# genome/bam-readcount

Measured on AMD Instinct MI355X. Metric: pileup base-events/sec, higher is better.
Workload: dtype u32+f32

## Files before the change

bam_readcount_amd/capi.py:

```python
import ctypes as C
import os

import numpy as np

HERE = os.path.dirname(os.path.abspath(__file__))
PRODUCT_LIB = os.path.join(HERE, "csrc", "libbrc_hip.so")

NBUCKET, NI, NF, NWARN, NKERNEL = 6, 9, 4, 4, 8
I_NAMES = ["n", "smq", "sse", "plus", "minus", "nq2", "smmq", "sclip", "sbq"]
F_NAMES = ["sev", "sq2", "snm", "s3p"]

EXPORTS = [
    "brc_strerror", "brc_last_error", "brc_kernel_name", "brc_engine_kind", "brc_create", "brc_destroy",
    "brc_begin_region", "brc_push_reads", "brc_upload", "brc_compute", "brc_fetch_result", "brc_end_region",
    "brc_clear_indel_queue", "brc_region_counts", "brc_format_region", "brc_format_window", "brc_region_windows", "brc_region_warnings", "brc_window_warnings", "brc_warnings_text", "brc_set_option", "brc_format_region_parts", "brc_set_chrom", "brc_fetch_window", "brc_compute_n", "brc_host_alloc", "brc_host_free", "brc_push_reads_pinned", "brc_region_piece_steps", "brc_device_view_get", "brc_device_indels_get",
]


class Stat(C.Structure):
    _fields_ = [("i", C.c_uint32 * NI), ("f", C.c_float * NF)]


class Config(C.Structure):
    _fields_ = [("abi_version", C.c_int32), ("min_mapq", C.c_int32), ("min_bq", C.c_int32), ("max_cnt", C.c_int32),
# ... 687 lines not shown
    "brc_panel_create", "brc_panel_destroy", "brc_panel_kind", "brc_panel_last_error", "brc_panel_gather", "brc_panel_last_timing",
]
PANEL_OUT_OF_RANGE, PANEL_NOT_ASCENDING = 1, 2
PANEL_DESTS = ("ncol", "depth", "unavail", "istat", "fstat", "metrics")


class Panel(_Handle):

    PREFIX, EXPORTS, LIB, NAME = "brc_panel", PANEL_EXPORTS, PANEL_LIB, "panel"
    PROTOS = {"brc_panel_gather": (C.c_int, [C.c_void_p, C.POINTER(DeviceView), C.c_void_p, C.c_int64, C.c_int64] + [C.c_void_p] * 8)}

    def gather_raw(self, view, idx, n, dst_stride, ncol=None, depth=None, unavail=None, istat=None, fstat=None, metrics=None, status=None,
                   stream=None):
        return self.lib.brc_panel_gather(self.h, _ref(view), idx, n, dst_stride,
                                         ncol, depth, unavail, istat, fstat, metrics, status, stream)

    def gather(self, view, idx, n, dst_stride, **kw):
        self._check("brc_panel_gather", self.gather_raw(view, idx, n, dst_stride, **kw))

    def last_timing(self):
        return super().last_timing()


SELECT_LIB = os.path.join(HERE, "csrc", "libbrc_select_hip.so")
SELECT_EXPORTS = [
    "brc_select_create", "brc_select_destroy", "brc_select_kind", "brc_select_last_error", "brc_select_workspace", "brc_select_sites",
    "brc_select_last_timing",
]
SELECT_SNV, SELECT_INDEL = 1, 2
ROLE_IGNORE, ROLE_CASE, ROLE_CONTROL = 0, 1, 2
SELECT_MAX_LIB = 254
WHY_A, WHY_C, WHY_G, WHY_T, WHY_INS, WHY_DEL = 1, 2, 4, 8, 16, 32


class SelectParams(C.Structure):
    _fields_ = [("role", C.c_void_p), ("flags", C.c_uint32), ("min_depth", C.c_uint32), ("min_alt", C.c_uint32), ("frac_num", C.c_uint32),
                ("frac_den", C.c_uint32), ("ctl_min_depth", C.c_uint32), ("ctl_max_alt", C.c_uint32), ("ctl_frac_num", C.c_uint32),
                ("ctl_frac_den", C.c_uint32)]


def select_params(role=None, flags=SELECT_SNV | SELECT_INDEL, min_depth=0, min_alt=1, frac=(0, 1), ctl_min_depth=0, ctl_max_alt=2 ** 32 - 1,
                  ctl_frac=(1, 1)):
    p = SelectParams(None, flags, min_depth, min_alt, frac[0], frac[1], ctl_min_depth, ctl_max_alt, ctl_frac[0], ctl_frac[1])
    keep = None
    if role is not None:
        keep = np.ascontiguousarray(role, np.uint8)
        p.role = keep.ctypes.data
    return p, keep


class Select(_Handle):

    PREFIX, EXPORTS, LIB, NAME = "brc_select", SELECT_EXPORTS, SELECT_LIB, "select"
    PROTOS = {"brc_select_workspace": (C.c_int64, [C.POINTER(DeviceView), C.POINTER(DeviceIndels), C.c_int64]),
              "brc_select_sites": (C.c_int, [C.c_void_p, C.POINTER(DeviceView), C.POINTER(DeviceIndels), C.POINTER(SelectParams), C.c_int64, C.c_int64, C.c_int64] +
                                   [C.c_void_p] * 5)}

    def workspace(self, view, indels, n):
        return int(self.lib.brc_select_workspace(_ref(view), _ref(indels), n))

    def sites_raw(self, view, indels, params, k0, n, cap=0, idx=None, why=None, counts=None, workspace=None, stream=None):
        return self.lib.brc_select_sites(self.h, _ref(view), _ref(indels), _ref(params), k0, n, cap, idx, why, counts, workspace, stream)

    def sites(self, view, indels, params, k0, n, **kw):
        self._check("brc_select_sites", self.sites_raw(view, indels, params, k0, n, **kw))

    def last_timing(self):
        return super().last_timing()


BINS_LIB = os.path.join(HERE, "csrc", "libbrc_bins_hip.so")
BINS_EXPORTS = [
    "brc_bins_create", "brc_bins_destroy", "brc_bins_kind", "brc_bins_last_error", "brc_bins_reduce", "brc_bins_last_timing",
]
BINS_NSUM, BINS_MAX_THR, BINS_MAX_HIST, BINS_MAX_LIB = 12, 8, 4096, 65535
BINS_S_DEPTH, BINS_S_NCOL, BINS_S_BUCKET, BINS_S_NONREF, BINS_S_INS, BINS_S_DEL, BINS_S_MAXDEPTH = 0, 1, 2, 8, 9, 10, 11
BINS_DESCENDS, BINS_OUTSIDE = 1, 2


class BinsParams(C.Structure):
    _fields_ = [("edges", C.c_void_p), ("width", C.c_int64), ("n_bins", C.c_int64), ("n_thr", C.c_int32), ("n_hist", C.c_int32),
                ("thr", C.c_uint32 * BINS_MAX_THR)]


def bins_params(width=0, edges=None, n_bins=0, thresholds=(), n_hist=0):
    p = BinsParams(edges, width, n_bins, len(thresholds), n_hist)
    for t, x in enumerate(thresholds[:BINS_MAX_THR]):
        p.thr[t] = x
    return p


class Bins(_Handle):

    PREFIX, EXPORTS, LIB, NAME = "brc_bins", BINS_EXPORTS, BINS_LIB, "bins"
    PROTOS = {"brc_bins_reduce": (C.c_int, [C.c_void_p, C.POINTER(DeviceView), C.POINTER(DeviceIndels), C.POINTER(BinsParams), C.c_int64, C.c_int64] +
                                  [C.c_void_p] * 3 + [C.c_int64, C.c_void_p, C.c_void_p])}

    def reduce_raw(self, view, indels, params, k0, n, dst_stride, sums=None, covered=None, hist=None, status=None, stream=None):
        return self.lib.brc_bins_reduce(self.h, _ref(view), _ref(indels), _ref(params), k0, n, sums, covered, hist, dst_stride, status, stream)

    def reduce(self, view, indels, params, k0, n, dst_stride, **kw):
        self._check("brc_bins_reduce", self.reduce_raw(view, indels, params, k0, n, dst_stride, **kw))

    def last_timing(self):
        return super().last_timing()


RUNS_LIB = os.path.join(HERE, "csrc", "libbrc_runs_hip.so")
RUNS_EXPORTS = [
    "brc_runs_create", "brc_runs_destroy", "brc_runs_kind", "brc_runs_last_error", "brc_runs_workspace", "brc_runs_find", "brc_runs_last_timing",
]
RUNS_MAX_LIB, RUNS_MAX_CUT = 254, 15
RUNS_MIN, RUNS_MAX, RUNS_SUM = 0, 1, 2
RUNS_REF_N = 1


class RunsParams(C.Structure):
    _fields_ = [("role", C.c_void_p), ("combine", C.c_uint32), ("n_cut", C.c_uint32), ("cut", C.c_uint32 * RUNS_MAX_CUT), ("keep", C.c_uint32),
                ("flags", C.c_uint32)]


def runs_params(cuts, combine=RUNS_MIN, role=None, keep=None, flags=0):
    cuts = list(cuts)
    p = RunsParams(None, combine, len(cuts))
    for i, x in enumerate(cuts[:RUNS_MAX_CUT]):
        p.cut[i] = x
    p.keep = (1 << (len(cuts) + (2 if flags & RUNS_REF_N else 1))) - 1 if keep is None else keep
    p.flags = flags
    keepalive = None
    if role is not None:
        keepalive = np.ascontiguousarray(role, np.uint8)
        p.role = keepalive.ctypes.data
    return p, keepalive


class Runs(_Handle):

    PREFIX, EXPORTS, LIB, NAME = "brc_runs", RUNS_EXPORTS, RUNS_LIB, "runs"
    PROTOS = {"brc_runs_workspace": (C.c_int64, [C.c_int64]),
              "brc_runs_find": (C.c_int, [C.c_void_p, C.POINTER(DeviceView), C.POINTER(DeviceIndels), C.POINTER(RunsParams), C.c_int64, C.c_int64, C.c_int64] +
                                [C.c_void_p] * 7)}

    def workspace(self, n):
        return int(self.lib.brc_runs_workspace(n))

    def find_raw(self, view, indels, params, k0, n, cap=0, start=None, end=None, cls=None, counts=None, per_class=None, workspace=None, stream=None):
        return self.lib.brc_runs_find(self.h, _ref(view), _ref(indels), _ref(params), k0, n, cap, start, end, cls, counts, per_class, workspace, stream)

    def find(self, view, indels, params, k0, n, **kw):
        self._check("brc_runs_find", self.find_raw(view, indels, params, k0, n, **kw))

    def last_timing(self):
        return super().last_timing()
```

bam_readcount_amd/csrc/brc_engine.hip:

```cpp
#include <hip/hip_runtime.h>
#include <atomic>
#include <chrono>

#include <stdio.h>
#include <stdlib.h>
#include <string.h>

#include <algorithm>
#include <string>
#include <mutex>
#include <vector>

#include "brc_host.h"

namespace brc {

struct Counters {
    unsigned long long n_events, n_positions, w_sm, w_nm, w_lib;
    unsigned int n_indel_slots, n_xev;
    unsigned int xev_max, n_wave_reads;
    unsigned int n_wave_big, n_wave_huge;
    unsigned int n_literal, n_wave_eqx;
    unsigned int n_wave_eqx_big, pad_;
};

#ifdef BRC_EXP_KNOBS
#define BRC_PVAR(n) (c.variant == (n))
#define BRC_AVAR(n) (c.ann_variant == (n))
#else
#define BRC_PVAR(n) false
#define BRC_AVAR(n) false
#endif


#ifdef BRC_CHECKED
__device__ __forceinline__ const char* uniform_ptr(const char* p) {
    const uint64_t v = (uint64_t)p;
    return (const char*)(((uint64_t)(uint32_t)__builtin_amdgcn_readfirstlane((int)(uint32_t)(v >> 32)) << 32) | (uint64_t)(uint32_t)__builtin_amdgcn_readfirstlane((int)(uint32_t)v));
}
#define BRC_CKS(c, K, SITE, BUF, p, bytes, unit, piece) uniform_ptr(BRC_CK(c, K, SITE, BUF, p, bytes, unit, piece))
#else
#define BRC_CKS(c, K, SITE, BUF, p, bytes, unit, piece) (p)
#endif

__device__ __forceinline__ unsigned long long wave_sum_u64(unsigned long long v) {
#pragma unroll
    for (int o = 32; o > 0; o >>= 1) v += __shfl_xor(v, o, 64);
    return v;
}

__device__ __forceinline__ uint32_t wave_sum_u32(uint32_t v) {
    v += (uint32_t)__builtin_amdgcn_update_dpp(0, (int)v, 0xB1, 0xf, 0xf, true);
    v += (uint32_t)__builtin_amdgcn_update_dpp(0, (int)v, 0x4E, 0xf, 0xf, true);
    v += (uint32_t)__builtin_amdgcn_update_dpp(0, (int)v, 0x141, 0xf, 0xf, true);
    v += (uint32_t)__builtin_amdgcn_update_dpp(0, (int)v, 0x140, 0xf, 0xf, true);
    v += (uint32_t)__builtin_amdgcn_update_dpp(0, (int)v, 0x142, 0xa, 0xf, false);
    v += (uint32_t)__builtin_amdgcn_update_dpp(0, (int)v, 0x143, 0xc, 0xf, false);
    return (uint32_t)__builtin_amdgcn_readlane((int)v, 63);
}

__device__ __forceinline__ uint64_t wave_min_u64(uint64_t v) {
#pragma unroll
    for (int o = 32; o > 0; o >>= 1) {
        const uint64_t u = ((uint64_t)(uint32_t)__shfl_xor((int)(uint32_t)(v >> 32), o, 64) << 32) | (uint64_t)(uint32_t)__shfl_xor((int)(uint32_t)v, o, 64);
        v = u < v ? u : v;
    }
    return ((uint64_t)(uint32_t)__builtin_amdgcn_readfirstlane((int)(uint32_t)(v >> 32)) << 32) | (uint64_t)(uint32_t)__builtin_amdgcn_readfirstlane((int)(uint32_t)v);
}

__device__ __forceinline__ int lane_shr1(int v) { return __builtin_amdgcn_update_dpp(0, v, 0x138, 0xf, 0xf, false); }
__device__ __forceinline__ int lane_shl1(int v) { return __builtin_amdgcn_update_dpp(0, v, 0x130, 0xf, 0xf, false); }


enum { REFCODE_PAD = 16 };
__global__ void k_divcheck(uint32_t* __restrict__ bad) {
    const uint32_t i = blockIdx.x * blockDim.x + threadIdx.x;
    const uint32_t n = i / DIV_SMALL_M, m = i % DIV_SMALL_M;
    if (n >= DIV_SMALL_N || m == 0u) return;
    const float q = div_small((float)n, (float)m), want = (float)n / (float)m;
    if (__float_as_uint(q) != __float_as_uint(want)) atomicAdd(bad, 1u);
}
__global__ __launch_bounds__(256) void k_refcode(const char* __restrict__ ref, uint8_t* __restrict__ code, int64_t n) {
    const int64_t i = (int64_t)blockIdx.x * blockDim.x + threadIdx.x;
    const int64_t j0 = i * 16 - REFCODE_PAD;
    if (j0 >= n + REFCODE_PAD) return;
    uint32_t w[4];
    uint8_t src[16];
    if (j0 >= 0 && j0 + 16 <= n) __builtin_memcpy(src, ref + j0, 16);
    else for (int k = 0; k < 16; ++k) { const int64_t j = j0 + k; src[k] = (j >= 0 && j < n) ? (uint8_t)ref[j] : (uint8_t)'N'; }
#pragma unroll
    for (int q = 0; q < 4; ++q) {
        uint32_t v = 0;
#pragma unroll
        for (int k = 0; k < 4; ++k) {
            const int64_t j = j0 + 4 * q + k;
            const uint32_t ch = src[4 * q + k];
            const uint32_t cd = (j >= 0 && j < n) ? (ch ? nt16_of_char(ch) : 0x8fu) : 0x0fu;
            v |= cd << (8 * k);
        }
        w[q] = v;
    }
    *reinterpret_cast<uint4*>(code + i * 16) = make_uint4(w[0], w[1], w[2], w[3]);
}

enum { AW_MCAP = 1024,
       AW_MCAP_BIG = 5120,
       AW_MCAP_HUGE = 13500,
       AW_MCAP_EQX = 768, AW_MCAP_EQX_BIG = 3840 };
struct AnnPar { uint4 a, b, c; };

__device__ __forceinline__ uint32_t nzb7(uint32_t x) { return x + 0x7f7f7f7fu; }

#ifndef BRC_ANN_WAVES_PER_EU
#define BRC_ANN_WAVES_PER_EU 6
#endif
#if BRC_ANN_WAVES_PER_EU > 0
#define BRC_ANN_OCC __attribute__((amdgpu_waves_per_eu(one_stream ? BRC_ANN_WAVES_PER_EU : 5, one_stream ? BRC_ANN_WAVES_PER_EU : 5)))
#else
#define BRC_ANN_OCC
#endif
template <bool one_stream, int SH>
__global__ __launch_bounds__(256) BRC_ANN_OCC void k_annotate_groups(DevCfg c, DevIn in, DRead* __restrict__ reads, const uint32_t* __restrict__ piece_off,
                                                         Piece* __restrict__ pieces, PieceRare* __restrict__ rare, int2* __restrict__ keyreach,
                                                         uint8_t* __restrict__ eb, IndelEv* __restrict__ ev_raw, uint32_t* __restrict__ bucket_cnt,
                                                         const uint32_t* __restrict__ cigar_ro, const uint8_t* __restrict__ qual_ro,
                                                         const uint8_t* __restrict__ seq_ro, const uint8_t* __restrict__ refcode,
                                                         const uint16_t* __restrict__ wanted ) {
    c.pack_shift = SH;
    struct WaveLds { AnnPar par[64]; uint32_t sum[64]; uint32_t redo[64]; uint32_t wide[64]; uint32_t G[64]; unsigned long long mark; };
    __shared__ WaveLds lds_all[4];
    const int lane = threadIdx.x & 63;
    const uint32_t wv = __builtin_amdgcn_readfirstlane((uint32_t)threadIdx.x >> 6);
    WaveLds& W = lds_all[wv];
    const int64_t rb = ((int64_t)blockIdx.x * 4 + wv) * 64;
    if (rb >= c.n_reads) return;
    const int nrd = (int)((c.n_reads - rb) < 64 ? (c.n_reads - rb) : 64);
    const int64_t my = rb + (lane < nrd ? lane : nrd - 1);
    const bool have = lane < nrd;
    const int32_t pos = in.pos[my];
    const uint32_t flag = in.flag[my];
    const int32_t L = in.l_qseq[my];
    const uint32_t nc = in.n_cigar[my];
    const uint64_t qoff = in.qual_off[my], soff = in.seq_off[my], brow = in.bq_row[my];
    const uint32_t coff = (uint32_t)in.cig_off[my];
    int32_t rlen = 0; int clipped = L, left_clip = 0, right_clip = L; int64_t tot_d = 0, tot_is = 0;
    uint32_t cig0 = 0, n_idp = 0;
    CigShape shape;
    int n_m = 0; int32_t m1lo = 0, m1hi = 0, m2lo = 0, m2hi = 0; int64_t d1 = 0, d2 = 0;
    {
        int rs = 0; int64_t x = pos;
#ifdef BRC_CHECKED
        const uint32_t* const cig_row = BRC_CK(c, CK_ANNOTATE, 1, CB_CIGAR, cigar_ro + coff, 4ull * nc, my, -1);
#define BRC_CIG_AT(k) cig_row[k]
#else
#define BRC_CIG_AT(k) cigar_ro[coff + (k)]
#endif
        for (uint32_t k = 0; k < nc; ++k) {
            const uint32_t cg = BRC_CIG_AT(k);
            if (k == 0) cig0 = cg;
            const uint32_t op = cg & 0xfu; const int len = (int)(cg >> 4);
            shape_add(shape, op, len);
            if (is_refop(op)) rlen += len;
            if (op == CINS || op == CDEL || op == CPAD) ++n_idp;
            if (op == CDEL || op == CREF_SKIP) tot_d += len;
            if (op == CINS || op == CSOFT_CLIP) tot_is += len;
// ... 1567 lines not shown
__global__ __launch_bounds__(256) void k_xev_fold(const XEv* __restrict__ list, uint32_t* __restrict__ cnt, uint32_t* __restrict__ end, int64_t n_buckets, uint32_t* __restrict__ idx, XAgg* __restrict__ out) {
    for (int64_t b = (int64_t)blockIdx.x * 256 + threadIdx.x; b < n_buckets; b += (int64_t)gridDim.x * 256) {
        const uint32_t n = cnt[b];
        if (!n) continue;
        const uint32_t start = end[b] - n;
        const int nd = fold_xev_bucket(list, idx + start, (int)n, out + start);
        for (uint32_t j = (uint32_t)nd; j < n; ++j) out[start + j].k = NONE32;
        cnt[b] = (uint32_t)nd; end[b] = start + (uint32_t)nd;
    }
}
__global__ __launch_bounds__(256) void k_last_processed(DevCfg c, const uint32_t* __restrict__ ncol, const uint32_t* __restrict__ unavail, uint32_t* __restrict__ last) {
    __shared__ uint32_t best;
    const int l = blockIdx.x;
    if (threadIdx.x == 0) best = 0u;
    __syncthreads();
    for (int64_t hi = c.P; hi > 0; hi -= 256) {
        const int64_t k = hi - 1 - (int64_t)threadIdx.x;
        if (k >= 0 && ncol[(int64_t)l * c.PS + k] != 0u && !(c.per_lib && unavail[k] != NONE32)) atomicMax(&best, (uint32_t)k + 1u);
        __syncthreads();
        const uint32_t seen = best;
        __syncthreads();
        if (seen) break;
    }
    if (threadIdx.x == 0) last[l] = best ? best - 1u : NONE32;
}

__global__ __launch_bounds__(256) void k_text_len(DevCfg c, DevIn in, Planes pl, TextCtx t, TextAux ax, uint32_t* __restrict__ len) {
    const int64_t k = (int64_t)blockIdx.x * blockDim.x + threadIdx.x;
    if (k > c.P) return;
    len[k] = k < c.P ? text_line(c, in, pl, t, ax, k, nullptr) : 0u;
}
__global__ __launch_bounds__(256) void k_text_total(const uint32_t* __restrict__ len, int64_t n, unsigned long long* __restrict__ total) {
    unsigned long long v = 0ull;
    for (int64_t k = (int64_t)blockIdx.x * blockDim.x + threadIdx.x; k < n; k += (int64_t)gridDim.x * blockDim.x) v += len[k];
#pragma unroll
    for (int o = 32; o > 0; o >>= 1) v += (unsigned long long)__shfl_xor((long long)v, o, 64);
    if ((threadIdx.x & 63) == 0 && v) atomicAdd(total, v);
}
__global__ __launch_bounds__(256) void k_text_write(DevCfg c, DevIn in, Planes pl, TextCtx t, TextAux ax, const uint32_t* __restrict__ off, char* __restrict__ text) {
    const int64_t k = (int64_t)blockIdx.x * blockDim.x + threadIdx.x;
    if (k >= c.P || off[k + 1] == off[k]) return;
    (void)text_line(c, in, pl, t, ax, k, text + off[k]);
}

__global__ __launch_bounds__(256) void k_indel_scatter(DevCfg c, const IndelEv* __restrict__ raw, int64_t n_raw, uint32_t* __restrict__ cursor,
                                                       IndelEv* __restrict__ ev) {
    const int64_t i = (int64_t)blockIdx.x * blockDim.x + threadIdx.x;
    if (i >= n_raw) return;
    const IndelEv e = raw[i];
    if (e.key_lo == NONE32) return;
    ev[atomicAdd(&cursor[indel_bucket(c, e.key_lo)], 1u)] = e;
}

__global__ __launch_bounds__(256) void k_unavail(DevCfg c, DevIn in, uint32_t* __restrict__ unavail) {
    const int64_t i = (int64_t)blockIdx.x * blockDim.x + threadIdx.x;
    if (i >= c.n_reads || in.lib[i] >= 0) return;
    const uint32_t nc = in.n_cigar[i]; const uint32_t* cg = in.cigar + in.cig_off[i];
    if (!read_enters(in.flag[i], cg, nc) || in.pos[i] < 0) return;
    int64_t rlen = 0;
    for (uint32_t k = 0; k < nc; ++k) if (is_refop(cg[k] & 0xfu)) rlen += (int64_t)(cg[k] >> 4);
    int64_t k0 = (int64_t)in.pos[i] - c.pos0, k1 = k0 + rlen;
    if (k0 < 0) k0 = 0;
    if (k1 > c.P) k1 = c.P;
    for (int64_t k = k0; k < k1; ++k) atomicMin(&unavail[k], (uint32_t)i);
}

__global__ __launch_bounds__(256) void k_indel_reduce(DevCfg c, DevIn in, const DRead* __restrict__ reads, const uint32_t* __restrict__ cnt,
                                                      const uint32_t* __restrict__ cursor, int64_t n_buckets, IndelEv* __restrict__ ev,
                                                      const uint32_t* __restrict__ unavail, IndelOut* __restrict__ out,
                                                      Counters* __restrict__ ctr) {
    __shared__ unsigned long long sh[4 * 2];
    unsigned long long w[2] = {0, 0};
    if (blockIdx.x == 0 && threadIdx.x == 0) ctr->n_indel_slots = n_buckets > 0 ? cursor[n_buckets - 1] : 0u;
    const int64_t stride = (int64_t)gridDim.x * blockDim.x;
    for (int64_t b = (int64_t)blockIdx.x * blockDim.x + threadIdx.x; b < n_buckets; b += stride) {
        const uint32_t n = cnt[b];
        if (!n) continue;
        const uint32_t start = cursor[b] - n;
        uint32_t wsm = 0, wnm = 0;
        reduce_indel_bucket(c, in, reads, ev + start, (int)n, unavail, out + start, wsm, wnm);
        w[0] += wsm; w[1] += wnm;
    }
    block_sum_u64<2>(w, sh);
    if (threadIdx.x == 0) {
        if (w[0]) atomicAdd(&ctr->w_sm, w[0]);
        if (w[1]) atomicAdd(&ctr->w_nm, w[1]);
    }
}


static void* pinned_alloc(size_t n) {
    void* p = nullptr;
    if (hipHostMalloc(&p, n ? n : 1, hipHostMallocDefault) != hipSuccess) return nullptr;
    return p;
}
static void pinned_release(void* p) { (void)hipHostFree(p); }
static const HostAlloc kPinned = {pinned_alloc, pinned_release};

template <class T>
struct PBuf : HBuf<T> {
    PBuf() { this->A = &kPinned; } ~PBuf() { this->destroy(); }
    PBuf(const PBuf&) = delete; PBuf& operator=(const PBuf&) = delete;
};

static std::atomic<uint64_t> g_dev_allocs{0}, g_dev_alloc_ns{0};
template <class T>
struct DBuf {
    T* p = nullptr; size_t cap = 0;
    size_t req = 0;
    DBuf() = default; DBuf(const DBuf&) = delete; DBuf& operator=(const DBuf&) = delete;
    ~DBuf() { if (p) (void)hipFree(p); }
    template <class U> U* as() const { return reinterpret_cast<U*>(p); }
    hipError_t ensure(size_t bytes) {
        req = bytes;
        if (bytes <= cap) return hipSuccess;
        struct Tm { std::chrono::steady_clock::time_point t0 = std::chrono::steady_clock::now();
                    ~Tm() { g_dev_alloc_ns += (uint64_t)std::chrono::duration_cast<std::chrono::nanoseconds>(std::chrono::steady_clock::now() - t0).count(); ++g_dev_allocs; } } tm_;
        const bool regrow = p != nullptr;
        if (p) { (void)hipFree(p); p = nullptr; cap = 0; }
        size_t want = bytes + (regrow ? bytes / 2 : bytes / 8) + 256;
        hipError_t e = hipMalloc((void**)&p, want);
        if (e != hipSuccess) { e = hipMalloc((void**)&p, bytes); want = bytes; }
        if (e == hipSuccess) cap = want;
        return e;
    }
};

template <class H, hipError_t (*DESTROY)(H)>
struct Owned {
    H h = nullptr;
    Owned() = default; Owned(const Owned&) = delete; Owned& operator=(const Owned&) = delete;
    ~Owned() { if (h) (void)DESTROY(h); }
    operator H() const { return h; }
};
typedef Owned<hipStream_t, hipStreamDestroy> Stream;
typedef Owned<hipEvent_t, hipEventDestroy> Event;

enum { T_ANNOTATE = 0, T_SCAN_ENDS, T_TILES, T_PILEUP, T_COUNT, T_INDEL_SCAN, T_INDEL_FILL, T_INDEL_REDUCE, T_N };
static const char* kKernelNames[BRC_NKERNEL] = {"k_annotate", "k_scan_ends", "k_tiles", "k_pileup", "k_xev_fold+finalize",
                                                "k_scan_indel", "k_indel_fill", "k_indel_reduce"};

#define HIPCHK(x) do { hipError_t _e = (x); if (_e != hipSuccess) { return hip_fail(_e, #x); } } while (0)

[[maybe_unused]] static void pin_instantiation_order() {
    const void* const k[] = {(const void*)k_annotate_groups<true, 16>, (const void*)k_annotate_groups<true, 12>, (const void*)k_annotate_groups<false, 16>, (const void*)k_annotate_groups<false, 12>,
        (const void*)k_annotate_wave<16, AW_MCAP, 4>, (const void*)k_annotate_wave<12, AW_MCAP, 4>, (const void*)k_annotate_wave<16, AW_MCAP_BIG, 1>, (const void*)k_annotate_wave<12, AW_MCAP_BIG, 1>,
        (const void*)k_annotate_wave<16, AW_MCAP_EQX, 4, true>, (const void*)k_annotate_wave<12, AW_MCAP_EQX, 4, true>, (const void*)k_annotate_wave<16, AW_MCAP_EQX_BIG, 1, true>, (const void*)k_annotate_wave<12, AW_MCAP_EQX_BIG, 1, true>,
        (const void*)k_annotate_wave<16, AW_MCAP_HUGE, 1>, (const void*)k_annotate_wave<12, AW_MCAP_HUGE, 1>, (const void*)k_annotate_cursor<16>, (const void*)k_annotate_cursor<12>,
        (const void*)k_scan_reduce<OpSumU32>, (const void*)k_scan_aggregates<OpSumU32>, (const void*)k_scan_apply<OpSumU32, false>, (const void*)k_scan_aggregates<OpMaxU64>, (const void*)k_compact_tiles<true>, (const void*)k_compact_tiles<false>,
        (const void*)k_pileup2<true, 16>, (const void*)k_pileup2<true, 12>, (const void*)k_pileup2<false, 16>, (const void*)k_pileup2<false, 12>};
    (void)k;
}

class HipBackend : public Backend {
    std::string err; int device = 0;
    DevCfg c; DevIn in;
    int64_t ntiles = 0; uint64_t n_indel_cap = 0;
    std::vector<int64_t> lib_base;
    std::vector<uint16_t> h_wanted; bool has_wanted = false; std::vector<uint32_t> h_tilelist;
    unsigned wide_slices = 1;
    bool text_started[2] = {false, false}; uint64_t text_total[2] = {0, 0}; int64_t text_n[2] = {0, 0}; int text_slot = 0;
    std::mutex text_mu;
    Planes pl_last;
    enum { COMPACT_PIECES_PER_READ = 12 };
    bool compact_on = false; uint64_t compact_total = 0; bool compact_sized = false;
    struct { const uint4* pieces; const PieceRare* rare; const uint2* rng; } kp = {nullptr, nullptr, nullptr};
    bool wave_on = false;
    bool wave_big = false;
    enum { WAVE_FORM_BLOCKS = 768,
           WAVE_FORM_BLOCKS_BIG = 512,
           WAVE_FORM_BLOCKS_HUGE = 256 };
    bool wave_huge = false;
    bool wave_eqx = false; uint32_t s_max_ncigar = 0;
    bool cursor_on = false;
    unsigned long long h_steps[3] = {0, 0, 0};
    std::vector<XAgg> xagg_compact; std::vector<IndelOut> iout_compact;
    enum { XEV_SHARDS = 1024 }; size_t xev_cap = 0;
    Counters h_ctr; bool computed = false;
    bool lists_enqueued = false, lists_host = false;
    Stream stream, stream2;
    enum { EV_RING = 32 };
    struct EvSet { Event evt[T_N + 1], ev_indel[4]; };
    EvSet evsets[EV_RING]; size_t n_evsets = 0;
    Event* evt = nullptr; Event* ev_indel = nullptr;
    Event ev_text[2], ev_lines;
    PBuf<Staged::WidePair> h_wpairs; PBuf<char> h_text[2]; PBuf<uint32_t> h_toff[2], h_total, h_lastproc[2];
    struct HostSet { PBuf<uint32_t> ncol, depth, slotid, si, unavail; PBuf<float> sf; } h_pl, w_pl;
    PBuf<IndelOut> h_iout; PBuf<XAgg> h_xagg;
    DBuf<int32_t> d_pos, d_lq, d_nm, d_sm; DBuf<uint16_t> d_flag; DBuf<uint8_t> d_mapq, d_tags, d_seq, d_qual; DBuf<int16_t> d_lib;
    DBuf<uint32_t> d_nc, d_cigar, d_pieceoff, d_ievoff; DBuf<uint64_t> d_co, d_so, d_qo, d_bqrow; DBuf<char> d_ref; DBuf<uint8_t> d_refcode;
    DBuf<uint16_t> d_wanted; DBuf<uint32_t> d_tilelist; DBuf<uint2> d_wpairs; DBuf<int64_t> d_libbase;
    DBuf<uint8_t> d_bq; DBuf<uint16_t> d_bqw; DBuf<Piece> d_pieces; DBuf<PieceRare> d_rare; DBuf<int2> d_keyreach; DBuf<DRead> d_reads;
    DBuf<uint32_t> d_wavelist, d_nc_k1; DBuf<unsigned long long> d_agg; DBuf<uint2> d_rng;
    DBuf<uint32_t> d_ccnt, d_coff; DBuf<Piece> d_cpieces; DBuf<PieceRare> d_crare; DBuf<uint2> d_crng; DBuf<unsigned long long> d_ctot;
    DBuf<uint32_t> d_ncol, d_depth, d_slotid, d_si, d_unavail; DBuf<float> d_sf; DBuf<uint4> d_tilectr; DBuf<unsigned long long> d_part; DBuf<Counters> d_ctr;
    DBuf<XEv> d_xev, d_xevc; DBuf<uint32_t> d_xevn, d_xcnt, d_xend, d_xidx; DBuf<XAgg> d_xagg;
    DBuf<uint32_t> d_cnt, d_cursor; DBuf<IndelEv> d_ev, d_evraw; DBuf<IndelOut> d_iout;
    DBuf<uint32_t> d_tlen, d_toff, d_lastproc; DBuf<char> d_text, d_tctx; DBuf<unsigned long long> d_total64;
#ifdef BRC_CHECKED
    DBuf<ChkState> d_chk; ChkState h_chk;
    void chk_fill() {
        memset(&h_chk, 0, sizeof h_chk);
        auto set = [&](int b, const auto& d) { h_chk.ext[b].lo = (uint64_t)d.p; h_chk.ext[b].hi = (uint64_t)d.p + d.req; };
        set(CB_CIGAR, d_cigar); set(CB_SEQ, d_seq); set(CB_QUAL, d_qual); set(CB_REFCODE, d_refcode); set(CB_EB, d_bq); set(CB_BQW, d_bqw);
        set(CB_PIECES, d_pieces); set(CB_RARE, d_rare); set(CB_KEYREACH, d_keyreach); set(CB_READS, d_reads); set(CB_EVRAW, d_evraw); set(CB_CNT, d_cnt);
        set(CB_WANTED, d_wanted); set(CB_RNG, d_rng); set(CB_UNAVAIL, d_unavail); set(CB_TILELIST, d_tilelist); set(CB_NCOL, d_ncol); set(CB_DEPTH, d_depth);
        set(CB_SLOTID, d_slotid); set(CB_SI, d_si); set(CB_SF, d_sf); set(CB_XEV, d_xev); set(CB_XEVN, d_xevn); set(CB_TILECTR, d_tilectr);
        const bool cz = compact_on && compact_sized;
        set(CB_KP_PIECES, cz ? d_cpieces : d_pieces); set(CB_KP_RARE, cz ? d_crare : d_rare); set(CB_KP_RNG, cz ? d_crng : d_rng);
        if (const char* sh = getenv("BRC_CHECKED_SHRINK")) { const int b = atoi(sh); const char* cpos = strchr(sh, ':'); if (b >= 0 && b < CB_N && cpos) { const uint64_t by = strtoull(cpos + 1, nullptr, 10); ChkExt& x = h_chk.ext[b]; x.hi = x.hi - x.lo > by ? x.hi - by : x.lo; } }
    }
    int chk_report() {
        if (hipMemcpy(&h_chk, d_chk.p, sizeof h_chk, hipMemcpyDeviceToHost) != hipSuccess) { err = "checked build: cannot read the fault record"; return BRC_E_HIP; }
        if (!h_chk.count) return BRC_OK;
        static const char* const kBuf[CB_N] = {"cigar", "seq4", "qual", "refcode", "event bytes", "wide words", "pieces", "rare records", "keyreach", "reads", "raw indel events", "indel bucket counts",
                                               "wanted lanes", "tile ranges", "unavail", "tile list", "ncol", "depth", "slotid", "integer slot planes", "float slot planes", "third-allele lists",
                                               "third-allele cursors", "tile counters", "LDS rows", "LDS queue", "pieces (pileup)", "rare records (pileup)", "tile ranges (pileup)"};
        char b[512];
        snprintf(b, sizeof b, "BRC_CHECKED: %u out-of-bounds device access(es); first: kernel %s, site %u, buffer '%s' [0x%llx, 0x%llx), address 0x%llx + %llu bytes (offset %lld), %s %lld, piece %lld",
                 h_chk.count, h_chk.kernel == CK_ANNOTATE ? "k_annotate_groups" : "k_pileup2", h_chk.site, h_chk.buf < CB_N ? kBuf[h_chk.buf] : "?",
                 (unsigned long long)h_chk.ext[h_chk.buf < CB_N ? h_chk.buf : 0].lo, (unsigned long long)h_chk.ext[h_chk.buf < CB_N ? h_chk.buf : 0].hi, (unsigned long long)h_chk.addr,
                 (unsigned long long)h_chk.bytes, (long long)(h_chk.addr - h_chk.ext[h_chk.buf < CB_N ? h_chk.buf : 0].lo), h_chk.kernel == CK_ANNOTATE ? "read" : "tile", (long long)h_chk.unit, (long long)h_chk.piece);
        err = b; fprintf(stderr, "%s\n", b);
        return BRC_E_HIP;
    }
#endif

    int hip_fail(hipError_t e, const char* what) {
        char b[512];
        snprintf(b, sizeof b, "%s: %s", what, hipGetErrorString(e));
        err = b;
        return e == hipErrorOutOfMemory ? BRC_E_NOMEM : BRC_E_HIP;
    }
    bool indels_active() const { return n_indel_cap > 0 && c.P > 0 && c.n_reads > 0; }
    int ensure_xev_lists() {
        const size_t n = (size_t)XEV_SHARDS * xev_cap + 1;
        HIPCHK(d_xev.ensure(n * sizeof(XEv))); HIPCHK(d_xevc.ensure(n * sizeof(XEv))); HIPCHK(d_xidx.ensure(n * 4)); HIPCHK(d_xagg.ensure(n * sizeof(XAgg)));
        return BRC_OK;
    }

  public:
    int init(int dev) {
        int n = 0;
        if (hipGetDeviceCount(&n) != hipSuccess || n <= 0) { err = "no HIP device visible"; return BRC_E_NODEVICE; }
        if (dev < 0 || dev >= n) { err = "device ordinal out of range"; return BRC_E_NODEVICE; }
        device = dev;
        HIPCHK(hipSetDevice(device));
        HIPCHK(hipStreamCreateWithFlags(&stream.h, hipStreamNonBlocking));
        { const int rc0 = ensure_evsets(1); if (rc0) return rc0; }
        HIPCHK(hipStreamCreateWithFlags(&stream2.h, hipStreamNonBlocking));
        {
            uint32_t* d_bad = nullptr; uint32_t bad = 0;
            HIPCHK(hipMalloc(&d_bad, sizeof(uint32_t)));
            HIPCHK(hipMemsetAsync(d_bad, 0, sizeof(uint32_t), stream));
            hipLaunchKernelGGL(k_divcheck, dim3((DIV_SMALL_N * DIV_SMALL_M + 255) / 256), dim3(256), 0, stream, d_bad);
            HIPCHK(hipMemcpyAsync(&bad, d_bad, sizeof(uint32_t), hipMemcpyDeviceToHost, stream));
            HIPCHK(hipStreamSynchronize(stream));
            (void)hipFree(d_bad);
            if (bad) { err = "this device's reciprocal does not give correctly rounded small-integer quotients (div_small self-check failed)"; return BRC_E_HIP; }
        }
        for (Event& e : ev_text) HIPCHK(hipEventCreateWithFlags(&e.h, hipEventDisableTiming));
        HIPCHK(hipEventCreateWithFlags(&ev_lines.h, hipEventDisableTiming));
        return BRC_OK;
    }
    ~HipBackend() override {
        (void)hipSetDevice(device);
        if (getenv("BRC_ENGINE_TIMING")) fprintf(stderr, "device buffers: %llu (re)allocations, %.3f s\n", (unsigned long long)g_dev_allocs.load(), (double)g_dev_alloc_ns.load() * 1e-9);
    }
    int ensure_evsets(size_t n) {
        for (; n_evsets < n; ++n_evsets) {
            for (Event& e : evsets[n_evsets].evt) if (!e.h) HIPCHK(hipEventCreate(&e.h));
            for (Event& e : evsets[n_evsets].ev_indel) if (!e.h) HIPCHK(hipEventCreate(&e.h));
        }
        evt = evsets[0].evt; ev_indel = evsets[0].ev_indel;
        return BRC_OK;
    }
    const HostAlloc* host_alloc() override { return &kPinned; }
    const char* last_error() const override { return err.c_str(); }

    template <class T>
    int up(DBuf<T>& d, const HBuf<T>& h, size_t n) {
        HIPCHK(d.ensure((n + 16) * sizeof(T)));
        if (n) HIPCHK(hipMemcpyAsync(d.p, h.p, n * sizeof(T), hipMemcpyHostToDevice, stream));
        return BRC_OK;
    }

    int up_arena(DBuf<uint8_t>& d, const HBuf<uint8_t>& h, const std::vector<Staged::Seg>& segs, uint64_t total) {
        if (segs.empty()) return up(d, h, h.n);
        HIPCHK(d.ensure((size_t)total + 16));
        for (const Staged::Seg& g : segs) if (g.n) HIPCHK(hipMemcpyAsync(d.p + g.off, g.p, (size_t)g.n, hipMemcpyHostToDevice, stream));
        return BRC_OK;
    }
    bool adopts_arenas() const override { return true; }

    int upload(const brc_config& cfg, const Staged& s, Geometry& g) override {
        HIPCHK(hipSetDevice(device));
        computed = false;
        memset(&c, 0, sizeof c);
        c.min_mapq = cfg.min_mapq; c.min_bq = cfg.min_bq; c.per_lib = cfg.per_lib; c.insertion_centric = cfg.insertion_centric;
        c.Lp = g.Lp; c.ref_len_check = cfg.ref_len_check; c.has_ref = g.ref != nullptr;
        g.PS = (g.P + 63) & ~(int64_t)63;
        c.beg0 = g.beg0; c.end = g.end; c.pos0 = g.pos0; c.P = g.P; c.PS = g.PS; c.ref_lo = g.ref_lo; c.ref_hi = g.ref_hi; c.ref_len = g.ref_len;
        c.n_reads = s.n; c.table_len = test_knob(TK_NO_TABLE) ? 0 : s.modal_len();
        c.n_pieces = s.n_pieces; lib_base = s.lib_base; c.max_lqseq = s.max_lqseq;
        c.ibucket_shift = indel_bucket_shift(s.n_indel_ops, c.P, c.Lp);
        if (const char* ib = test_knob(TK_IBUCKET_SHIFT)) { const int v = atoi(ib); if (v == 2 || v == 4 || v == 6) c.ibucket_shift = v; }
        choose_pack(s.max_lqseq, test_knob(TK_FLUSH_K) ? atoi(test_knob(TK_FLUSH_K)) : 0, test_knob(TK_PACK_LIM) ? atoi(test_knob(TK_PACK_LIM)) : 0, c.flush_k, c.pack_lim, c.pack_lim_lo, c.pack_shift);
        c.force_dom = test_knob(TK_FORCE_DOM) ? atoi(test_knob(TK_FORCE_DOM)) : -1;
#ifdef BRC_CHECKED
        HIPCHK(d_chk.ensure(sizeof(ChkState))); c.chk = d_chk.p;
#endif
#ifdef BRC_EXP_KNOBS
        c.variant = getenv("BRC_PILEUP_VARIANT") ? atoi(getenv("BRC_PILEUP_VARIANT")) : 0;
        c.ann_variant = getenv("BRC_ANN_VARIANT") ? atoi(getenv("BRC_ANN_VARIANT")) : 0;
#endif
        compact_on = s.n > 0 && s.n_pieces > (int64_t)COMPACT_PIECES_PER_READ * s.n;
        if (const char* ck = test_knob(TK_COMPACT)) compact_on = atoi(ck) != 0 && s.n_pieces > 0;
        compact_sized = false; compact_total = 0; h_steps[0] = h_steps[1] = h_steps[2] = 0;
        const size_t n = (size_t)s.n;
        int rc;
        if ((rc = up(d_pos, s.pos, n)) || (rc = up(d_flag, s.flag, n)) || (rc = up(d_mapq, s.mapq, n)) || (rc = up(d_lib, s.lib, n)) ||
            (rc = up(d_lq, s.l_qseq, n)) || (rc = up(d_nc, s.n_cigar, n)) || (rc = up(d_co, s.cig_off, n)) || (rc = up(d_so, s.seq_off, n)) ||
            (rc = up(d_qo, s.qual_off, n)) || (rc = up(d_nm, s.nm, n)) || (rc = up(d_sm, s.sm, n)) || (rc = up(d_tags, s.tags, n)) ||
            (rc = up(d_cigar, s.cigar, s.cigar.n)) || (rc = up_arena(d_seq, s.seq4, s.seq_seg, s.seq_total)) || (rc = up_arena(d_qual, s.qual, s.qual_seg, s.qual_total)))
            return rc;
        const size_t rl = (size_t)(g.ref_hi - g.ref_lo);
        HIPCHK(d_ref.ensure(rl + 16));
        HIPCHK(d_refcode.ensure(rl + 2 * REFCODE_PAD + 16));
        if (rl) HIPCHK(hipMemcpyAsync(d_ref.p, g.ref + g.ref_lo, rl, hipMemcpyHostToDevice, stream));
        in.pos = d_pos.p; in.flag = d_flag.p; in.mapq = d_mapq.p; in.lib = d_lib.p; in.l_qseq = d_lq.p; in.n_cigar = d_nc.p; in.cig_off = d_co.p;
        in.seq_off = d_so.p; in.qual_off = d_qo.p; in.nm = d_nm.p; in.sm = d_sm.p; in.tags = d_tags.p; in.cigar = d_cigar.p; in.seq4 = d_seq.p; in.qual = d_qual.p;
        in.ref = d_ref.p;
        HIPCHK(d_bq.ensure(s.bq_elems + EB_PAD_FRONT + EB_PAD_BACK + (size_t)std::max<int32_t>(s.max_lqseq, 0)));
        {
            if (s.bq_elems >> 34) { err = "region too large: 2^34 bases and more"; return BRC_E_LIMIT; }
            const size_t tab_bytes = ((((size_t)(s.bq_elems >> 4) + 2) * 4) + 255) & ~(size_t)255;
            h_wpairs.clear();
            { const size_t nw = s.n_wide(); if (!h_wpairs.reserve(nw + 1)) { err = "host allocation failed (wide-stream list)"; return BRC_E_NOMEM; } h_wpairs.n = nw; }
            const uint64_t wq_elems = s.wide_layout(h_wpairs.p, (uint32_t)(tab_bytes / 32));
            {
                const uint64_t groups = (h_wpairs.n + 63) / 64, per_group = groups ? (wq_elems >> 4) / groups : 0;
                wide_slices = (unsigned)std::min<uint64_t>(std::max<uint64_t>(per_group / 512, 1), 64);
            }
            if ((tab_bytes / 32 + (wq_elems >> 4)) >> 32) { err = "region too large: 2^36 bases of reads with escape bases"; return BRC_E_LIMIT; }
            HIPCHK(d_bqw.ensure(tab_bytes + ((size_t)wq_elems + 16) * sizeof(uint16_t)));
            in.bqw = d_bqw.p;
#ifdef BRC_CHECKED
            HIPCHK(hipMemsetAsync(d_bqw.p, 0xff, tab_bytes, stream));
#endif
            if (h_wpairs.n) {
                HIPCHK(d_wpairs.ensure(h_wpairs.n * sizeof(Staged::WidePair)));
                HIPCHK(hipMemcpyAsync(d_wpairs.p, h_wpairs.p, h_wpairs.n * sizeof(Staged::WidePair), hipMemcpyHostToDevice, stream));
            }
        }
        in.eb = d_bq.p + EB_PAD_FRONT;
        if ((rc = up(d_bqrow, s.bq_row, n)) || (rc = up(d_pieceoff, s.piece_off, n))) return rc;
        in.bq_row = d_bqrow.p;
        in.rcp = nullptr;
        const size_t np = (size_t)c.n_pieces;
        HIPCHK(d_pieces.ensure((np + 4) * sizeof(Piece))); HIPCHK(d_rare.ensure((np + 2) * sizeof(PieceRare)));
        HIPCHK(d_keyreach.ensure((np + 16) * sizeof(int2)));
        wave_eqx = n > 0 && c.has_ref && s.has_eqx && s.max_ncigar >= 3;
        wave_on = n > 0 && c.has_ref && (s.max_ncigar >= 5 || wave_eqx);
        s_max_ncigar = s.max_ncigar;
        if (const char* wk = test_knob(TK_WAVE_FORM)) { wave_on = wave_on && atoi(wk) != 0; wave_eqx = wave_eqx && wave_on; }
        wave_big = wave_on && s.max_ncigar > (uint32_t)AW_MCAP;
        wave_huge = wave_on && s.max_ncigar > (uint32_t)AW_MCAP_BIG;
        cursor_on = n > 0 && s.has_empty_m;
        if (wave_on || cursor_on) { HIPCHK(d_wavelist.ensure((4 * (size_t)n + 96) * sizeof(uint32_t))); HIPCHK(d_nc_k1.ensure(((size_t)n + 16) * sizeof(uint32_t))); }
        HIPCHK(d_libbase.ensure((lib_base.size() + 1) * sizeof(int64_t)));
        if (!lib_base.empty()) HIPCHK(hipMemcpyAsync(d_libbase.p, lib_base.data(), lib_base.size() * sizeof(int64_t), hipMemcpyHostToDevice, stream));
        const size_t P = (size_t)c.PS, Lp = (size_t)c.Lp;
        ntiles = (c.P + TILE - 1) / TILE;
        n_indel_cap = c.has_ref ? s.n_indel_ops : 0;
        h_wanted = s.wanted_tiles(c.pos0, c.P); has_wanted = !h_wanted.empty();
        h_tilelist.clear();
        if (has_wanted) {
            HIPCHK(d_wanted.ensure(h_wanted.size() * 2 + 16)); HIPCHK(hipMemcpyAsync(d_wanted.p, h_wanted.data(), h_wanted.size() * 2, hipMemcpyHostToDevice, stream));
            for (size_t t = 0; t < h_wanted.size(); ++t) if (h_wanted[t] != (uint16_t)TILE_UNWANTED) h_tilelist.push_back((uint32_t)t);
            HIPCHK(d_tilelist.ensure(h_tilelist.size() * 4 + 16));
            if (!h_tilelist.empty()) HIPCHK(hipMemcpyAsync(d_tilelist.p, h_tilelist.data(), h_tilelist.size() * 4, hipMemcpyHostToDevice, stream));
        }
        if (n_indel_cap && ((uint64_t)c.P * (uint64_t)c.Lp >= 0xffffffffull || n_indel_cap >= 0xfffffff0ull)) { err = "region too large: (positions x libraries) and the indel operators must stay below 2^32"; return BRC_E_ARG; }
        const size_t nagg = std::max<size_t>(std::max<size_t>((std::max<size_t>(np, P * Lp) + SCAN_CHUNK - 1) / SCAN_CHUNK, (np + TR_CHUNK - 1) / TR_CHUNK), 1);
        HIPCHK(d_reads.ensure((n + 1) * sizeof(DRead)));
        HIPCHK(d_agg.ensure(nagg * 8 + 16)); HIPCHK(d_rng.ensure(((size_t)ntiles * Lp + 1) * sizeof(uint2)));
        HIPCHK(d_ncol.ensure(Lp * P * 4 + 16)); HIPCHK(d_depth.ensure(Lp * P * 4 + 16)); HIPCHK(d_unavail.ensure(P * 4 + 16));
        HIPCHK(d_slotid.ensure(Lp * P * 4 + 16)); HIPCHK(d_si.ensure(Lp * 2 * NI * P * 4 + 16)); HIPCHK(d_sf.ensure(Lp * 2 * NF * P * 4 + 16));
        {
            const char* xc = test_knob(TK_XEV_CAP);
            const size_t want = xc ? (size_t)std::max(atoi(xc), 1) : std::max<size_t>(256, np / 8 / XEV_SHARDS);
            if (want > xev_cap) xev_cap = want;
        }
        if ((rc = ensure_xev_lists())) return rc;
        HIPCHK(d_xevn.ensure((size_t)XEV_SHARDS * XEV_CTR_STRIDE * 4));
        HIPCHK(d_xcnt.ensure(((size_t)ntiles * Lp + 2) * 4)); HIPCHK(d_xend.ensure(((size_t)ntiles * Lp + 2) * 4));
        HIPCHK(d_part.ensure(4096 * 5 * sizeof(unsigned long long)));
        HIPCHK(d_ctr.ensure(sizeof(Counters))); HIPCHK(d_tilectr.ensure(((size_t)ntiles * Lp + 1) * sizeof(uint4)));
        in.iev_off = nullptr;
        if (n_indel_cap) {
            const size_t nbk = (size_t)indel_buckets(c);
            if ((rc = up(d_ievoff, s.iev_off, n))) return rc;
            in.iev_off = d_ievoff.p;
            HIPCHK(d_cnt.ensure(nbk * 4 + 16)); HIPCHK(d_cursor.ensure(nbk * 4 + 16)); HIPCHK(d_evraw.ensure((n_indel_cap + 1) * sizeof(IndelEv)));
            HIPCHK(d_ev.ensure((n_indel_cap + 1) * sizeof(IndelEv))); HIPCHK(d_iout.ensure((n_indel_cap + 1) * sizeof(IndelOut)));
        }
        if (has_wanted && P) {
            HIPCHK(hipMemsetAsync(d_ncol.p, 0, Lp * P * 4, stream)); HIPCHK(hipMemsetAsync(d_depth.p, 0, Lp * P * 4, stream));
            HIPCHK(hipMemsetD32Async((hipDeviceptr_t)d_slotid.p, (int)((uint32_t)NB_NONE | ((uint32_t)NB_NONE << 8)), Lp * P, stream));
            HIPCHK(hipMemsetAsync(d_tilectr.p, 0, (size_t)ntiles * Lp * sizeof(uint4), stream));
        }
        HIPCHK(hipStreamSynchronize(stream));
        return BRC_OK;
    }

    template <class K> K by_pack(K k16, K k12) const { return c.pack_shift == 16 ? k16 : k12; }
    uint8_t* eb_out() const { return d_bq.p + EB_PAD_FRONT; }
    IndelEv* evraw() const { return indels_active() ? d_evraw.p : nullptr; }
    const uint16_t* wanted() const { return has_wanted ? d_wanted.p : nullptr; }
    const uint8_t* refcode() const { return d_refcode.p + REFCODE_PAD; }

    void launch_annotate_groups(const DevIn& in_k1) {
        const auto k = c.Lp == 1 ? by_pack(k_annotate_groups<true, 16>, k_annotate_groups<true, 12>) : by_pack(k_annotate_groups<false, 16>, k_annotate_groups<false, 12>);
        hipLaunchKernelGGL(k, dim3((unsigned)((c.n_reads + 255) / 256)), dim3(256), 0, stream, c, in_k1, d_reads.p, d_pieceoff.p, d_pieces.p, d_rare.p, d_keyreach.p,
                           eb_out(), evraw(), d_cnt.p, in.cigar, in.qual, in.seq4, refcode(), wanted());
    }
    template <int MCAP, int WAVES, bool EQX = false>
    void launch_annotate_wave(unsigned grid, const uint32_t* list, int step, const unsigned int* count) {
        hipLaunchKernelGGL(by_pack(k_annotate_wave<16, MCAP, WAVES, EQX>, k_annotate_wave<12, MCAP, WAVES, EQX>), dim3(grid), dim3(WAVES * 64), 0, stream, c, in, list, step, count,
                           d_reads.p, d_pieceoff.p, d_pieces.p, d_rare.p, d_keyreach.p, eb_out(), evraw(), d_cnt.p, refcode(), wanted());
    }
    void launch_annotate_cursor() {
        hipLaunchKernelGGL(by_pack(k_annotate_cursor<16>, k_annotate_cursor<12>), dim3((unsigned)std::min<int64_t>((c.n_reads + 63) / 64, 1024)), dim3(64), 0, stream, c, in,
                           d_wavelist.p + (2 * (size_t)c.n_reads + 32), &d_ctr.p->n_literal, d_reads.p, d_pieceoff.p, d_pieces.p, d_rare.p, d_keyreach.p, eb_out(), evraw(), d_cnt.p, wanted());
    }
    template <class Op, bool INCL>
    int scan(const typename Op::T* src, typename Op::T* dst, int64_t n) {
        if (n <= 0) return BRC_OK;
        const int64_t nb = (n + SCAN_CHUNK - 1) / SCAN_CHUNK;
        typename Op::T* agg = d_agg.as<typename Op::T>();
        hipLaunchKernelGGL((k_scan_reduce<Op>), dim3((unsigned)nb), dim3(SCAN_T), 0, stream, src, n, agg);
        hipLaunchKernelGGL((k_scan_aggregates<Op>), dim3(1), dim3(1024), 0, stream, agg, nb);
        hipLaunchKernelGGL((k_scan_apply<Op, INCL>), dim3((unsigned)nb), dim3(SCAN_T), 0, stream, src, dst, n, agg);
        HIPCHK(hipGetLastError());
        return BRC_OK;
    }
    template <bool COUNT>
    void launch_compact_tiles() {
        hipLaunchKernelGGL((k_compact_tiles<COUNT>), dim3((unsigned)((ntiles + 3) / 4), (unsigned)c.Lp), dim3(256), 0, stream, c, d_pieces.as<const uint4>(), d_rare.p, d_rng.p, ntiles, d_ccnt.p,
                           COUNT ? nullptr : d_coff.p, COUNT ? nullptr : d_cpieces.as<uint4>(), COUNT ? nullptr : d_crare.p, COUNT ? nullptr : d_crng.p, d_ctot.p);
    }
    void stage_pileup() {
        const int64_t n_listed = (int64_t)h_tilelist.size();
        if (ntiles <= 0 || (has_wanted && n_listed == 0)) return;
        unsigned nwg = (unsigned)(((has_wanted ? n_listed : ntiles) + PILEUP_WAVES - 1) / PILEUP_WAVES);
        nwg = (nwg + 7u) & ~7u;
#ifdef BRC_EXP_KNOBS
        static const unsigned dyn_lds = getenv("BRC_PILEUP_LDS_PAD") ? (unsigned)atoi(getenv("BRC_PILEUP_LDS_PAD")) : 0u;
#else
        const unsigned dyn_lds = 0u;
#endif
        const auto k = has_wanted ? by_pack(k_pileup2<true, 16>, k_pileup2<true, 12>) : by_pack(k_pileup2<false, 16>, k_pileup2<false, 12>);
        hipLaunchKernelGGL(k, dim3(nwg, (unsigned)c.Lp), dim3(PILEUP_WAVES * 64), dyn_lds, stream, c, in, kp.pieces, kp.rare, kp.rng, ntiles, pl_last, d_tilectr.p, in.eb, in.bqw, d_unavail.p,
                           refcode(), d_wanted.p, d_tilelist.p, n_listed);
    }

    int stage_annotate() {
        const int64_t n = c.n_reads;
        if (n <= 0) { if (c.per_lib && c.P > 0) HIPCHK(hipMemsetAsync(d_unavail.p, 0xff, (size_t)c.PS * 4, stream)); return BRC_OK; }
        Counters* const ctr = d_ctr.p;
        const int64_t rl = c.ref_hi - c.ref_lo;
        if (c.has_ref)
            hipLaunchKernelGGL(k_refcode, dim3((unsigned)(((rl + 2 * REFCODE_PAD + 15) / 16 + 255) / 256)), dim3(256), 0, stream, in.ref, d_refcode.p, rl);
        if (h_wpairs.n)
            hipLaunchKernelGGL(k_wide_rows, dim3((unsigned)((h_wpairs.n + 255) / 256), wide_slices), dim3(256), 0, stream, c, in, d_wpairs.p, (uint32_t)h_wpairs.n, d_bqw.p);
        DevIn in_k1 = in;
        if (wave_on || cursor_on) {
            hipLaunchKernelGGL(k_pick_wave, dim3((unsigned)((n + 255) / 256)), dim3(256), 0, stream, c, in, d_nc_k1.p, d_wavelist.p, (uint32_t)n, &ctr->n_wave_reads, &ctr->n_wave_big, &ctr->n_wave_huge,
                               wave_on ? 1 : 0, cursor_on ? 1 : 0, &ctr->n_literal, &ctr->n_wave_eqx, &ctr->n_wave_eqx_big);
            in_k1.n_cigar = d_nc_k1.p;
        }
        launch_annotate_groups(in_k1);
        if (wave_on) {
            const uint32_t* const wl = d_wavelist.p;
            const unsigned nb = (unsigned)std::min<int64_t>((n + 3) / 4, (int64_t)WAVE_FORM_BLOCKS), nb_big = (unsigned)std::min<int64_t>(n, (int64_t)WAVE_FORM_BLOCKS_BIG);
            launch_annotate_wave<AW_MCAP, 4>(nb, wl, 1, &ctr->n_wave_reads);
            if (wave_big)
                launch_annotate_wave<AW_MCAP_BIG, 1>(nb_big, wl + (n - 1), -1, &ctr->n_wave_big);
            if (wave_eqx) {
                launch_annotate_wave<AW_MCAP_EQX, 4, true>(nb, wl + (3 * n + 48), 1, &ctr->n_wave_eqx);
                if (s_max_ncigar > (uint32_t)AW_MCAP_EQX) launch_annotate_wave<AW_MCAP_EQX_BIG, 1, true>(nb_big, wl + (4 * n + 47), -1, &ctr->n_wave_eqx_big);
            }
            if (wave_huge)
                launch_annotate_wave<AW_MCAP_HUGE, 1>((unsigned)std::min<int64_t>(n, (int64_t)WAVE_FORM_BLOCKS_HUGE), wl + (n + 16), 1, &ctr->n_wave_huge);
        }
        if (cursor_on) launch_annotate_cursor();
        if (c.per_lib) {
            HIPCHK(hipMemsetAsync(d_unavail.p, 0xff, (size_t)c.PS * 4, stream));
            hipLaunchKernelGGL(k_unavail, dim3((unsigned)((n + 255) / 256)), dim3(256), 0, stream, c, in, d_unavail.p);
        }
        return BRC_OK;
    }
    bool have_tiles() const { return c.n_pieces > 0 && ntiles > 0; }
    unsigned reach_blocks() const { return (unsigned)((c.n_pieces + TR_CHUNK - 1) / TR_CHUNK); }
    void stage_tile_reach() {
        if (!have_tiles()) return;
        hipLaunchKernelGGL(k_reach_blockmax, dim3(reach_blocks()), dim3(TR_T), 0, stream, d_keyreach.p, c.n_pieces, d_libbase.p, c.Lp, d_agg.p);
        hipLaunchKernelGGL((k_scan_aggregates<OpMaxU64>), dim3(1), dim3(1024), 0, stream, d_agg.p, (int64_t)reach_blocks());
    }
    int stage_tile_ranges() {
        const int Lp = c.Lp;
        for (int l = 0; l < Lp && ntiles > 0; ++l)
            if (lib_base[(size_t)l + 1] == lib_base[(size_t)l]) HIPCHK(hipMemsetAsync(d_rng.p + (int64_t)l * ntiles, 0, (size_t)ntiles * sizeof(uint2), stream));
        if (have_tiles())
            hipLaunchKernelGGL(k_tiles_all, dim3(reach_blocks()), dim3(TR_T), 0, stream, c, d_keyreach.p, c.n_pieces, d_libbase.p, Lp, d_agg.p, ntiles, d_rng.p);
        const int64_t n_listed = (int64_t)h_tilelist.size();
        if (has_wanted && n_listed > 0)
            hipLaunchKernelGGL(k_narrow_tiles, dim3((unsigned)((n_listed * Lp + 255) / 256)), dim3(256), 0, stream, d_wanted.p, d_tilelist.p, n_listed, ntiles, Lp, c.pos0, d_rng.p, d_keyreach.p);
        kp = {d_pieces.as<const uint4>(), d_rare.p, d_rng.p};
        return BRC_OK;
    }
    int stage_compact() {
        if (!compact_on || !have_tiles()) return BRC_OK;
        int rc; const int64_t np_all = c.n_pieces;
        const size_t nslot = (size_t)ntiles * (size_t)c.Lp;
        HIPCHK(d_ccnt.ensure((nslot + 2) * 4)); HIPCHK(d_coff.ensure((nslot + 2) * 4)); HIPCHK(d_crng.ensure((nslot + 1) * sizeof(uint2))); HIPCHK(d_ctot.ensure(24));
        HIPCHK(hipMemsetAsync(d_ctot.p, 0, 24, stream));
        HIPCHK(hipMemsetAsync(d_ccnt.p + nslot, 0, 4, stream));
        const bool by_read = c.Lp == 1 && !(test_knob(TK_COMPACT) && atoi(test_knob(TK_COMPACT)) == 2);
        if (by_read) {
            HIPCHK(hipMemsetAsync(d_ccnt.p, 0, nslot * 4, stream));
            hipLaunchKernelGGL(k_count_piece_tiles, dim3((unsigned)((np_all + 255) / 256)), dim3(256), 0, stream, c, d_pieces.as<const uint4>(), np_all, d_ccnt.p);
        } else launch_compact_tiles<true>();
        if ((rc = scan<OpSumU32, false>(d_ccnt.p, d_coff.p, (int64_t)nslot + 1))) return rc;
        const bool first_pass = !compact_sized;
        if (first_pass) {
            uint32_t tot = 0;
            HIPCHK(hipMemcpyAsync(&tot, d_coff.p + nslot, 4, hipMemcpyDeviceToHost, stream));
            HIPCHK(hipMemcpyAsync(h_steps, d_ctot.p, 16, hipMemcpyDeviceToHost, stream));
            HIPCHK(hipStreamSynchronize(stream));
            compact_total = tot; compact_sized = true;
            HIPCHK(d_cpieces.ensure(((size_t)compact_total + 4) * sizeof(Piece))); HIPCHK(d_crare.ensure(((size_t)compact_total + 2) * sizeof(PieceRare)));
        }
        if (by_read)
            hipLaunchKernelGGL(k_compact_reads, dim3((unsigned)((ntiles + 4 * CR_GROUP - 1) / (4 * CR_GROUP))), dim3(256), 0, stream, c, d_pieces.as<const uint4>(), d_rare.p, d_rng.p, d_pieceoff.p, d_keyreach.p, ntiles,
                               d_coff.p, d_cpieces.as<uint4>(), d_crare.p, d_crng.p, d_ctot.p);
        else launch_compact_tiles<false>();
        if (by_read && first_pass) {
            HIPCHK(hipMemcpyAsync(h_steps, d_ctot.p, 24, hipMemcpyDeviceToHost, stream));
            HIPCHK(hipStreamSynchronize(stream));
            if (h_steps[2]) { err = "tile compaction: a tile holds more live read segments than the pass over the segments counted for it"; return BRC_E_HIP; }
        }
        kp = {d_cpieces.as<const uint4>(), d_crare.p, d_crng.p};
#ifdef BRC_CHECKED
        {
            HIPCHK(hipStreamSynchronize(stream));
            ChkState seen; HIPCHK(hipMemcpy(&seen, d_chk.p, sizeof seen, hipMemcpyDeviceToHost));
            chk_fill(); ChkState upd = h_chk; upd.count = seen.count; upd.kernel = seen.kernel; upd.site = seen.site; upd.buf = seen.buf; upd.addr = seen.addr; upd.bytes = seen.bytes; upd.unit = seen.unit; upd.piece = seen.piece;
            HIPCHK(hipMemcpy(d_chk.p, &upd, sizeof upd, hipMemcpyHostToDevice));
        }
#endif
        return BRC_OK;
    }
    int stage_xev_fold() {
        if (ntiles <= 0) return BRC_OK;
        int rc; const int64_t nxb = ntiles * c.Lp;
        HIPCHK(hipMemsetAsync(d_xcnt.p, 0, (size_t)nxb * 4, stream));
        hipLaunchKernelGGL(k_xev_compact, dim3((unsigned)XEV_SHARDS), dim3(256), 0, stream, d_xev.p, d_xevn.p, (uint32_t)xev_cap, (uint32_t)XEV_SHARDS, d_xevc.p, d_ctr.p, d_xcnt.p, c.Lp);
        if ((rc = scan<OpSumU32, false>(d_xcnt.p, d_xend.p, nxb))) return rc;
        hipLaunchKernelGGL(k_xev_scatter, dim3(256), dim3(256), 0, stream, d_xevc.p, d_ctr.p, d_xend.p, d_xidx.p, c.Lp);
        hipLaunchKernelGGL(k_xev_fold, dim3((unsigned)std::min<int64_t>((nxb + 255) / 256, 2048)), dim3(256), 0, stream, d_xevc.p, d_xcnt.p, d_xend.p, nxb, d_xidx.p, d_xagg.p);
        return BRC_OK;
    }
    void stage_counters() {
        if (c.P <= 0) return;
        const unsigned nb = (unsigned)std::min<int64_t>(((c.Lp > 1 ? c.P / 4 : ntiles) + 255) / 256 + 1, c.Lp > 1 ? 4096 : 256);
        hipLaunchKernelGGL(k_finalize, dim3(nb), dim3(256), 0, stream, c, d_ncol.p, d_tilectr.p, (int64_t)ntiles * c.Lp, d_part.p);
        hipLaunchKernelGGL(k_finalize_sum, dim3(1), dim3(256), 0, stream, d_part.p, (int)nb, d_ctr.p);
    }
    int stage_indels() {
        int rc; const int64_t n_buckets = indel_buckets(c);
        HIPCHK(hipEventRecord(ev_indel[0], stream));
        if ((rc = scan<OpSumU32, false>(d_cnt.p, d_cursor.p, n_buckets))) return rc;
        HIPCHK(hipEventRecord(ev_indel[1], stream));
        hipLaunchKernelGGL(k_indel_scatter, dim3((unsigned)((n_indel_cap + 255) / 256)), dim3(256), 0, stream, c, d_evraw.p, (int64_t)n_indel_cap, d_cursor.p, d_ev.p);
        HIPCHK(hipEventRecord(ev_indel[2], stream));
        hipLaunchKernelGGL(k_indel_reduce, dim3((unsigned)std::min<int64_t>((n_buckets + 255) / 256, 4096)), dim3(256), 0, stream, c, in, d_reads.p, d_cnt.p, d_cursor.p, n_buckets, d_ev.p, d_unavail.p,
                           d_iout.p, d_ctr.p);
        HIPCHK(hipEventRecord(ev_indel[3], stream));
        return BRC_OK;
    }

    int enqueue_pass(size_t set) {
        evt = evsets[set].evt; ev_indel = evsets[set].ev_indel;
        int rc;
        lists_host = lists_enqueued = false;
        HIPCHK(hipMemsetAsync(d_ctr.p, 0, sizeof(Counters), stream));
        HIPCHK(hipMemsetAsync(d_xevn.p, 0, (size_t)XEV_SHARDS * XEV_CTR_STRIDE * 4, stream));
        if (indels_active()) HIPCHK(hipMemsetAsync(d_cnt.p, 0, (size_t)indel_buckets(c) * 4, stream));
#ifdef BRC_CHECKED
        if (set == 0) { chk_fill(); HIPCHK(hipMemcpyAsync(d_chk.p, &h_chk, sizeof h_chk, hipMemcpyHostToDevice, stream)); HIPCHK(hipStreamSynchronize(stream)); }
#endif
        pl_last = Planes{d_ncol.p, d_depth.p, d_slotid.p, d_si.p, d_sf.p, d_unavail.p, d_xev.p, d_xevn.p, (uint32_t)xev_cap, (uint32_t)XEV_SHARDS};
        HIPCHK(hipEventRecord(evt[T_ANNOTATE], stream));
        if ((rc = stage_annotate())) return rc;
        HIPCHK(hipEventRecord(evt[T_SCAN_ENDS], stream));
        stage_tile_reach();
        HIPCHK(hipEventRecord(evt[T_TILES], stream));
        if ((rc = stage_tile_ranges()) || (rc = stage_compact())) return rc;
        HIPCHK(hipEventRecord(evt[T_PILEUP], stream));
        stage_pileup();
        HIPCHK(hipEventRecord(evt[T_COUNT], stream));
        if ((rc = stage_xev_fold())) return rc;
        stage_counters();
        HIPCHK(hipEventRecord(evt[T_INDEL_SCAN], stream));
        if (indels_active() && (rc = stage_indels())) return rc;
        HIPCHK(hipEventRecord(evt[T_N], stream));
        HIPCHK(hipGetLastError());
        return BRC_OK;
    }
    int finish_passes(bool* again) {
        HIPCHK(hipMemcpyAsync(&h_ctr, d_ctr.p, sizeof(Counters), hipMemcpyDeviceToHost, stream));
        HIPCHK(hipStreamSynchronize(stream));
        *again = false;
#ifdef BRC_CHECKED
        { const int rcc = chk_report(); if (rcc) return rcc; }
#endif
        if ((size_t)h_ctr.xev_max > xev_cap) {
            xev_cap = (size_t)h_ctr.xev_max * 2;
            const int rc = ensure_xev_lists(); if (rc) return rc;
            *again = true;
        }
        return BRC_OK;
    }
    int add_timing(size_t set, brc_timing* t) {
// ... 218 lines not shown
```

bam_readcount_amd/csrc/brc_host.cpp:

```cpp
#if defined(__x86_64__)
#include <immintrin.h>
#endif
#include "brc_host.h"

#include <math.h>
#include <stdio.h>
#include <stdlib.h>

#include <algorithm>
#include <atomic>
#include <chrono>
#include <deque>
#include <thread>
#include <functional>
#include <memory>
#include <queue>
#include <condition_variable>

namespace brc {

static unsigned probe_cpus() {
    unsigned n = std::thread::hardware_concurrency(); if (n == 0) n = 1;
    double quota = 0;
    if (FILE* f = fopen("/sys/fs/cgroup/cpu.max", "r")) {
        char q[64]; long long per = 0;
        if (fscanf(f, "%63s %lld", q, &per) == 2 && strcmp(q, "max") != 0 && per > 0) quota = atof(q) / (double)per;
        fclose(f);
    } else {
        long long q = -1, per = 0;
        if (FILE* g = fopen("/sys/fs/cgroup/cpu/cpu.cfs_quota_us", "r")) { if (fscanf(g, "%lld", &q) != 1) q = -1; fclose(g); }
        if (FILE* g = fopen("/sys/fs/cgroup/cpu/cpu.cfs_period_us", "r")) { if (fscanf(g, "%lld", &per) != 1) per = 0; fclose(g); }
        if (q > 0 && per > 0) quota = (double)q / (double)per;
    }
    if (quota > 0 && quota < (double)n) n = (unsigned)(quota + 0.999);
    if (n < 1) n = 1;
    return n;
}
unsigned effective_cpus() { static const unsigned cached = probe_cpus(); return cached; }

static inline double now_s() { return std::chrono::duration<double>(std::chrono::steady_clock::now().time_since_epoch()).count(); }

template <class F>
static void parallel_for(int64_t n, unsigned nthr, F fn) {
    if (n <= 0) return;
    if (nthr > (unsigned)n) nthr = (unsigned)n;
    if (nthr <= 1) { for (int64_t i = 0; i < n; ++i) fn(i); return; }
    std::atomic<int64_t> next(0);
    auto work = [&]() { for (;;) { const int64_t i = next.fetch_add(1); if (i >= n) break; fn(i); } };
    std::vector<std::thread> th;
    for (unsigned t = 1; t < nthr; ++t) th.emplace_back(work);
    work();
    for (std::thread& t : th) t.join();
}

class Pool {
    std::vector<std::thread> th;
    std::mutex mu; std::condition_variable cv_go, cv_done;
    std::function<void(int64_t)> job; int64_t job_n = 0; std::atomic<int64_t> next{0};
    uint64_t gen = 0; unsigned busy = 0; bool stop = false;
    void worker() {
        uint64_t seen = 0;
        for (;;) {
            { std::unique_lock<std::mutex> lk(mu); cv_go.wait(lk, [&] { return stop || gen != seen; }); if (stop) return; seen = gen; }
            for (;;) { const int64_t i = next.fetch_add(1); if (i >= job_n) break; job(i); }
            { std::lock_guard<std::mutex> lk(mu); if (--busy == 0) cv_done.notify_one(); }
        }
    }
  public:
    explicit Pool(unsigned n) { try { th.reserve(n); for (unsigned t = 0; t < n; ++t) th.emplace_back([this] { worker(); }); } catch (...) {} }
    ~Pool() { { std::lock_guard<std::mutex> lk(mu); stop = true; } cv_go.notify_all(); for (std::thread& t : th) t.join(); }
    unsigned size() const { return (unsigned)th.size() + 1; }
    template <class F> void run(int64_t n, F fn) {
        if (n <= 0) return;
        if (th.empty() || n == 1) { for (int64_t i = 0; i < n; ++i) fn(i); return; }
        { std::lock_guard<std::mutex> lk(mu); job = fn; job_n = n; next = 0; busy = (unsigned)th.size(); ++gen; }
        cv_go.notify_all();
        for (;;) { const int64_t i = next.fetch_add(1); if (i >= n) break; fn(i); }
        std::unique_lock<std::mutex> lk(mu); cv_done.wait(lk, [&] { return busy == 0; });
    }
};

void Staged::init(const HostAlloc* A) { each_buf([A](auto& h) { h.A = A; }); }
void Staged::clear() {
    each_buf([](auto& h) { h.clear(); });
    bq_elems = 0; memset(len_hist, 0, sizeof len_hist); n = 0; min_pos = 0; max_end = 0; n_indel_ops = 0;
    seq_seg.clear(); qual_seg.clear(); seq_total = 0; qual_total = 0;
    lib_base.clear(); n_pieces = 0; max_lqseq = 0; max_ncigar = 0; has_empty_m = false; has_eqx = false; max_span = 0;
    win_beg.clear(); win_end.clear();
}
void Staged::destroy() { each_buf([](auto& h) { h.destroy(); }); }
bool Staged::reserve_reads(size_t reads, size_t cigar_ops) {
    bool ok = cigar.reserve(cigar_ops);
    each_read_buf([&](auto& h) { ok = ok && h.reserve(reads); });
    return ok;
}
std::vector<uint16_t> Staged::wanted_tiles(int32_t pos0, int64_t P) const {
    std::vector<uint16_t> w;
    if (win_beg.empty() || P <= 0) return w;
    const int64_t nt = (P + TILE - 1) / TILE;
    w.assign((size_t)nt, (uint16_t)TILE_UNWANTED);
    for (size_t i = 0; i < win_beg.size(); ++i) {
        int64_t k0 = (int64_t)win_beg[i] - 1 - pos0, k1 = (int64_t)win_end[i] - pos0;
        if (k0 < 0) k0 = 0;
        if (k1 > P) k1 = P;
        for (int64_t t = k0 / TILE; k1 > k0 && t <= (k1 - 1) / TILE; ++t) {
            const uint32_t a = (uint32_t)std::max<int64_t>(k0 - t * TILE, 0), b = (uint32_t)std::min<int64_t>(k1 - 1 - t * TILE, TILE - 1);
            uint16_t& x = w[(size_t)t];
            if (x == (uint16_t)TILE_UNWANTED) x = (uint16_t)(a | (b << 8));
            else x = (uint16_t)(std::min<uint32_t>(x & 0xffu, a) | (std::max<uint32_t>(x >> 8, b) << 8));
        }
    }
    return w;
}
void Staged::layout_pieces(int Lp, bool per_lib) {
    lib_base.assign((size_t)Lp + 1, 0);
    for (int64_t i = 0; i < n; ++i) if (piece_cnt.p[i]) lib_base[(size_t)(per_lib ? lib.p[i] : 0) + 1] += piece_cnt.p[i];
    for (int l = 0; l < Lp; ++l) lib_base[(size_t)l + 1] += lib_base[(size_t)l];
    n_pieces = lib_base[(size_t)Lp];
    std::vector<int64_t> cur(lib_base.begin(), lib_base.end() - 1);
    piece_off.n = (size_t)n;
    for (int64_t i = 0; i < n; ++i) {
        const int l = per_lib ? (int)lib.p[i] : 0;
        if (!piece_cnt.p[i]) { piece_off.p[i] = (uint32_t)cur[(size_t)((l >= 0 && l < Lp) ? l : 0)]; continue; }
        piece_off.p[i] = (uint32_t)cur[(size_t)l]; cur[(size_t)l] += piece_cnt.p[i];
    }
    if (per_lib && Lp > 1) {
        std::vector<uint64_t> rows((size_t)Lp + 2, 0);
        auto slot = [&](int64_t i) { const int l = (int)lib.p[i]; return (size_t)((l >= 0 && l < Lp) ? l : Lp); };
        for (int64_t i = 0; i < n; ++i) rows[slot(i) + 1] += ((uint64_t)l_qseq.p[i] + 15u) & ~(uint64_t)15u;
        for (int l = 0; l <= Lp; ++l) rows[(size_t)l + 1] += rows[(size_t)l];
        for (int64_t i = 0; i < n; ++i) { const size_t k = slot(i); bq_row.p[i] = rows[k]; rows[k] += ((uint64_t)l_qseq.p[i] + 15u) & ~(uint64_t)15u; }
    }
}
uint64_t Staged::wide_layout(WidePair* pairs, uint32_t first16) const {
    uint64_t w = 0; size_t k = 0;
    for (int64_t i = 0; i < n; ++i) if (wide.p[i]) {
        if (pairs) { WidePair x; x.read = (uint32_t)i; x.w16 = first16 + (uint32_t)(w >> 4); pairs[k++] = x; }
        w += ((uint64_t)l_qseq.p[i] + 15u) & ~(uint64_t)15u;
    }
    return w;
}
static bool read_has_escape_words(const uint8_t* qual, const uint8_t* seq4, int32_t L) {
    if (L <= 0) return false;
    const uint64_t K01 = 0x0101010101010101ull, K80 = 0x8080808080808080ull, K7F = 0x7f7f7f7f7f7f7f7full;
    int32_t j = 0;
    for (; j + 8 <= L; j += 8) {
        uint64_t x; memcpy(&x, qual + j, 8);
        const uint64_t zero = (x - K01) & ~x & K80;
        const uint64_t big = (((x & K7F) + (uint64_t)(128 - EB_ESC) * K01) | x) & K80;
        if (zero | big) return true;
    }
    for (; j < L; ++j) if ((uint8_t)(qual[j] - 1u) >= (uint8_t)(EB_ESC - 1)) return true;
    const int32_t nb = L / 2;
    const uint64_t K11 = 0x1111111111111111ull, K88 = 0x8888888888888888ull;
    int32_t t = 0;
    for (; t + 8 <= nb; t += 8) {
        uint64_t x; memcpy(&x, seq4 + t, 8);
        if ((x - K11) & ~x & K88) return true;
        if (x & (x - K11)) return true;
    }
    auto bad = [](uint32_t n) { return n == 0u || (n & (n - 1u)) != 0u; };
    for (; t < nb; ++t) if (bad(seq4[t] >> 4) || bad(seq4[t] & 15u)) return true;
    if ((L & 1) && bad(seq4[nb] >> 4)) return true;
    return false;
}
#if defined(__x86_64__)
__attribute__((target("ssse3"))) static bool read_has_escape_ssse3(const uint8_t* qual, const uint8_t* seq4, int32_t L) {
    if (L < 32) return read_has_escape_words(qual, seq4, L);
    const __m128i one = _mm_set1_epi8(1), lim = _mm_set1_epi8((char)(EB_ESC - 1)), zero = _mm_setzero_si128(), m0f = _mm_set1_epi8(0x0f);
    const __m128i lut = _mm_setr_epi8(0, 1, 1, 0, 1, 0, 0, 0, 1, 0, 0, 0, 0, 0, 0, 0);
    __m128i bad = zero;
#define BRC_Q16(p) { const __m128i t_ = _mm_sub_epi8(_mm_loadu_si128(reinterpret_cast<const __m128i*>(p)), one); bad = _mm_or_si128(bad, _mm_cmpeq_epi8(_mm_max_epu8(t_, lim), t_)); }
#define BRC_S16(p) { const __m128i x_ = _mm_loadu_si128(reinterpret_cast<const __m128i*>(p)); \
                     const __m128i ok_ = _mm_and_si128(_mm_shuffle_epi8(lut, _mm_and_si128(x_, m0f)), _mm_shuffle_epi8(lut, _mm_and_si128(_mm_srli_epi16(x_, 4), m0f))); \
                     bad = _mm_or_si128(bad, _mm_cmpeq_epi8(ok_, zero)); }
    int32_t j = 0;
    for (; j + 16 <= L; j += 16) BRC_Q16(qual + j)
    if (j < L) BRC_Q16(qual + L - 16)
    if (_mm_movemask_epi8(bad)) return true;
    const int32_t nb = L / 2;
    int32_t t = 0;
    for (; t + 16 <= nb; t += 16) BRC_S16(seq4 + t)
    if (t < nb) BRC_S16(seq4 + nb - 16)
    if (_mm_movemask_epi8(bad)) return true;
#undef BRC_Q16
#undef BRC_S16
    if (L & 1) { const uint32_t n = seq4[nb] >> 4; if (n == 0u || (n & (n - 1u)) != 0u) return true; }
    return false;
}
static bool read_has_escape(const uint8_t* qual, const uint8_t* seq4, int32_t L) {
    static const bool ssse3 = __builtin_cpu_supports("ssse3") != 0;
    return ssse3 ? read_has_escape_ssse3(qual, seq4, L) : read_has_escape_words(qual, seq4, L);
}
#else
static bool read_has_escape(const uint8_t* qual, const uint8_t* seq4, int32_t L) { return read_has_escape_words(qual, seq4, L); }
#endif

static const char kD2[201] =
    "00010203040506070809101112131415161718192021222324252627282930313233343536373839404142434445464748495051525354555657585960616263646566676869"
    "707172737475767778798081828384858687888990919293949596979899";

static inline int fmt_u64(char* out, uint64_t v) {
    char t[24]; int n = 0;
    while (v >= 100) { const unsigned d = (unsigned)(v % 100); v /= 100; t[n++] = kD2[2 * d + 1]; t[n++] = kD2[2 * d]; }
    if (v >= 10) { t[n++] = kD2[2 * v + 1]; t[n++] = kD2[2 * v]; } else t[n++] = (char)('0' + v);
    for (int i = 0; i < n; ++i) out[i] = t[n - 1 - i];
    return n;
}
int fmt_u32(char* out, uint32_t v) {
    if (v < 10) { out[0] = (char)('0' + v); return 1; }
    if (v < 100) { out[0] = kD2[2 * v]; out[1] = kD2[2 * v + 1]; return 2; }
    return fmt_u64(out, v);
}

int fmt_f2(char* out, float v) {
    if (!(fabsf(v) < 4.0e13f)) return snprintf(out, 64, "%.2f", (double)v);
    const double s = fabs((double)v * 100.0);
    volatile double big = s + 4503599627370496.0;
    const uint64_t u = (uint64_t)(big - 4503599627370496.0);
    int n = 0;
    if (signbit(v)) out[n++] = '-';
    const uint64_t ip = u / 100; const unsigned fr = (unsigned)(u % 100);
    n += ip < 100 ? fmt_u32(out + n, (uint32_t)ip) : fmt_u64(out + n, ip);
    out[n++] = '.'; out[n++] = kD2[2 * fr]; out[n++] = kD2[2 * fr + 1];
    return n;
}

void expand_slots(const HostPlanes& hp, int Lp, int64_t P, int64_t PS, uint32_t* istat, float* fstat) {
    const int64_t CH = 1 << 16;
    const int64_t nch = (PS + CH - 1) / CH;
    std::atomic<int64_t> next(0);
    auto work = [&]() {
        for (;;) {
            const int64_t ci = next.fetch_add(1);
            if (ci >= nch) break;
            const int64_t k0 = ci * CH, k1 = std::min(PS, k0 + CH);
            for (int l = 0; l < Lp; ++l) {
                for (int b = 0; b < NBUCKET; ++b) {
                    for (int f = 0; f < NI; ++f) memset(istat + (((int64_t)l * NBUCKET + b) * NI + f) * PS + k0, 0, (size_t)(k1 - k0) * 4);
                    for (int f = 0; f < NF; ++f) memset(fstat + (((int64_t)l * NBUCKET + b) * NF + f) * PS + k0, 0, (size_t)(k1 - k0) * 4);
                }
                const uint32_t* sid = hp.slotid + (int64_t)l * PS;
                for (int sl = 0; sl < 2; ++sl) {
                    for (int f = 0; f < NI; ++f) {
                        const uint32_t* src = hp.si + (((int64_t)l * 2 + sl) * NI + f) * PS;
                        for (int64_t k = k0; k < std::min(P, k1); ++k) {
                            const uint32_t b = (sid[k] >> (8 * sl)) & 0xffu;
                            if (b < (uint32_t)NBUCKET && src[k]) istat[(((int64_t)l * NBUCKET + b) * NI + f) * PS + k] = src[k];
                        }
                    }
                    for (int f = 0; f < NF; ++f) {
                        const float* src = hp.sf + (((int64_t)l * 2 + sl) * NF + f) * PS;
                        for (int64_t k = k0; k < std::min(P, k1); ++k) {
                            const uint32_t b = (sid[k] >> (8 * sl)) & 0xffu;
                            if (b < (uint32_t)NBUCKET) fstat[(((int64_t)l * NBUCKET + b) * NF + f) * PS + k] = src[k];
                        }
                    }
                }
            }
        }
    };
    unsigned nt = effective_cpus(); if (nt > 32) nt = 32; if (nt < 1) nt = 1;
    if (nch < (int64_t)nt) nt = (unsigned)nch;
    std::vector<std::thread> th;
    for (unsigned t = 1; t < nt; ++t) th.emplace_back(work);
// ... 197 lines not shown
}

extern "C" {

const char* brc_strerror(int code) {
    switch (code) {
        case BRC_OK: return "ok";
        case BRC_E_ARG: return "bad argument or call order";
        case BRC_E_NODEVICE: return "no HIP device / kernels unavailable (the engine has no CPU fallback)";
        case BRC_E_HIP: return "HIP runtime error";
        case BRC_E_NOMEM: return "out of memory";
        case BRC_E_LIMIT: return "engine limit exceeded";
        default: return "unknown error";
    }
}
const char* brc_last_error(const brc_engine* e) { return e ? e->err.c_str() : ""; }
const char* brc_kernel_name(int k) { return (k >= 0 && k < BRC_NKERNEL) ? backend_kernel_name(k) : NULL; }
const char* brc_engine_kind(void) { return backend_kind(); }

int brc_create(const brc_config* cfg, brc_engine** out) {
    if (!cfg || !out || cfg->abi_version != BRC_ABI_VERSION) return BRC_E_ARG;
    if (cfg->per_lib && (cfg->n_libs < 0 || (cfg->n_libs > 0 && !cfg->lib_names) || cfg->n_libs > 254)) return BRC_E_ARG;
    if (cfg->per_lib) for (int i = 0; i < cfg->n_libs; ++i) {
        if (!cfg->lib_names[i]) return BRC_E_ARG;
        if (i && strcmp(cfg->lib_names[i - 1], cfg->lib_names[i]) >= 0) return BRC_E_ARG;
    }
    brc_engine* e = new (std::nothrow) brc_engine();
    if (!e) return BRC_E_NOMEM;
    e->cfg = *cfg;
    if (e->cfg.max_cnt <= 0) e->cfg.max_cnt = 10000000;
    if (cfg->per_lib) for (int i = 0; i < cfg->n_libs; ++i) e->libs.push_back(cfg->lib_names[i]);
    e->cfg.lib_names = NULL;
    e->g.Lp = cfg->per_lib ? (cfg->n_libs > 0 ? cfg->n_libs : 1) : 1;
    int err = BRC_OK;
    e->be.reset(make_backend(e->cfg, &err));
    if (!e->be) { delete e; return err ? err : BRC_E_NODEVICE; }
    e->st.init(e->be->host_alloc());
    e->queue.resize((size_t)e->g.Lp);
    *out = e;
    return BRC_OK;
}

void brc_destroy(brc_engine* e) {
    if (!e) return;
    if (getenv("BRC_ENGINE_TIMING"))
        fprintf(stderr, "engine timing (%lld regions): push %.3f s, upload %.3f s, compute %.3f s, download %.3f s, assemble %.3f s, format %.3f s (of which waiting for the device text %.3f s); third-allele events %llu, indel buckets %llu\n",
                (long long)e->n_regions, e->t_push, e->t_upload, e->t_compute, e->t_d2h, e->t_post, e->t_format, e->t_textwait, (unsigned long long)e->n_xev_total, (unsigned long long)e->n_indel_total);
    e->st.destroy();
    delete e;
}

int brc_set_chrom(brc_engine* e, const char* chrom) {
    if (!e || !chrom) return BRC_E_ARG;
    e->chrom = chrom;
    return BRC_OK;
}

int brc_set_option(brc_engine* e, int option, int64_t value) {
    if (!e) return BRC_E_ARG;
    switch (option) {
        case BRC_OPT_TEXT_ONLY: e->text_only = value != 0; return BRC_OK;
        case BRC_OPT_EXPECT_READS: e->hint_reads = value > 0 ? (size_t)std::min<int64_t>(value, (int64_t)1 << 31) : 0; return BRC_OK;
        case BRC_OPT_EXPECT_BASES: e->hint_bases = value > 0 ? (size_t)std::min<int64_t>(value, (int64_t)1 << 36) : 0; return BRC_OK;
        case BRC_OPT_DEVICE_TEXT: e->device_text = value != 0; return BRC_OK;
        case BRC_OPT_CONTINUES_PREVIOUS: e->continues = value == 1; e->warn_skip_lead = value == 1 || value == 2; return BRC_OK;
        case BRC_OPT_FORMAT_THREADS: e->format_threads = value > 0 ? (unsigned)std::min<int64_t>(value, 1024) : 0u; return BRC_OK;
        case BRC_OPT_MAX_COUNT: if (value < INT32_MIN || value > INT32_MAX) return fail(e, BRC_E_ARG, "max count out of range"); e->cfg.max_cnt = (int32_t)value; return BRC_OK;
        case BRC_OPT_EXPECT_TEXT: { if (value <= 0) return BRC_OK; const int rc = e->be->reserve_text((size_t)value); return rc ? fail(e, rc, e->be->last_error()) : BRC_OK; }
        default: return fail(e, BRC_E_ARG, "unknown engine option");
    }
}

int brc_begin_region(brc_engine* e, int32_t tid, int32_t beg0, int32_t end, const char* ref, int64_t ref_len) {
    if (!e) return BRC_E_ARG;
    if (beg0 < 0 || end < beg0 || (ref && ref_len < 0)) return fail(e, BRC_E_ARG, "bad region");
    e->st.clear();
    e->g.tid = tid; e->g.beg0 = beg0; e->g.end = end; e->g.ref = ref; e->g.ref_len = ref ? ref_len : 0;
    e->g.P = 0; e->g.pos0 = 0;
    e->accepted = 0; e->n_ext = 0; e->last_acc_pos = 0; e->last_pos = INT32_MIN; e->heap_built = false;
    while (!e->live_ends.empty()) e->live_ends.pop();
    e->state = 1;
    return BRC_OK;
}

}

static inline int32_t cigar_rlen(const uint32_t* cig, uint32_t nc, uint64_t* n_indel_ops) {
    int64_t l = 0;
    for (uint32_t k = 0; k < nc; ++k) {
        const uint32_t op = cig[k] & 0xfu;
        if (is_refop(op)) l += (int64_t)(cig[k] >> 4);
        if (op == CINS || op == CDEL || op == CPAD) ++*n_indel_ops;
    }
    return l > INT32_MAX ? -1 : (int32_t)l;
}

static const char* const kEmptyM = "a mapped read has an empty M/=/X CIGAR operator behind its last base (the reference would read past the read's qualities)";
struct Chunk {
    uint64_t bq = 0, idp = 0, np = 0;
    int32_t max_lq = 0; int64_t max_span = 0, min_pos = INT64_MAX, max_end = INT64_MIN, n_ext = 0, acc = 0;
    int32_t last_acc_pos = 0; bool empty_m = false, eqx = false;
    int err = 0; const char* msg = nullptr;
    uint32_t hist[TABLE_MAX + 1];
    Chunk() { memset(hist, 0, sizeof hist); }
};
struct PushCtx { brc_engine* e; const brc_read_batch* b; size_t n0; uint64_t cb, sb, qb; };

template <class Admit>
static inline bool stage_read(const PushCtx& x, size_t i, int32_t prev, Chunk& C, Admit admit) {
    brc_engine* const e = x.e; Staged& s = e->st; const brc_read_batch* const b = x.b;
    auto bad = [&](int code, const char* m) { C.err = code; C.msg = m; return false; };
    const size_t r = x.n0 + i;
    uint32_t nc = s.n_cigar.p[r];
    const int32_t lq = s.l_qseq.p[r];
    if (b->cigar_off[i] + nc > b->n_cigar_total || b->qual_off[i] + (uint64_t)(lq > 0 ? lq : 0) > b->qual_bytes ||
        b->seq_off[i] + (uint64_t)((lq + 1) / 2) > b->seq_bytes || lq < 0) return bad(BRC_E_ARG, "read offsets outside the batch arenas");
    if (e->cfg.per_lib && s.lib.p[r] >= e->g.Lp) return bad(BRC_E_ARG, "library index out of range");
    s.cig_off.p[r] += x.cb; s.seq_off.p[r] += x.sb; s.qual_off.p[r] += x.qb;
    const uint64_t rowlen = ((uint64_t)lq + 15u) & ~(uint64_t)15u;
    s.bq_row.p[r] = rowlen; C.bq += rowlen;
    if (lq <= TABLE_MAX) C.hist[lq]++;
    if (lq >= (1 << 22)) return bad(BRC_E_LIMIT, "reads of 4 Mbases and more are not supported");
    if (lq > C.max_lq) C.max_lq = lq;
    const int32_t pos = s.pos.p[r];
    if (pos < prev) return bad(BRC_E_ARG, "reads are not coordinate-sorted");
    uint16_t fl = (uint16_t)(s.flag.p[r] & 0x7fffu);
    const uint32_t* const cg = s.cigar.p + s.cig_off.p[r];
    if (lq > 0 && nc > 0) {
        int64_t ql = 0; bool empty_m = false, eqx = false;
        for (uint32_t k = 0; k < nc; ++k) { const uint32_t op = cg[k] & 0xfu; if (op == CMATCH || op == CINS || op == CSOFT_CLIP || op == CEQUAL || op == CDIFF) ql += cg[k] >> 4; if (is_mop(op) && (cg[k] >> 4) == 0u) empty_m = true; if (op == CEQUAL || op == CDIFF) eqx = true; }
        if (ql != lq) {
            if (!(fl & FUNMAP)) return bad(BRC_E_ARG, "a read's CIGAR and sequence length disagree");
            nc = 0; s.n_cigar.p[r] = 0;
        } else if (empty_m && !(fl & FUNMAP)) C.empty_m = true;
        if (eqx) C.eqx = true;
    }
    uint64_t idp = 0;
    const int32_t rlen = cigar_rlen(cg, nc, &idp);
    if (rlen < 0 || (int64_t)pos + rlen > (int64_t)INT32_MAX) {
        if (!(fl & FUNMAP)) return bad(BRC_E_ARG, "a read ends beyond the last 32-bit position");
        nc = 0; s.n_cigar.p[r] = 0; idp = 0;
    }
    s.iev_off.p[r] = (uint32_t)idp; C.idp += idp;
    if (lq == 0 && nc > 0 && !(fl & (FUNMAP | BRC_NOCOUNT_MASK))) return bad(BRC_E_ARG, "a read without sequence would be counted");
    const int32_t end = (!(fl & FUNMAP) && nc > 0) ? pos + rlen : pos + 1;
    if (rlen > C.max_span) C.max_span = rlen;
    if (!(fl & FUNMAP) && pos >= 0) {
        if (pos < C.min_pos) C.min_pos = pos;
        if (end > C.max_end) C.max_end = end;
        C.n_ext++;
        if (admit(r, pos, end, C)) { C.acc++; C.last_acc_pos = pos; } else fl |= FHOSTDROP;
    }
    s.flag.p[r] = fl;
    const bool entered = read_enters(fl, cg, nc) && pos >= 0 && !(e->cfg.per_lib && s.lib.p[r] < 0);
    const bool counts = (int)s.mapq.p[r] >= e->cfg.min_mapq && !(fl & BRC_NOCOUNT_MASK);
    uint32_t np = 0; bool past = false;
    walk_pieces(e->cfg.insertion_centric != 0, entered, counts, pos, cg, nc, [&](int32_t, int32_t len, int32_t, int qoff, bool) { ++np; if (len > 0 && qoff + len > lq) past = true; });
    if (past) return bad(BRC_E_ARG, kEmptyM);
    s.piece_cnt.p[r] = np; C.np += np;
    s.wide.p[r] = read_has_escape(b->qual + b->qual_off[i], b->seq4 + b->seq_off[i], lq) ? 1 : 0;
    return true;
}
template <class Admit>
static void stage_chunk(const PushCtx& x, size_t i0, size_t i1, Chunk& C, Admit admit) {
    const Staged& s = x.e->st;
    for (size_t i = i0; i < i1; ++i) if (!stage_read(x, i, i == 0 ? x.e->last_pos : s.pos.p[x.n0 + i - 1], C, admit)) return;
}
static int merge_chunks(brc_engine* e, const Chunk* ch, size_t nch, uint64_t* bq0, uint64_t* idp0) {
    Staged& s = e->st;
    for (size_t ci = 0; ci < nch; ++ci) if (ch[ci].err) return fail(e, ch[ci].err, ch[ci].msg);
    for (size_t ci = 0; ci < nch; ++ci) {
        const Chunk& C = ch[ci];
        bq0[ci] = s.bq_elems; idp0[ci] = s.n_indel_ops;
        s.bq_elems += C.bq; s.n_indel_ops += C.idp;
        if ((uint64_t)(s.n_pieces += (int64_t)C.np) >= 0xFFFFFFF0ull) return fail(e, BRC_E_LIMIT, "more than 2^32 read segments in one region: split the region");
        for (int l = 0; l <= TABLE_MAX; ++l) s.len_hist[l] += C.hist[l];
        if (C.max_lq > s.max_lqseq) s.max_lqseq = C.max_lq;
        if (C.max_span > s.max_span) s.max_span = C.max_span;
        if (C.n_ext) {
            if (e->n_ext == 0) { s.min_pos = C.min_pos; s.max_end = C.max_end; }
            else { if (C.min_pos < s.min_pos) s.min_pos = C.min_pos; if (C.max_end > s.max_end) s.max_end = C.max_end; }
            e->n_ext += C.n_ext;
        }
        if (C.acc) { e->accepted += C.acc; e->last_acc_pos = C.last_acc_pos; }
        if (C.empty_m) s.has_empty_m = true;
        if (C.eqx) s.has_eqx = true;
    }
    return BRC_OK;
}
static void stage_offsets(Staged& s, size_t r0, size_t r1, uint64_t bq, uint64_t idp) {
    for (size_t r = r0; r < r1; ++r) {
        const uint64_t len = s.bq_row.p[r]; s.bq_row.p[r] = bq; bq += len;
        const uint32_t k = s.iev_off.p[r]; s.iev_off.p[r] = (uint32_t)idp; idp += k;
    }
}

static int push_reads_staged(brc_engine* e, const brc_read_batch* b, bool* touched, bool pinned) {
    if (e->state != 1) return fail(e, BRC_E_ARG, "brc_push_reads outside an open region");
    if (b->n_reads < 0) return fail(e, BRC_E_ARG, "negative n_reads");
    if (e->cfg.per_lib && !b->lib && b->n_reads) return fail(e, BRC_E_ARG, "per-library mode needs brc_read_batch.lib");
    Staged& s = e->st;
    const double t_in = now_s();
    struct Tm { brc_engine* e; double t0; ~Tm() { e->t_push += now_s() - t0; } } tm_{e, t_in};
    const size_t n = (size_t)b->n_reads, n0 = (size_t)s.n;
    if ((uint64_t)s.n + n >= 0xFFFFFFF0ull || s.cigar.n + b->n_cigar_total >= 0xFFFFFFF0ull)
        return fail(e, BRC_E_LIMIT, "more than 2^32 reads or CIGAR operators in one region: split the region");
    const bool adopt = pinned && e->be->adopts_arenas();
    if (s.n > 0 && adopt != s.adopted() && (s.seq_total || s.qual_total)) return fail(e, BRC_E_ARG, "a region takes brc_push_reads or brc_push_reads_pinned, not both");
    const PushCtx x = {e, b, n0, s.cigar.n, s.seq_total, s.qual_total};
    if (e->hint_reads > n0 + n || e->hint_bases > x.qb + b->qual_bytes) {
        const size_t hr = std::max(e->hint_reads, n0 + n) + 16, hb = std::max<size_t>(e->hint_bases, x.qb + b->qual_bytes) + 16;
        if (!(s.reserve_reads(hr, hr + hr / 4) && (adopt || (s.qual.reserve(hb) && s.seq4.reserve(hb / 2 + hr))))) return fail(e, BRC_E_NOMEM, "host staging allocation failed");
    }
    unsigned pthr = effective_cpus(); if (pthr > 8) pthr = 8;
    if (e->format_threads && e->format_threads < pthr) pthr = e->format_threads;
    const bool par = n >= 8192 && pthr > 1;
    if (par && !e->pool) e->pool.reset(new (std::nothrow) Pool(pthr - 1));
    Pool* const pool = par ? e->pool.get() : nullptr;
    *touched = true;
    bool ok = s.reserve_reads(n0 + n + 16, s.cigar.n + b->n_cigar_total + 16) &&
              s.pos.append(b->pos, n) && s.flag.append(b->flag, n) && s.mapq.append(b->mapq, n) && s.l_qseq.append(b->l_qseq, n) &&
              s.n_cigar.append(b->n_cigar, n) && s.cig_off.append(b->cigar_off, n) && s.seq_off.append(b->seq_off, n) &&
              s.qual_off.append(b->qual_off, n) && s.cigar.append(b->cigar, b->n_cigar_total) &&
              (adopt || (append_big(pool, s.seq4, b->seq4, b->seq_bytes) && append_big(pool, s.qual, b->qual, b->qual_bytes)));
    if (!ok) return fail(e, BRC_E_NOMEM, "host staging allocation failed");
    { uint32_t mx = s.max_ncigar; for (size_t i = 0; i < n; ++i) mx = b->n_cigar[i] > mx ? b->n_cigar[i] : mx; s.max_ncigar = mx; }
    if (adopt) {
        if (b->seq_bytes) { Staged::Seg g; g.p = b->seq4; g.off = x.sb; g.n = b->seq_bytes; s.seq_seg.push_back(g); }
        if (b->qual_bytes) { Staged::Seg g; g.p = b->qual; g.off = x.qb; g.n = b->qual_bytes; s.qual_seg.push_back(g); }
    }
    s.seq_total = x.sb + b->seq_bytes; s.qual_total = x.qb + b->qual_bytes;
    for (size_t i = 0; i < n; ++i) {
        uint64_t off = ~0ull;
        if (b->qname && b->qname[i]) { off = s.qnames.n; if (!s.qnames.append(b->qname[i], strlen(b->qname[i]) + 1)) return fail(e, BRC_E_NOMEM, "host staging allocation failed"); }
        s.qname_off.p[n0 + i] = off;
    }
    for (size_t i = 0; i < n; ++i) {
        s.lib.p[n0 + i] = (e->cfg.per_lib && b->lib) ? b->lib[i] : 0;
        s.nm.p[n0 + i] = b->nm ? b->nm[i] : 0;
        s.sm.p[n0 + i] = b->sm ? b->sm[i] : 0;
        s.tags.p[n0 + i] = b->tags ? b->tags[i] : 0;
    }
    s.qname_off.n = s.lib.n = s.nm.n = s.sm.n = s.tags.n = s.bq_row.n = s.wide.n = s.piece_cnt.n = s.iev_off.n = n0 + n;
    const int32_t maxcnt = e->cfg.max_cnt;
    if (pool && e->accepted + (int64_t)n < (int64_t)maxcnt && !e->heap_built) {
        const size_t CH = (n + (size_t)pool->size() * 4 - 1) / ((size_t)pool->size() * 4);
        const size_t nch = (n + CH - 1) / CH;
        std::vector<Chunk> ch(nch); std::vector<uint64_t> bq0(nch), idp0(nch);
        pool->run((int64_t)nch, [&](int64_t ci) { stage_chunk(x, (size_t)ci * CH, std::min(n, (size_t)ci * CH + CH), ch[(size_t)ci], [](size_t, int32_t, int32_t, const Chunk&) { return true; }); });
        const int rc = merge_chunks(e, ch.data(), nch, bq0.data(), idp0.data());
        if (rc) return rc;
        pool->run((int64_t)nch, [&](int64_t ci) { stage_offsets(s, n0 + (size_t)ci * CH, n0 + std::min(n, (size_t)ci * CH + CH), bq0[(size_t)ci], idp0[(size_t)ci]); });
    } else {
        Chunk C; uint64_t bq0 = 0, idp0 = 0;
        stage_chunk(x, 0, n, C, [&](size_t r, int32_t pos, int32_t end, const Chunk& c) {
            bool take = true;
            if (e->accepted + c.acc >= maxcnt) {
                if (!e->heap_built) {
                    uint64_t dummy = 0;
                    for (size_t j = 0; j < r; ++j) {
                        if (s.flag.p[j] & BRC_PUSH_MASK) continue;
                        const int32_t rl = cigar_rlen(s.cigar.p + s.cig_off.p[j], s.n_cigar.p[j], &dummy);
                        e->live_ends.push(s.n_cigar.p[j] > 0 ? s.pos.p[j] + rl : s.pos.p[j] + 1);
                    }
                    e->heap_built = true;
                }
                while (!e->live_ends.empty() && e->live_ends.top() < pos) e->live_ends.pop();
                take = !(pos == (c.acc ? c.last_acc_pos : e->last_acc_pos) && (int64_t)e->live_ends.size() + 1 > (int64_t)maxcnt);
            }
            if (take && e->heap_built) e->live_ends.push(end);
            return take;
        });
        const int rc = merge_chunks(e, &C, 1, &bq0, &idp0);
        if (rc) return rc;
        stage_offsets(s, n0, n0 + n, bq0, idp0);
    }
    if (n) e->last_pos = s.pos.p[n0 + n - 1];
    s.n += (int64_t)n;
    return BRC_OK;
}

static int push_reads_any(brc_engine* e, const brc_read_batch* b, bool pinned) {
    if (!e || !b) return BRC_E_ARG;
    bool touched = false;
    int rc;
    try { rc = push_reads_staged(e, b, &touched, pinned); }
    catch (const std::bad_alloc&) { touched = true; rc = fail(e, BRC_E_NOMEM, "host allocation failed while staging reads"); }
    catch (const std::exception& ex) { touched = true; rc = fail(e, BRC_E_NOMEM, ex.what()); }
    catch (...) { touched = true; rc = fail(e, BRC_E_NOMEM, "unexpected failure while staging reads"); }
    if (rc != BRC_OK && touched) e->state = 0;
    return rc;
}

extern "C" {

void* brc_host_alloc(size_t bytes) { return backend_host_alloc(bytes); }
void brc_host_free(void* p) { if (p) backend_host_free(p); }
int brc_push_reads(brc_engine* e, const brc_read_batch* b) { return push_reads_any(e, b, false); }
int brc_push_reads_pinned(brc_engine* e, const brc_read_batch* b) { return push_reads_any(e, b, true); }

int brc_upload(brc_engine* e) {
    if (!e) return BRC_E_ARG;
    if (e->state != 1) return fail(e, BRC_E_ARG, "brc_upload needs an open region");
    const double t_in = now_s();
    Geometry& g = e->g; const Staged& s = e->st;
    int64_t lo = g.beg0 > 0 ? g.beg0 - 1 : 0, hi = g.end;
    if (e->n_ext == 0) { hi = lo; }
    else { if (s.min_pos > lo) lo = s.min_pos; if (s.max_end < hi) hi = s.max_end; if (hi < lo) hi = lo; }
    g.pos0 = (int32_t)lo; g.P = hi - lo;
    g.ref_lo = g.ref_hi = 0;
    if (g.ref && e->n_ext) {
        g.ref_lo = std::min<int64_t>(std::max<int64_t>(s.min_pos, 0), g.ref_len);
        g.ref_hi = std::min<int64_t>(std::max<int64_t>(s.max_end, g.ref_lo), g.ref_len);
    }
    e->st.layout_pieces(g.Lp, e->cfg.per_lib != 0);
    int rc = e->be->upload(e->cfg, s, g);
    if (rc) return fail(e, rc, e->be->last_error());
    e->state = 2; e->t_upload += now_s() - t_in; e->n_regions++;
    return BRC_OK;
}

static int compute_passes(brc_engine* e, int32_t n, brc_timing* t);
int brc_compute(brc_engine* e, brc_timing* t) { return compute_passes(e, 0, t); }
int brc_compute_n(brc_engine* e, int32_t n, brc_timing* t) {
    if (n < 1) return e ? fail(e, BRC_E_ARG, "brc_compute_n: at least one pass") : BRC_E_ARG;
    return compute_passes(e, n, t);
}
static int compute_passes(brc_engine* e, int32_t n, brc_timing* t) {
    if (!e) return BRC_E_ARG;
    if (e->state < 2) return fail(e, BRC_E_ARG, "brc_compute before brc_upload");
    const double t_in = now_s();
    int rc = n > 0 ? e->be->compute_n(n, t) : e->be->compute(t);
    if (rc) return fail(e, rc, e->be->last_error());
    uint64_t nx_ = 0, ni_ = 0; e->be->list_sizes(&nx_, &ni_);
    e->text_computed = e->text_only && e->device_text && !e->chrom.empty() &&
                       (double)e->g.P * (double)e->g.Lp * 700.0 + 64.0 * (double)e->g.P + 2.0 * (double)ni_ * (700.0 + (double)e->st.max_span) < 4.0e9;
    if (e->text_computed) {
        rc = e->be->text_begin(e->chrom, e->libs, &e->text_slot_computed);
        if (rc == BRC_TEXT_TOO_LONG) e->text_computed = false;
        else if (rc) return fail(e, rc, e->be->last_error());
    }
    e->state = 3; e->t_compute += now_s() - t_in;
    return BRC_OK;
}

static void fill_refbase(const Geometry& g, int64_t pos0, int64_t n, std::vector<char>& out) {
    out.resize((size_t)n + 1);
    const int64_t have = g.ref ? std::max<int64_t>(0, std::min<int64_t>(n, g.ref_len - pos0)) : 0;
    if (have) memcpy(out.data(), g.ref + pos0, (size_t)have);
    for (int64_t k = 0; k < have; ++k) if (!out[(size_t)k]) out[(size_t)k] = 'N';
    if (n > have) memset(out.data() + have, 'N', (size_t)(n - have));
}
static int expand_dense(brc_engine* e, DenseResult& d, const HostPlanes& hp, int64_t n, int64_t stride) {
    if (!d.ensure((size_t)e->g.Lp * NBUCKET * (size_t)stride + 16)) return fail(e, BRC_E_NOMEM, "host allocation of the dense planes failed");
    expand_slots(hp, e->g.Lp, n, stride, d.i, d.f);
    return BRC_OK;
}
static void fill_result(const brc_engine* e, brc_result* out, int32_t beg0, int32_t end, int32_t pos0, int64_t n, int64_t stride, const HostPlanes& hp, const DenseResult& d) {
    memset(out, 0, sizeof *out);
    out->tid = e->g.tid; out->beg0 = beg0; out->end = end; out->pos0 = pos0; out->n_pos = n; out->stride = stride; out->n_lib = e->g.Lp;
    out->ncol = hp.ncol; out->depth = hp.depth; out->istat = d.i; out->fstat = d.f;
    out->unavail = e->cfg.per_lib ? hp.unavail : NULL;
    out->refbase = d.refbase.data();
    out->n_indel = (int64_t)d.indels.size(); out->indel = d.indels.data();
    out->alleles = d.alleles.data(); out->alleles_len = d.alleles.size();
}

int brc_fetch_result(brc_engine* e, brc_result* out) {
    if (!e || !out) return BRC_E_ARG;
    if (e->state < 3) return fail(e, BRC_E_ARG, "brc_fetch_result before brc_compute");
    const double t_in = now_s();
    e->text_result = e->text_computed; e->text_slot = e->text_slot_computed;
    int rc = e->be->fetch(&e->hp, !e->text_result);
    if (rc) return fail(e, rc, e->be->last_error());
    const double t_dl = now_s(); e->t_d2h += t_dl - t_in;
    e->n_xev_total += e->hp.n_xagg; e->n_indel_total += (uint64_t)e->hp.n_indel;
    const Geometry& g = e->g; const HostPlanes& hp = e->hp; DenseResult& d = e->res;
    if (e->text_result) {
        d.indels.clear(); d.alleles.clear(); prepare_text_queues(e);
    } else {
        fill_refbase(g, g.pos0, g.P, d.refbase);
        assemble_indels(e, hp.indel, hp.n_indel, d);
        if (e->text_only) {
            e->xagg.clear(); e->xagg.reserve((size_t)hp.n_xagg);
            for (uint64_t i = 0; i < hp.n_xagg; ++i) {
                const XAgg& x = hp.xagg[i];
                if ((int64_t)(x.lib_b >> 8) >= g.Lp || (x.lib_b & 0xffu) >= (uint32_t)NBUCKET || (int64_t)x.k >= g.P) continue;
                XKey a; a.key = ((uint64_t)x.k << 16) | (uint64_t)(x.lib_b & 0xffffu); a.st = stat_of(x);
                e->xagg.push_back(a);
            }
            std::sort(e->xagg.begin(), e->xagg.end(), [](const XKey& a, const XKey& b) { return a.key < b.key; });
        } else if ((rc = expand_dense(e, d, hp, g.P, g.PS)) != BRC_OK) return rc;
    }
    fill_result(e, out, g.beg0, g.end, g.pos0, g.P, g.PS, hp, d);
    if (e->text_only) { out->istat = NULL; out->fstat = NULL; }
    if (e->text_result) { out->ncol = out->depth = out->unavail = NULL; out->refbase = NULL; }
    out->n_events = hp.n_events;
    for (int w = 0; w < BRC_N_WARN; ++w) out->warn[w] = hp.warn[w];
    e->state = 4; e->t_post += now_s() - t_dl;
    return BRC_OK;
}

int brc_fetch_window(brc_engine* e, int32_t beg0, int32_t end, brc_result* out) {
    if (!e || !out) return BRC_E_ARG;
    if (e->state < 3) return fail(e, BRC_E_ARG, "brc_fetch_window before brc_compute");
    const Geometry& g = e->g;
    if (beg0 < g.beg0 || end > g.end || end < beg0) return fail(e, BRC_E_ARG, "brc_fetch_window: the window must lie inside the computed region");
    int64_t k0 = (int64_t)(beg0 > 0 ? beg0 - 1 : 0) - g.pos0, k1 = (int64_t)end - g.pos0;
    if (k0 < 0) k0 = 0;
    if (k0 > g.P) k0 = g.P;
    if (k1 > g.P) k1 = g.P;
    if (k1 < k0) k1 = k0;
    const int64_t n = k1 - k0;
    HostPlanes hw; int64_t WS = 0;
    int rc = e->be->fetch_window(k0, n, &hw, &WS);
    if (rc) return fail(e, rc, e->be->last_error());
    const int32_t wpos0 = (int32_t)(g.pos0 + k0);
    e->win_xagg.clear(); e->win_iout.clear();
    for (uint64_t i = 0; i < hw.n_xagg; ++i) { const XAgg& x = hw.xagg[i]; if ((int64_t)x.k >= k0 && (int64_t)x.k < k1) { XAgg y = x; y.k = (uint32_t)((int64_t)x.k - k0); e->win_xagg.push_back(y); } }
    for (int64_t i = 0; i < hw.n_indel; ++i) { const IndelOut& o = hw.indel[i]; if (o.pos >= wpos0 && (int64_t)o.pos < (int64_t)wpos0 + n) e->win_iout.push_back(o); }
    hw.xagg = e->win_xagg.data(); hw.n_xagg = e->win_xagg.size();
    DenseResult& d = e->win;
    assemble_indels(e, e->win_iout.data(), (int64_t)e->win_iout.size(), d);
    if ((rc = expand_dense(e, d, hw, n, WS)) != BRC_OK) return rc;
    fill_refbase(g, wpos0, n, d.refbase);
    fill_result(e, out, beg0, end, wpos0, n, WS, hw, d);
    uint64_t ev = 0;
    for (int l = 0; l < g.Lp; ++l) for (int64_t k = 0; k < n; ++k) {
        if ((int64_t)wpos0 + k < (int64_t)beg0) continue;
        if (e->cfg.per_lib && hw.unavail && hw.unavail[k] != 0xFFFFFFFFu) continue;
        ev += hw.ncol[(int64_t)l * WS + k];
    }
    out->n_events = ev;
    return BRC_OK;
}

int brc_end_region(brc_engine* e, brc_result* out) {
    int rc = brc_upload(e);
    if (rc) return rc;
    rc = brc_compute(e, NULL);
    if (rc) return rc;
    return brc_fetch_result(e, out);
}

int brc_region_counts(brc_engine* e, uint64_t* n_events, uint64_t* n_positions) {
    if (!e) return BRC_E_ARG;
    if (e->state < 3) return fail(e, BRC_E_ARG, "brc_region_counts before brc_compute");
    int rc = e->be->counts(n_events, n_positions);
    if (rc) return fail(e, rc, e->be->last_error());
    return BRC_OK;
}

int brc_region_piece_steps(brc_engine* e, uint64_t* ranged, uint64_t* walked) {
    if (!e || !ranged || !walked) return BRC_E_ARG;
    if (e->state < 3) return fail(e, BRC_E_ARG, "brc_region_piece_steps before brc_compute");
    e->be->piece_steps(ranged, walked);
    return BRC_OK;
}

int brc_device_view_get(brc_engine* e, brc_device_view* out) {
    if (!e || !out) return BRC_E_ARG;
    if (e->state < 3) return fail(e, BRC_E_ARG, "brc_device_view_get before brc_compute");
    brc_device_view v; memset(&v, 0, sizeof v);
    const int rc = e->be->device_view(&v);
    if (rc) return fail(e, rc, e->be->last_error());
    const Geometry& g = e->g;
    v.n_lib = g.Lp; v.pos0 = g.pos0; v.n_pos = g.P; v.stride = g.PS;
    if (!e->cfg.per_lib) v.unavail = NULL;
// ... 564 lines not shown
```

bam_readcount_amd/csrc/brc_host.h:

```cpp
#ifndef BRC_HOST_H
#define BRC_HOST_H

#include <stddef.h>
#include <stdint.h>
#include <string.h>

#include <string>
#include <vector>

#include "../../include/brc.h"
#include "brc_core.h"

namespace brc {

struct HostAlloc {
    void* (*alloc)(size_t bytes);
    void (*release)(void* p);
};

template <class T>
struct HBuf {
    T* p = nullptr;
    size_t n = 0, cap = 0;
    const HostAlloc* A = nullptr;
    bool reserve(size_t want) {
        if (want <= cap) return true;
        size_t c = cap ? 2 * cap : (size_t)(1u << 16);
        if (c < want) c = want + want / 8;
        T* q = (T*)A->alloc(c * sizeof(T));
        if (!q) return false;
        if (n) memcpy(q, p, n * sizeof(T));
        if (p) A->release(p);
        p = q; cap = c;
        return true;
    }
    bool append(const T* src, size_t k) {
        if (!reserve(n + k + 16)) return false;
        if (k) memcpy(p + n, src, k * sizeof(T));
        n += k;
        return true;
    }
    void clear() { n = 0; }
    void destroy() { if (p) A->release(p); p = nullptr; n = cap = 0; }
};

struct Staged {
    HBuf<int32_t> pos; HBuf<uint16_t> flag; HBuf<uint8_t> mapq; HBuf<int16_t> lib; HBuf<int32_t> l_qseq;
    HBuf<uint32_t> n_cigar; HBuf<uint64_t> cig_off, seq_off, qual_off; HBuf<int32_t> nm, sm; HBuf<uint8_t> tags;
    HBuf<uint32_t> cigar; HBuf<uint8_t> seq4, qual;
    struct Seg { const uint8_t* p; uint64_t off, n; };
    std::vector<Seg> seq_seg, qual_seg;
    uint64_t seq_total = 0, qual_total = 0;
    bool adopted() const { return !seq_seg.empty() || !qual_seg.empty(); }
    static const uint8_t* seg_at(const std::vector<Seg>& v, uint64_t off) {
        size_t lo = 0, hi = v.size();
        while (hi - lo > 1) { const size_t mid = (lo + hi) / 2; if (v[mid].off <= off) lo = mid; else hi = mid; }
        return v[lo].p + (off - v[lo].off);
    }
    const uint8_t* seq_at(uint64_t off) const { return seq_seg.empty() ? seq4.p + off : seg_at(seq_seg, off); }
    const uint8_t* qual_at(uint64_t off) const { return qual_seg.empty() ? qual.p + off : seg_at(qual_seg, off); }
    HBuf<uint64_t> bq_row;
    uint64_t bq_elems = 0;
    HBuf<uint8_t> wide;
    struct WidePair { uint32_t read, w16; };
    uint64_t wide_layout(WidePair* pairs , uint32_t first16) const;
    size_t n_wide() const { size_t k = 0; for (int64_t i = 0; i < n; ++i) k += wide.p[i] != 0; return k; }
    HBuf<char> qnames; HBuf<uint64_t> qname_off;
    HBuf<uint32_t> piece_cnt, piece_off;
    HBuf<uint32_t> iev_off;
    std::vector<int64_t> lib_base;
    int64_t n_pieces = 0;
    int32_t max_lqseq = 0;
    uint32_t max_ncigar = 0;
    bool has_eqx = false;
    bool has_empty_m = false;
    int64_t max_span = 0;
    void layout_pieces(int Lp, bool per_lib);
    uint32_t len_hist[TABLE_MAX + 1] = {0};
    int32_t modal_len() const { uint32_t best = 0; int32_t arg = 0; for (int l = 1; l <= TABLE_MAX; ++l) if (len_hist[l] > best) { best = len_hist[l]; arg = l; } return arg; }
    int64_t n = 0;
    int64_t min_pos = 0, max_end = 0;
    uint64_t n_indel_ops = 0;
    std::vector<int32_t> win_beg, win_end;
    std::vector<uint16_t> wanted_tiles(int32_t pos0, int64_t P) const;
    template <class F> void each_read_buf(F f) {
        f(pos); f(flag); f(mapq); f(lib); f(l_qseq); f(n_cigar); f(cig_off); f(seq_off); f(qual_off); f(nm); f(sm); f(tags);
        f(bq_row); f(wide); f(piece_cnt); f(piece_off); f(iev_off); f(qname_off);
    }
    template <class F> void each_buf(F f) { each_read_buf(f); f(cigar); f(seq4); f(qual); f(qnames); }
    bool reserve_reads(size_t reads, size_t cigar_ops);
    void init(const HostAlloc* A);
    void clear();
    void destroy();
};

struct Geometry {
    int32_t tid = 0, beg0 = 0, end = 0;
    int32_t pos0 = 0; int64_t P = 0; int Lp = 1;
    int64_t PS = 0;
    const char* ref = nullptr; int64_t ref_len = 0;
    int64_t ref_lo = 0, ref_hi = 0;
};

struct HostPlanes {
    uint32_t *ncol = nullptr, *depth = nullptr, *slotid = nullptr, *si = nullptr, *unavail = nullptr;
    float* sf = nullptr;
    const XAgg* xagg = nullptr; uint64_t n_xagg = 0;
    const IndelOut* indel = nullptr; int64_t n_indel = 0;
    uint64_t n_events = 0, n_positions = 0;
    uint64_t warn[BRC_N_WARN] = {0, 0, 0, 0};
};

struct HostText { const char* text = nullptr; const uint32_t* off = nullptr; uint64_t total = 0; int64_t n = 0;
                  const uint32_t* last_processed = nullptr; };

enum { BRC_TEXT_TOO_LONG = 1000 };

class Backend {
  public:
    virtual ~Backend() {}
    virtual const HostAlloc* host_alloc() = 0;
    virtual bool adopts_arenas() const { return false; }
    virtual int upload(const brc_config& cfg, const Staged& s, Geometry& g) = 0;
    virtual int compute(brc_timing* t) = 0;
    virtual int compute_n(int n, brc_timing* t) {
        brc_timing acc; memset(&acc, 0, sizeof acc);
        for (int i = 0; i < n; ++i) { brc_timing one; memset(&one, 0, sizeof one); const int rc = compute(&one); if (rc) return rc; for (int k = 0; k < BRC_NKERNEL; ++k) acc.ms[k] += one.ms[k]; acc.total_ms += one.total_ms; }
        if (t && n > 0) { for (int k = 0; k < BRC_NKERNEL; ++k) t->ms[k] = acc.ms[k] / (float)n; t->total_ms = acc.total_ms / (float)n; }
        return BRC_OK;
    }
    virtual int fetch(HostPlanes* out, bool planes) = 0;
    virtual int fetch_window(int64_t k0, int64_t n, HostPlanes* out, int64_t* stride) = 0;
    virtual int text_begin(const std::string& chrom, const std::vector<std::string>& libs, int* slot) = 0;
    virtual int text_wait(int slot, HostText* out) = 0;
    virtual int reserve_text(size_t) { return BRC_OK; }
    virtual void list_sizes(uint64_t* n_xev, uint64_t* n_indel_slots) { *n_xev = 0; *n_indel_slots = 0; }
    virtual int device_view(brc_device_view* out) {
        HostPlanes hp;
        const int rc = fetch(&hp, true); if (rc) return rc;
        out->memory = BRC_MEM_HOST; out->device = 0;
        out->ncol = hp.ncol; out->depth = hp.depth; out->slotid = hp.slotid; out->si = hp.si; out->sf = hp.sf; out->unavail = hp.unavail;
        out->xagg = hp.xagg; out->n_xagg = hp.n_xagg;
        return BRC_OK;
    }
    virtual int device_indels(const Staged& s, const Geometry& g, brc_device_indels* out) {
        HostPlanes hp;
        const int rc = fetch(&hp, false); if (rc) return rc;
        out->memory = BRC_MEM_HOST; out->device = 0;
        out->slots = hp.n_indel ? hp.indel : nullptr; out->n_slots = (uint64_t)hp.n_indel;
        out->seq4 = s.seq4.p; out->seq_off = s.seq_off.p; out->l_qseq = s.l_qseq.p; out->n_reads = s.n;
        out->ref = g.ref ? g.ref + g.ref_lo : nullptr;
        return BRC_OK;
    }
    virtual int counts(uint64_t* n_events, uint64_t* n_positions) = 0;
    virtual void piece_steps(uint64_t* ranged, uint64_t* walked) { *ranged = 0; *walked = 0; }
    virtual const char* last_error() const = 0;
};

Backend* make_backend(const brc_config& cfg, int* err);
void* backend_host_alloc(size_t bytes);
void backend_host_free(void* p);
const char* backend_kind();
const char* backend_kernel_name(int k);

void expand_slots(const HostPlanes& hp, int Lp, int64_t P, int64_t PS, uint32_t* istat, float* fstat);

unsigned effective_cpus();

enum TestKnob { TK_NO_TABLE = 0, TK_FLUSH_K, TK_PACK_LIM, TK_FORCE_DOM, TK_IBUCKET_SHIFT, TK_XEV_CAP, TK_DEVICE_TEXT_LIMIT, TK_FORMAT_THREADS, TK_FORMAT_CHUNK, TK_COMPACT, TK_WAVE_FORM, TK_N };
const char* test_knob(int which);

int fmt_f2(char* out, float v);
int fmt_u32(char* out, uint32_t v);

}
#endif
```

Before: 346.1 billion.

## Split annotation into per-class kernels via separate annotator library

Reads are classified on the host into general, uniform-length simple and other simple lists, and a separate annotator library launches specialised wave-per-64-reads kernels for the simple single-match reads. These kernels cooperatively fetch quality, sequence and reference bytes in 8-base groups and compute mismatch runs across lanes. The aim is to replace the thread-per-read annotate kernel for the common case with coalesced wave-level work. It adds host classification passes, extra list uploads and a fallback path when the library declines a region.

```diff
diff --git a/bam_readcount_amd/capi.py b/bam_readcount_amd/capi.py
--- a/bam_readcount_amd/capi.py
+++ b/bam_readcount_amd/capi.py
@@ -863,3 +863,44 @@
 
     def last_timing(self):
         return super().last_timing()
+
+
+ANNOT_LIB = os.path.join(HERE, "csrc", "libbrc_annot_hip.so")
+ANNOT_LIB_CHECKED = os.path.join(HERE, "csrc", "libbrc_annot_hip_checked.so")
+ANNOT_EXPORTS = ["brc_annot_kind", "brc_annot_region", "brc_annot_simple", "brc_annot_general", "brc_annot_last_counts"]
+ANNOT_COUNTS = ("uniform", "other", "general", "declined")
+
+
+class AnnotBufs(C.Structure):
+    _fields_ = [("reads", C.c_void_p), ("piece_off", C.c_void_p), ("pieces", C.c_void_p), ("rare", C.c_void_p), ("keyreach", C.c_void_p),
+                ("eb", C.c_void_p), ("ev_raw", C.c_void_p), ("bucket_cnt", C.c_void_p), ("refcode", C.c_void_p), ("wanted", C.c_void_p)]
+
+
+class Annot:
+
+    PROTOS = {"brc_annot_kind": (C.c_char_p, []),
+              "brc_annot_region": (C.c_int, [C.c_void_p, C.c_size_t, C.c_size_t]),
+              "brc_annot_simple": (C.c_int, [C.c_void_p, C.c_size_t, C.c_void_p, C.c_size_t, C.POINTER(AnnotBufs), C.c_void_p, C.c_uint32, C.c_int32, C.c_void_p]),
+              "brc_annot_general": (C.c_int, [C.c_void_p, C.c_size_t, C.c_void_p, C.c_size_t, C.POINTER(AnnotBufs), C.c_void_p, C.c_uint32, C.c_void_p]),
+              "brc_annot_last_counts": (None, [C.POINTER(C.c_uint64 * 4)])}
+
+    def __init__(self, path=None):
+        path = path or ANNOT_LIB
+        if not os.path.exists(path):
+            raise BrcError("annotator library not found: %s (run `python __graft_entry__.py` / build() first)" % path)
+        self.path = path
+        self.lib = L = _load(path)
+        for s in ANNOT_EXPORTS:
+            if not hasattr(L, s):
+                raise BrcError("%s does not export %s" % (path, s))
+        for name, (restype, argtypes) in self.PROTOS.items():
+            f = getattr(L, name)
+            f.restype = restype; f.argtypes = argtypes
+
+    def kind(self):
+        return self.lib.brc_annot_kind().decode()
+
+    def last_counts(self):
+        out = (C.c_uint64 * 4)()
+        self.lib.brc_annot_last_counts(C.byref(out))
+        return dict(zip(ANNOT_COUNTS, (int(x) for x in out)))
diff --git a/bam_readcount_amd/csrc/brc_annot.hip b/bam_readcount_amd/csrc/brc_annot.hip
--- /dev/null
+++ b/bam_readcount_amd/csrc/brc_annot.hip
@@ -0,0 +1,555 @@
+#include <hip/hip_runtime.h>
+#include <atomic>
+
+#include <stdint.h>
+#include <string.h>
+
+#include "../../include/brc_annot.h"
+#include "brc_annot_core.h"
+
+namespace brc {
+
+enum { REFCODE_PAD = BRC_ANNOT_REFCODE_PAD };
+
+struct RunCarry { bool open; uint32_t t; int jr; };
+__device__ __forceinline__ void grp_mismatch_runs(int lane, int jr, bool act, uint2 mm, uint2 Q, uint32_t* sum, RunCarry& cy) {
+    const bool has_mm = (mm.x | mm.y) != 0u;
+    const int nbits = __builtin_popcount(mm.x) + __builtin_popcount(mm.y);
+    const bool bit0 = (mm.x & 0x80u) != 0u, bit7 = (mm.y & 0x80000000u) != 0u;
+    const int pjr = lane_shr1(jr); const int pb7 = lane_shr1(bit7 ? 1 : 0);
+    const bool link = bit0 && (lane ? (pjr == jr && pb7 != 0) : (cy.open && cy.jr == jr));
+    if (cy.open && lane == 0 && !link) atomicAdd(&sum[cy.jr], cy.t);
+    const unsigned long long any_mm = __ballot(has_mm);
+    uint32_t t_out = 0u;
+    if (any_mm) {
+        const int nlink = lane_shl1(link ? 1 : 0);
+        const unsigned long long hard = __ballot(has_mm && (nbits > 1 || link || (bit7 && (lane == 63 || nlink != 0))));
+        if (!hard) {
+            if (has_mm) {
+                const int k = mm.x ? (__builtin_ctz(mm.x) >> 3) : 4 + (__builtin_ctz(mm.y) >> 3);
+                const uint32_t qv = ((k < 4 ? Q.x : Q.y) >> ((k & 3) << 3)) & 0xffu;
+                atomicAdd(&sum[jr], qv);
+            }
+        } else {
+            const unsigned long long m64 = (unsigned long long)mm.x | ((unsigned long long)mm.y << 32);
+            const unsigned long long q64 = (unsigned long long)Q.x | ((unsigned long long)Q.y << 32);
+            const bool full = nbits == 8;
+            uint32_t t_own = 0u; { bool open = false; uint32_t cur = 0u;
+                _Pragma("unroll") for (int k = 0; k < 8; ++k) { const bool m = (m64 >> (8 * k + 7)) & 1ull; const uint32_t qv = (uint32_t)(q64 >> (8 * k)) & 0xffu;
+                    if (m) { cur = open ? (cur > qv ? cur : qv) : qv; open = true; } else open = false; }
+                t_own = open ? cur : 0u; }
+            uint32_t t = t_own;
+            for (;;) {
+                uint32_t pt = (uint32_t)lane_shr1((int)t);
+                if (lane == 0) pt = cy.t;
+                const uint32_t nt = (full && link) ? (t_own > pt ? t_own : pt) : t_own;
+                const bool ch = nt != t; t = nt;
+                if (!__ballot(ch)) break;
+            }
+            uint32_t pt = (uint32_t)lane_shr1((int)t);
+            if (lane == 0) pt = cy.t;
+            uint32_t add = 0u; { bool open = link; uint32_t cur = link ? pt : 0u;
+                _Pragma("unroll") for (int k = 0; k < 8; ++k) { const bool m = (m64 >> (8 * k + 7)) & 1ull; const uint32_t qv = (uint32_t)(q64 >> (8 * k)) & 0xffu;
+                    if (m) { cur = open ? (cur > qv ? cur : qv) : qv; open = true; } else { if (open) add += cur; open = false; } }
+                if (open) { if (lane < 63 && !nlink) add += cur; else t_out = cur; } }
+            if (has_mm || link) { if (add) atomicAdd(&sum[jr], add); }
+            if (lane < 63) t_out = 0u;
+        }
+    }
+    cy.open = __builtin_amdgcn_readlane((bit7 && act) ? 1 : 0, 63) != 0;
+    cy.t = (uint32_t)__builtin_amdgcn_readlane((int)t_out, 63);
+    cy.jr = __builtin_amdgcn_readlane(jr, 63);
+}
+
+__device__ __forceinline__ int q2_scan(const uint8_t* q, int32_t L, bool rev, bool have_w0, unsigned long long w0) {
+    int found = -1;
+    if (rev) {
+        for (int k = 0; k < L && found < 0; k += 8) {
+            unsigned long long w; const int nv = L - k < 8 ? L - k : 8;
+            if (k == 0 && have_w0) w = w0; else if (nv == 8) __builtin_memcpy(&w, q + k, 8); else { w = 0x0202020202020202ull; for (int j = 0; j < nv; ++j) w = (w & ~(0xffull << (8 * j))) | ((unsigned long long)q[k + j] << (8 * j)); }
+            const unsigned long long x = w ^ 0x0202020202020202ull;
+            if (x) found = k + (__builtin_ctzll(x) >> 3);
+        }
+    } else {
+        for (int k = L; k > 0 && found < 0; k -= 8) {
+            unsigned long long w; const int lo8 = k - 8;
+            if (k == L && have_w0) w = w0; else if (lo8 >= 0) __builtin_memcpy(&w, q + lo8, 8); else { w = 0x0202020202020202ull; for (int j = 0; j < k; ++j) w = (w & ~(0xffull << (8 * (j - lo8)))) | ((unsigned long long)q[j] << (8 * (j - lo8))); }
+            const unsigned long long x = w ^ 0x0202020202020202ull;
+            if (x) found = lo8 + ((63 - __builtin_clzll(x)) >> 3);
+        }
+    }
+    return found;
+}
+
+typedef uint32_t u32x2s __attribute__((ext_vector_type(2)));
+typedef uint32_t u32x4s __attribute__((ext_vector_type(4)));
+
+template <bool UNIFORM, int SH>
+__global__ __launch_bounds__(256) void k_annot_simple(DevCfg c, DevIn in, const uint32_t* __restrict__ piece_off, Piece* __restrict__ pieces, PieceRare* __restrict__ rare,
+                                                      int2* __restrict__ keyreach, uint8_t* __restrict__ eb, const uint8_t* __restrict__ qual_ro, const uint8_t* __restrict__ seq_ro,
+                                                      const uint8_t* __restrict__ refcode, const uint32_t* __restrict__ list, uint32_t n_list,
+                                                      int32_t Lu, uint32_t Gu, uint32_t magic ) {
+    c.pack_shift = SH;
+    struct WaveLds { uint4 a[64]; uint4 b[64]; uint32_t sum[64]; uint32_t redo[64]; uint32_t wide[64]; unsigned long long mark; };
+    __shared__ WaveLds lds_all[4];
+    const int lane = threadIdx.x & 63;
+    const uint32_t wv = __builtin_amdgcn_readfirstlane((uint32_t)threadIdx.x >> 6);
+    WaveLds& W = lds_all[wv];
+    const uint32_t rb = (blockIdx.x * 4u + wv) * 64u;
+    if (rb >= n_list) return;
+    const int nrd = (int)((n_list - rb) < 64u ? (n_list - rb) : 64u);
+    const bool have = lane < nrd;
+    const int64_t my = (int64_t)list[rb + (uint32_t)(have ? lane : nrd - 1)];
+    const int32_t pos = in.pos[my];
+    const uint32_t flag = in.flag[my];
+    const int32_t L = in.l_qseq[my];
+    const uint64_t qoff = in.qual_off[my], soff = in.seq_off[my], brow = in.bq_row[my];
+    const int64_t d1 = (int64_t)pos - c.ref_lo;
+    const uint64_t qbase = wave_min_u64(qoff), sbase = wave_min_u64(soff);
+    const bool odd = d1 < -(int64_t)L || d1 > 0x7fff0000ll || qoff - qbase > 0xff000000ull || soff - sbase > 0xff000000ull || L <= 0 || (UNIFORM && L != Lu);
+    const bool serial_wave = __ballot(odd) != 0ull;
+    if (!serial_wave) {
+        if (have) {
+            W.a[lane] = make_uint4((uint32_t)(qoff - qbase), (uint32_t)(soff - sbase), (uint32_t)brow, (uint32_t)(brow >> 32));
+            W.b[lane].x = (uint32_t)(int32_t)d1; W.b[lane].y = (uint32_t)L;
+        }
+        W.sum[lane] = 0u; W.redo[lane] = 0u; W.wide[lane] = 0u;
+        uint32_t T, g_me = 0u, S_me = 0u;
+        if (UNIFORM) T = (uint32_t)nrd * Gu;
+        else {
+            g_me = have ? ((uint32_t)L + 7u) >> 3 : 0u;
+            uint32_t incl = g_me;
+#pragma unroll
+            for (int d = 1; d < 64; d <<= 1) { const uint32_t o = (uint32_t)__shfl_up((int)incl, d, 64); if (lane >= d) incl += o; }
+            T = (uint32_t)__builtin_amdgcn_readlane((int)incl, 63);
+            S_me = incl - g_me;
+            if (have) W.b[lane].z = S_me;
+        }
+        __builtin_amdgcn_fence(__ATOMIC_SEQ_CST, "wavefront");
+
+        int jbefore = -1;
+        RunCarry cy = {false, 0u, -1};
+        const int64_t ref_n = c.ref_hi - c.ref_lo;
+        const uint8_t* const qwave = qual_ro + qbase; const uint8_t* const swave = seq_ro + sbase; const uint8_t* const refpad = refcode - REFCODE_PAD;
+        struct Fetch { int jr; int32_t b; uint2 Q; uint32_t S; uint2 R1; };
+        auto fetch = [&](uint32_t base) -> Fetch {
+            Fetch F;
+            const uint32_t G = base + (uint32_t)lane;
+            if (UNIFORM) {
+                const uint32_t q = annot_group_div(G, Gu, magic);
+                F.jr = G < T ? (int)q : nrd - 1;
+                F.b = G < T ? (int32_t)((G - q * Gu) << 3) : 0;
+            } else {
+                if (lane == 0) __hip_atomic_store(&W.mark, 0ull, __ATOMIC_RELAXED, __HIP_MEMORY_SCOPE_WAVEFRONT);
+                __builtin_amdgcn_fence(__ATOMIC_SEQ_CST, "wavefront");
+                { const uint32_t d = S_me - base; if (g_me && d < 64u) __hip_atomic_fetch_or(&W.mark, 1ull << d, __ATOMIC_RELAXED, __HIP_MEMORY_SCOPE_WAVEFRONT); }
+                __builtin_amdgcn_fence(__ATOMIC_SEQ_CST, "wavefront");
+                unsigned long long M = __hip_atomic_load(&W.mark, __ATOMIC_RELAXED, __HIP_MEMORY_SCOPE_WAVEFRONT);
+                M = (unsigned long long)(uint32_t)__builtin_amdgcn_readfirstlane((int)(uint32_t)M) | ((unsigned long long)(uint32_t)__builtin_amdgcn_readfirstlane((int)(uint32_t)(M >> 32)) << 32);
+                const int below = (int)__builtin_amdgcn_mbcnt_hi((uint32_t)(M >> 32), __builtin_amdgcn_mbcnt_lo((uint32_t)M, 0u));
+                F.jr = jbefore + below + (int)((M >> lane) & 1ull);
+                jbefore += __builtin_popcountll(M);
+                F.b = G < T ? (int32_t)((G - W.b[F.jr].z) << 3) : 0;
+            }
+            const uint4 Pa = W.a[F.jr];
+            __builtin_memcpy(&F.Q, BRC_CK(c, CK_ANNOTATE, 2, CB_QUAL, qwave + (uint32_t)(Pa.x + (uint32_t)F.b), 8, rb + F.jr, F.b), 8);
+            __builtin_memcpy(&F.S, BRC_CK(c, CK_ANNOTATE, 3, CB_SEQ, swave + (uint32_t)(Pa.y + ((uint32_t)F.b >> 1)), 4, rb + F.jr, F.b), 4);
+            int64_t r1off = (int64_t)F.b + (int32_t)W.b[F.jr].x;
+            if (r1off < -8 || r1off > ref_n) r1off = 0;
+            __builtin_memcpy(&F.R1, BRC_CK(c, CK_ANNOTATE, 4, CB_REFCODE, refpad + (uint32_t)((int32_t)r1off + REFCODE_PAD), 8, rb + F.jr, F.b), 8);
+            return F;
+        };
+        Fetch Fn = fetch(0u);
+        for (uint32_t base = 0; base < T; base += 64u) {
+            const Fetch F = Fn;
+            if (base + 64u < T) Fn = fetch(base + 64u);
+            const int jr = F.jr;
+            const bool act = base + (uint32_t)lane < T;
+            const uint4 Pa = W.a[jr];
+            const int32_t b = F.b;
+            const int32_t Lr = UNIFORM ? Lu : (int32_t)W.b[jr].y;
+            const int nv = act ? (Lr - b < 8 ? Lr - b : 8) : 0;
+            const uint2 Q = F.Q; const uint32_t S = F.S; const uint2 R1 = F.R1;
+            const unsigned long long vflags = (nv >= 8 ? ~0ull : ((1ull << (8 * nv)) - 1ull)) & 0x8080808080808080ull;
+            const uint32_t Ev = (S >> 4) & 0x0f0f0f0fu, Od = S & 0x0f0f0f0fu;
+            uint2 N;
+            N.x = __builtin_amdgcn_perm(Od, Ev, 0x05010400u);
+            N.y = __builtin_amdgcn_perm(Od, Ev, 0x07030602u);
+            uint2 mm;
+            const uint32_t rx = R1.x & 0x0f0f0f0fu, ry = R1.y & 0x0f0f0f0fu;
+            mm.x = nzb7(N.x ^ rx) & nzb7(rx ^ 0x0f0f0f0fu) & nzb7(N.x) & (uint32_t)vflags;
+            mm.y = nzb7(N.y ^ ry) & nzb7(ry ^ 0x0f0f0f0fu) & nzb7(N.y) & (uint32_t)(vflags >> 32);
+            const uint32_t nul = (R1.x & (uint32_t)vflags) | (R1.y & (uint32_t)(vflags >> 32));
+            if (act) {
+                uint32_t ex, ey;
+                uint2 E; E.x = grp_ev_bytes(Q.x, grp_index_of(N.x), (uint32_t)vflags, ex); E.y = grp_ev_bytes(Q.y, grp_index_of(N.y), (uint32_t)(vflags >> 32), ey);
+                if (ex | ey) { grp_escape(c, Q, ex, ey, E); atomicOr(&W.wide[jr], 1u); }
+                u32x2s* dst = reinterpret_cast<u32x2s*>(BRC_CK(c, CK_ANNOTATE, 7, CB_EB, eb + ((((uint64_t)Pa.w) << 32) | (uint64_t)Pa.z) + (uint32_t)b, 8, rb + jr, b));
+                const u32x2s val = {E.x, E.y};
+                __builtin_nontemporal_store(val, dst);
+            }
+            if (nul & 0x80808080u) atomicOr(&W.redo[jr], 1u);
+            grp_mismatch_runs(lane, jr, act, mm, Q, W.sum, cy);
+        }
+        if (cy.open && lane == 0) atomicAdd(&W.sum[cy.jr], cy.t);
+        __builtin_amdgcn_fence(__ATOMIC_SEQ_CST, "wavefront");
+    }
+    if (!have) return;
+    const uint32_t mapq_l = in.mapq[my], tags_l = in.tags[my];
+    const bool rev = (flag & FREVERSE) != 0;
+    const bool serial = serial_wave || W.redo[lane] != 0u;
+    const bool q2_pre = !serial_wave && L >= 8;
+    unsigned long long q2_w0 = 0ull;
+    if (q2_pre) __builtin_memcpy(&q2_w0, BRC_CK(c, CK_ANNOTATE, 8, CB_QUAL, qual_ro + qoff + (rev ? 0 : L - 8), 8, my, -1), 8);
+    bool wide = !serial_wave && W.wide[lane] != 0u;
+    DRead r;
+    if (serial) {
+        r = annotate_read(c, in, my, eb, nullptr, wide);
+    } else {
+        const int found = q2_scan(BRC_CK(c, CK_ANNOTATE, 9, CB_QUAL, qual_ro + qoff, (uint64_t)L, my, -1), L, rev, q2_pre, q2_w0);
+        int tp, q2 = found >= 0 ? found - 1 : -1;
+        if (rev) { tp = 0; if (tp < q2) tp = q2; }
+        else { tp = L - 1; if (tp > q2 && q2 != -1) tp = q2; }
+        r.pos = pos; r.end = pos + L;
+        r.cig_off = 0u; r.n_cigar = 1u; r.bq_off = brow;
+        uint32_t misc = (mapq_l << 8) | (1u << 16) | M_SIMPLE | M_STAGED;
+        if (rev) misc |= M_REV;
+        if (flag & BRC_NOCOUNT_MASK) misc |= M_NOCOUNT;
+        if (q2 > -1) misc |= M_Q2OK;
+        uint32_t sse;
+        if (flag & FPROPER_PAIR) { if (tags_l & 2u) sse = (uint32_t)in.sm[my]; else { sse = 0; misc |= M_SMW; } } else sse = mapq_l;
+        float snm = 0.0f;
+        if (tags_l & 1u) snm = (float)in.nm[my] / (float)L; else misc |= M_NMW;
+        r.misc = finish_misc(misc, c.table_len > 0 && L == c.table_len, false); r.l_qseq = L; r.q2 = q2; r.tp = tp; r.left = 0; r.clipped = L;
+        r.zm_sum = W.sum[lane]; r.sse_add = sse; r.snm_add = snm; r.clipped_dup = L;
+    }
+    {
+        struct Cig1 { uint32_t c0; __device__ __forceinline__ uint32_t operator()(uint32_t) const { return c0; } } cig1;
+        cig1.c0 = ((uint32_t)L << 4) | (uint32_t)CMATCH;
+        const ReadConst rc = read_const(c, r, (uint32_t)my, wide);
+        uint32_t slot = piece_off[my];
+        walk_pieces_at(c.insertion_centric != 0, r.end > r.pos && pos >= 0, rc.counts, pos, cig1, 1u, [&](int32_t rs, int32_t len, int32_t ext, int qoff_, bool nb) {
+            Piece h; PieceRare rr;
+            make_piece(c, rc, rs, len, ext, qoff_, nb, h, rr, SH);
+            Piece* const pdst = BRC_CK(c, CK_ANNOTATE, 12, CB_PIECES, pieces + slot, sizeof(Piece), my, slot);
+            const u32x4s* hs = reinterpret_cast<const u32x4s*>(&h); u32x4s* hd = reinterpret_cast<u32x4s*>(pdst);
+            __builtin_nontemporal_store(hs[0], hd); __builtin_nontemporal_store(hs[1], hd + 1); __builtin_nontemporal_store(hs[2], hd + 2);
+            if (piece_has_rare(piece_flags(h))) *BRC_CK(c, CK_ANNOTATE, 13, CB_RARE, rare + slot, sizeof(PieceRare), my, slot) = rr;
+            *BRC_CK(c, CK_ANNOTATE, 14, CB_KEYREACH, keyreach + slot, sizeof(int2), my, slot) = make_int2(pos, rs + ext);
+            ++slot;
+        });
+    }
+}
+
+struct AnnPar { uint4 a, b, c; };
+template <bool one_stream, int SH>
+__global__ __launch_bounds__(256) void k_annot_general(DevCfg c, DevIn in, DRead* __restrict__ reads, const uint32_t* __restrict__ piece_off,
+                                                       Piece* __restrict__ pieces, PieceRare* __restrict__ rare, int2* __restrict__ keyreach,
+                                                       uint8_t* __restrict__ eb, IndelEv* __restrict__ ev_raw, uint32_t* __restrict__ bucket_cnt,
+                                                       const uint32_t* __restrict__ cigar_ro, const uint8_t* __restrict__ qual_ro,
+                                                       const uint8_t* __restrict__ seq_ro, const uint8_t* __restrict__ refcode,
+                                                       const uint16_t* __restrict__ wanted ,
+                                                       const uint32_t* __restrict__ list, uint32_t n_list) {
+    c.pack_shift = SH;
+    struct WaveLds { AnnPar par[64]; uint32_t sum[64]; uint32_t redo[64]; uint32_t wide[64]; uint32_t G[64]; unsigned long long mark; };
+    __shared__ WaveLds lds_all[4];
+    const int lane = threadIdx.x & 63;
+    const uint32_t wv = __builtin_amdgcn_readfirstlane((uint32_t)threadIdx.x >> 6);
+    WaveLds& W = lds_all[wv];
+    const uint32_t rb = (blockIdx.x * 4u + wv) * 64u;
+    if (rb >= n_list) return;
+    const int nrd = (int)((n_list - rb) < 64u ? (n_list - rb) : 64u);
+    const bool have = lane < nrd;
+    const int64_t my = (int64_t)list[rb + (uint32_t)(have ? lane : nrd - 1)];
+    const int32_t pos = in.pos[my];
+    const uint32_t flag = in.flag[my];
+    const int32_t L = in.l_qseq[my];
+    const uint32_t nc = in.n_cigar[my];
+    const uint64_t qoff = in.qual_off[my], soff = in.seq_off[my], brow = in.bq_row[my];
+    const uint32_t coff = (uint32_t)in.cig_off[my];
+    int32_t rlen = 0; int clipped = L, left_clip = 0, right_clip = L; int64_t tot_d = 0, tot_is = 0;
+    uint32_t cig0 = 0, n_idp = 0;
+    CigShape shape;
+    int n_m = 0; int32_t m1lo = 0, m1hi = 0, m2lo = 0, m2hi = 0; int64_t d1 = 0, d2 = 0;
+    {
+        int rs = 0; int64_t x = pos;
+#ifdef BRC_CHECKED
+        const uint32_t* const cig_row = BRC_CK(c, CK_ANNOTATE, 1, CB_CIGAR, cigar_ro + coff, 4ull * nc, my, -1);
+#define BRC_CIG_AT(k) cig_row[k]
+#else
+#define BRC_CIG_AT(k) cigar_ro[coff + (k)]
+#endif
+        for (uint32_t k = 0; k < nc; ++k) {
+            const uint32_t cg = BRC_CIG_AT(k);
+            if (k == 0) cig0 = cg;
+            const uint32_t op = cg & 0xfu; const int len = (int)(cg >> 4);
+            shape_add(shape, op, len);
+            if (is_refop(op)) rlen += len;
+            if (op == CINS || op == CDEL || op == CPAD) ++n_idp;
+            if (op == CDEL || op == CREF_SKIP) tot_d += len;
+            if (op == CINS || op == CSOFT_CLIP) tot_is += len;
+            if (op == CSOFT_CLIP) { clipped -= len; if (k == 0) left_clip += len; else right_clip -= len; }
+            if (op == CMATCH) {
+                if (n_m == 0) { m1lo = rs; m1hi = rs + len; d1 = x - rs - c.ref_lo; }
+                else if (n_m == 1) { m2lo = rs; m2hi = rs + len; d2 = x - rs - c.ref_lo; }
+                ++n_m; rs += len; x += len;
+            } else if (op == CDEL || op == CREF_SKIP) x += len;
+            else if (op == CINS || op == CSOFT_CLIP) rs += len;
+        }
+#undef BRC_CIG_AT
+    }
+    const bool simple = nc == 1 && (cig0 & 0xfu) == CMATCH;
+    bool dropped = (flag & BRC_PUSH_MASK) != 0;
+    if (nc == 0) dropped = true;
+    if (nc == 1 && !is_mop(cig0 & 0xfu)) dropped = true;
+    if (m1hi > L) m1hi = L; if (m2hi > L) m2hi = L; if (m1lo > m1hi) m1lo = m1hi; if (m2lo > m2hi) m2lo = m2hi;
+    const uint64_t qbase = wave_min_u64(qoff), sbase = wave_min_u64(soff);
+    const bool fallback = !c.has_ref || pos < 0 || (int64_t)pos + rlen > c.ref_len || n_m > 2 ||
+                          d1 < -(int64_t)L || d2 < -(int64_t)L || d1 > 0x7fff0000ll || d2 > 0x7fff0000ll ||
+                          qoff - qbase > 0xff000000ull || soff - sbase > 0xff000000ull;
+    const bool work_me = have && !dropped && !fallback && L > 0;
+    const unsigned long long work = __ballot(work_me);
+    const int nd = __builtin_popcountll(work);
+    const int rank = (int)__builtin_amdgcn_mbcnt_hi((uint32_t)(work >> 32), __builtin_amdgcn_mbcnt_lo((uint32_t)work, 0u));
+    uint32_t T = 0;
+    if (nd) {
+        if (work_me) {
+            AnnPar p;
+            p.a = make_uint4((uint32_t)L, (uint32_t)(qoff - qbase), (uint32_t)(soff - sbase), (uint32_t)brow);
+            p.b = make_uint4(0u, (uint32_t)m1lo, (uint32_t)m1hi, (uint32_t)(int32_t)d1);
+            p.c = make_uint4((uint32_t)m2lo, (uint32_t)m2hi, (uint32_t)(int32_t)d2, (uint32_t)(brow >> 32));
+            W.par[rank] = p;
+            W.G[rank] = ((uint32_t)L + 7u) >> 3;
+        }
+        W.sum[lane] = 0u; W.redo[lane] = 0u; W.wide[lane] = 0u;
+        __builtin_amdgcn_fence(__ATOMIC_SEQ_CST, "wavefront");
+        const uint32_t g_me = lane < nd ? W.G[lane] : 0u;
+        uint32_t incl = g_me;
+#pragma unroll
+        for (int d = 1; d < 64; d <<= 1) { const uint32_t o = (uint32_t)__shfl_up((int)incl, d, 64); if (lane >= d) incl += o; }
+        T = (uint32_t)__builtin_amdgcn_readlane((int)incl, 63);
+        const uint32_t S_me = incl - g_me;
+        if (lane < nd) W.par[lane].b.x = S_me;
+        __builtin_amdgcn_fence(__ATOMIC_SEQ_CST, "wavefront");
+
+        int jbefore = -1;
+        RunCarry cy = {false, 0u, -1};
+        const int64_t ref_n = c.ref_hi - c.ref_lo;
+        const uint8_t* const qwave = qual_ro + qbase; const uint8_t* const swave = seq_ro + sbase; const uint8_t* const refpad = refcode - REFCODE_PAD;
+        struct Fetch { int jr; int32_t b; uint2 Q; uint32_t S; uint2 R1; };
+        auto fetch = [&](uint32_t base) -> Fetch {
+            Fetch F;
+            if (lane == 0) __hip_atomic_store(&W.mark, 0ull, __ATOMIC_RELAXED, __HIP_MEMORY_SCOPE_WAVEFRONT);
+            __builtin_amdgcn_fence(__ATOMIC_SEQ_CST, "wavefront");
+            { const uint32_t d = S_me - base; if (lane < nd && g_me && d < 64u) __hip_atomic_fetch_or(&W.mark, 1ull << d, __ATOMIC_RELAXED, __HIP_MEMORY_SCOPE_WAVEFRONT); }
+            __builtin_amdgcn_fence(__ATOMIC_SEQ_CST, "wavefront");
+            unsigned long long M = __hip_atomic_load(&W.mark, __ATOMIC_RELAXED, __HIP_MEMORY_SCOPE_WAVEFRONT);
+            M = (unsigned long long)(uint32_t)__builtin_amdgcn_readfirstlane((int)(uint32_t)M) | ((unsigned long long)(uint32_t)__builtin_amdgcn_readfirstlane((int)(uint32_t)(M >> 32)) << 32);
+            const int below = (int)__builtin_amdgcn_mbcnt_hi((uint32_t)(M >> 32), __builtin_amdgcn_mbcnt_lo((uint32_t)M, 0u));
+            F.jr = jbefore + below + (int)((M >> lane) & 1ull);
+            jbefore += __builtin_popcountll(M);
+            const uint32_t G = base + (uint32_t)lane;
+            const uint4 Pa = W.par[F.jr].a, Pb = W.par[F.jr].b;
+            F.b = G < T ? (int32_t)((G - Pb.x) << 3) : 0;
+            __builtin_memcpy(&F.Q, BRC_CK(c, CK_ANNOTATE, 2, CB_QUAL, qwave + (uint32_t)(Pa.y + (uint32_t)F.b), 8, rb + F.jr, F.b), 8);
+            __builtin_memcpy(&F.S, BRC_CK(c, CK_ANNOTATE, 3, CB_SEQ, swave + (uint32_t)(Pa.z + ((uint32_t)F.b >> 1)), 4, rb + F.jr, F.b), 4);
+            int64_t r1off = (int64_t)F.b + (int32_t)Pb.w;
+            if (r1off < -8 || r1off > ref_n) r1off = 0;
+            __builtin_memcpy(&F.R1, BRC_CK(c, CK_ANNOTATE, 4, CB_REFCODE, refpad + (uint32_t)((int32_t)r1off + REFCODE_PAD), 8, rb + F.jr, F.b), 8);
+            return F;
+        };
+        Fetch Fn = fetch(0u);
+        for (uint32_t base = 0; base < T; base += 64u) {
+            const Fetch F = Fn;
+            if (base + 64u < T) Fn = fetch(base + 64u);
+            const int jr = F.jr;
+            const uint32_t G = base + (uint32_t)lane;
+            const bool act = G < T;
+            const AnnPar P = W.par[jr];
+
+            const int32_t b = F.b;
+            const int32_t Lr = (int32_t)P.a.x;
+            const int nv = act ? (Lr - b < 8 ? Lr - b : 8) : 0;
+            const uint2 Q = F.Q; const uint32_t S = F.S; const uint2 R1 = F.R1;
+            const unsigned long long vflags = (nv >= 8 ? ~0ull : ((1ull << (8 * nv)) - 1ull)) & 0x8080808080808080ull;
+            unsigned long long f1 = vflags, f2 = 0ull;
+            const bool plain = (int32_t)P.b.y == 0 && (int32_t)P.b.z == Lr;
+            if (__ballot(act && !plain)) {
+                const int lo1 = (int32_t)P.b.y - b, hi1 = (int32_t)P.b.z - b;
+                const int a1 = lo1 < 0 ? 0 : (lo1 > 8 ? 8 : lo1), e1 = hi1 < 0 ? 0 : (hi1 > 8 ? 8 : hi1);
+                const unsigned long long below_e1 = e1 >= 8 ? ~0ull : ((1ull << (8 * e1)) - 1ull), below_a1 = a1 >= 8 ? ~0ull : ((1ull << (8 * a1)) - 1ull);
+                f1 = vflags & below_e1 & ~below_a1;
+                const int lo2 = (int32_t)P.c.x - b, hi2 = (int32_t)P.c.y - b;
+                const int a2 = lo2 < 0 ? 0 : (lo2 > 8 ? 8 : lo2), e2 = hi2 < 0 ? 0 : (hi2 > 8 ? 8 : hi2);
+                const unsigned long long below_e2 = e2 >= 8 ? ~0ull : ((1ull << (8 * e2)) - 1ull), below_a2 = a2 >= 8 ? ~0ull : ((1ull << (8 * a2)) - 1ull);
+                f2 = vflags & below_e2 & ~below_a2;
+            }
+            const uint32_t Ev = (S >> 4) & 0x0f0f0f0fu, Od = S & 0x0f0f0f0fu;
+            uint2 N;
+            N.x = __builtin_amdgcn_perm(Od, Ev, 0x05010400u);
+            N.y = __builtin_amdgcn_perm(Od, Ev, 0x07030602u);
+            uint2 mm; uint32_t nul;
+            {
+                const uint32_t rx = R1.x & 0x0f0f0f0fu, ry = R1.y & 0x0f0f0f0fu;
+                mm.x = nzb7(N.x ^ rx) & nzb7(rx ^ 0x0f0f0f0fu) & nzb7(N.x) & (uint32_t)f1;
+                mm.y = nzb7(N.y ^ ry) & nzb7(ry ^ 0x0f0f0f0fu) & nzb7(N.y) & (uint32_t)(f1 >> 32);
+                nul = (R1.x & (uint32_t)f1) | (R1.y & (uint32_t)(f1 >> 32));
+            }
+            if (__ballot(f2 != 0ull)) {
+                int64_t r2off = (int64_t)b + (int32_t)P.c.z;
+                if (!f2 || r2off < -8 || r2off > ref_n) r2off = 0;
+                uint2 R2; __builtin_memcpy(&R2, BRC_CK(c, CK_ANNOTATE, 5, CB_REFCODE, refpad + (uint32_t)((int32_t)r2off + REFCODE_PAD), 8, rb + jr, b), 8);
+                const uint32_t rx = R2.x & 0x0f0f0f0fu, ry = R2.y & 0x0f0f0f0fu;
+                mm.x |= nzb7(N.x ^ rx) & nzb7(rx ^ 0x0f0f0f0fu) & nzb7(N.x) & (uint32_t)f2;
+                mm.y |= nzb7(N.y ^ ry) & nzb7(ry ^ 0x0f0f0f0fu) & nzb7(N.y) & (uint32_t)(f2 >> 32);
+                nul |= (R2.x & (uint32_t)f2) | (R2.y & (uint32_t)(f2 >> 32));
+            }
+            if (act) {
+                uint32_t ex, ey;
+                uint2 E; E.x = grp_ev_bytes(Q.x, grp_index_of(N.x), (uint32_t)vflags, ex); E.y = grp_ev_bytes(Q.y, grp_index_of(N.y), (uint32_t)(vflags >> 32), ey);
+                if (ex | ey) { grp_escape(c, Q, ex, ey, E); atomicOr(&W.wide[jr], 1u); }
+                u32x2s* dst = reinterpret_cast<u32x2s*>(BRC_CK(c, CK_ANNOTATE, 7, CB_EB, eb + ((((uint64_t)P.c.w) << 32) | (uint64_t)P.a.w) + (uint32_t)b, 8, rb + jr, b));
+                const u32x2s val = {E.x, E.y};
+                if (one_stream) __builtin_nontemporal_store(val, dst); else *dst = val;
+            }
+            if (nul & 0x80808080u) atomicOr(&W.redo[jr], 1u);
+            grp_mismatch_runs(lane, jr, act, mm, Q, W.sum, cy);
+        }
+        if (cy.open && lane == 0) atomicAdd(&W.sum[cy.jr], cy.t);
+        __builtin_amdgcn_fence(__ATOMIC_SEQ_CST, "wavefront");
+    }
+    if (!have) return;
+    const uint32_t mapq_l = in.mapq[my], tags_l = in.tags[my];
+    const int lib_l = c.per_lib ? (int)in.lib[my] : 0;
+    const uint32_t cig1_l = nc > 1u ? cigar_ro[coff + 1u] : 0u, cig2_l = nc > 2u ? cigar_ro[coff + 2u] : 0u;
+    const bool q2_pre = work_me && L >= 8;
+    unsigned long long q2_w0 = 0ull;
+    if (q2_pre) __builtin_memcpy(&q2_w0, BRC_CK(c, CK_ANNOTATE, 8, CB_QUAL, qual_ro + qoff + ((flag & FREVERSE) ? 0 : L - 8), 8, my, -1), 8);
+    DRead r;
+    bool serial = fallback;
+    bool wide = work_me && W.wide[rank] != 0u;
+    uint32_t my_sum = 0; int my_hi = -1, my_lo = -1;
+    if (work_me && W.redo[rank]) serial = true;
+    if (work_me && !serial) {
+        my_sum = W.sum[rank];
+        const int found = q2_scan(BRC_CK(c, CK_ANNOTATE, 9, CB_QUAL, qual_ro + qoff, (uint64_t)L, my, -1), L, (flag & FREVERSE) != 0, q2_pre, q2_w0);
+        if (flag & FREVERSE) my_lo = found; else my_hi = found;
+    }
+    if (serial) {
+        r = annotate_read(c, in, my, eb, nullptr, wide);
+    } else {
+        const bool rev = (flag & FREVERSE) != 0;
+        int tp, q2;
+        if (rev) { tp = 0; if (tp < left_clip) tp = left_clip; q2 = my_lo >= 0 ? my_lo - 1 : -1; if (tp < q2) tp = q2; }
+        else { tp = L - 1; if (tp > right_clip) tp = right_clip; q2 = my_hi >= 0 ? my_hi - 1 : -1; if (tp > q2 && q2 != -1) tp = q2; }
+        const uint32_t mapq = mapq_l; const uint32_t tags = tags_l;
+        r.pos = pos; r.end = dropped ? pos : pos + rlen;
+        r.cig_off = coff; r.n_cigar = nc; r.bq_off = brow;
+        const int lib = lib_l;
+        uint32_t misc = (mapq << 8) | ((uint32_t)((lib + 1) & 0xff) << 16);
+        if (rev) misc |= M_REV;
+        if (flag & BRC_NOCOUNT_MASK) misc |= M_NOCOUNT;
+        if (q2 > -1) misc |= M_Q2OK;
+        if (simple) misc |= M_SIMPLE;
+        if (tot_d + tot_is <= STAGE_SLACK) misc |= M_STAGED | ((uint32_t)tot_d << 24);
+        uint32_t sse;
+        if (flag & FPROPER_PAIR) { if (tags & 2u) sse = (uint32_t)in.sm[my]; else { sse = 0; misc |= M_SMW; } } else sse = mapq;
+        float snm = 0.0f;
+        if (tags & 1u) snm = (float)in.nm[my] / (float)clipped; else misc |= M_NMW;
+        r.misc = finish_misc(misc, c.table_len > 0 && L == c.table_len && clipped == L, shape_clipm(shape, nc, left_clip)); r.l_qseq = L; r.q2 = q2; r.tp = tp; r.left = left_clip; r.clipped = clipped;
+        r.zm_sum = my_sum; r.sse_add = sse; r.snm_add = snm; r.clipped_dup = clipped;
+    }
+    if (nc >= 2u) *BRC_CK(c, CK_ANNOTATE, 10, CB_READS, reads + my, sizeof(DRead), my, -1) = r;
+    struct CigRegs {
+        uint32_t c0, c1, c2; const uint32_t* p;
+        __device__ __forceinline__ uint32_t operator()(uint32_t k) const { return k == 0u ? c0 : k == 1u ? c1 : k == 2u ? c2 : p[k]; }
+    } cigr;
+    cigr.p = BRC_CK(c, CK_ANNOTATE, 11, CB_CIGAR, cigar_ro + coff, 4ull * nc, my, -1); cigr.c0 = cig0;
+    cigr.c1 = cig1_l; cigr.c2 = cig2_l;
+    {
+        const bool nolib = c.per_lib && lib_l < 0;
+        const bool enters = r.end > r.pos && pos >= 0;
+        const ReadConst rc = read_const(c, r, (uint32_t)my, wide);
+        uint32_t slot = piece_off[my];
+        walk_pieces_at(c.insertion_centric != 0, enters && !nolib, rc.counts, pos, cigr, nc, [&](int32_t rs, int32_t len, int32_t ext, int qoff_, bool nb) {
+            Piece h; PieceRare rr;
+            make_piece(c, rc, rs, len, ext, qoff_, nb, h, rr, SH);
+            Piece* const pdst = BRC_CK(c, CK_ANNOTATE, 12, CB_PIECES, pieces + slot, sizeof(Piece), my, slot);
+            const u32x4s* hs = reinterpret_cast<const u32x4s*>(&h); u32x4s* hd = reinterpret_cast<u32x4s*>(pdst);
+            if (one_stream) { __builtin_nontemporal_store(hs[0], hd); __builtin_nontemporal_store(hs[1], hd + 1); __builtin_nontemporal_store(hs[2], hd + 2); }
+            else *pdst = h;
+            if (piece_has_rare(piece_flags(h))) *BRC_CK(c, CK_ANNOTATE, 13, CB_RARE, rare + slot, sizeof(PieceRare), my, slot) = rr;
+            *BRC_CK(c, CK_ANNOTATE, 14, CB_KEYREACH, keyreach + slot, sizeof(int2), my, slot) = make_int2(pos, rs + ext);
+            ++slot;
+        });
+    }
+    if (ev_raw && n_idp) {
+        const int lib = (int)((r.misc >> 16) & 0xffu) - 1;
+        IndelEv* slot = BRC_CK(c, CK_ANNOTATE, 15, CB_EVRAW, ev_raw + in.iev_off[my], sizeof(IndelEv) * (uint64_t)n_idp, my, -1); uint32_t used = 0;
+        enumerate_indels_at(c, cigr, r, qual_ro + qoff, [&](int32_t p, int qpos, int len) {
+            IndelEv e; e.read = (uint32_t)my; e.qpos = qpos; e.len = len; e.key_lo = (uint32_t)((int64_t)(p - c.pos0) * c.Lp + lib);
+            if (wanted && !tile_wants(*BRC_CK(c, CK_ANNOTATE, 16, CB_WANTED, wanted + ((uint32_t)(p - c.pos0) >> 6), 2, my, p), (uint32_t)(p - c.pos0) & 63u)) return;
+            if (used < n_idp) { slot[used++] = e; atomicAdd(BRC_CK(c, CK_ANNOTATE, 17, CB_CNT, bucket_cnt + indel_bucket_of(c, (uint32_t)(p - c.pos0), (uint32_t)lib), 4, my, p), 1u); }
+        });
+        for (; used < n_idp; ++used) slot[used].key_lo = NONE32;
+    }
+}
+
+static std::atomic<uint64_t> g_counts[4];
+
+}
+
+using namespace brc;
+
+extern "C" {
+
+const char* brc_annot_kind(void) {
+#ifdef BRC_CHECKED
+    return "hip-gfx950-checked";
+#else
+    return "hip-gfx950";
+#endif
+}
+
+int brc_annot_region(const void* cfg, size_t cfg_bytes, size_t in_bytes) {
+    for (auto& x : g_counts) x.store(0);
+    bool take = cfg && cfg_bytes == sizeof(DevCfg) && in_bytes == sizeof(DevIn);
+    if (take) { const DevCfg& c = *(const DevCfg*)cfg; take = c.has_ref && !c.per_lib && c.Lp == 1; }
+    if (!take) g_counts[BRC_ANNOT_N_DECLINED].store(1);
+    return take ? BRC_ANNOT_ENQUEUED : BRC_ANNOT_DECLINED;
+}
+
+int brc_annot_simple(const void* cfg, size_t cfg_bytes, const void* in, size_t in_bytes, const brc_annot_bufs* o,
+                     const uint32_t* list, uint32_t n, int32_t uniform_len, void* stream) {
+    if (!cfg || !in || !o || cfg_bytes != sizeof(DevCfg) || in_bytes != sizeof(DevIn) || uniform_len < 0 || uniform_len > TABLE_MAX) return BRC_ANNOT_DECLINED;
+    const DevCfg& c = *(const DevCfg*)cfg; const DevIn& di = *(const DevIn*)in;
+    if (!c.has_ref || c.per_lib || c.Lp != 1 || (c.pack_shift != 16 && c.pack_shift != 12)) return BRC_ANNOT_DECLINED;
+    g_counts[uniform_len ? BRC_ANNOT_N_UNIFORM : BRC_ANNOT_N_OTHER].store(n);
+    if (!n) return BRC_ANNOT_ENQUEUED;
+    const uint32_t Gu = ((uint32_t)uniform_len + 7u) >> 3, magic = annot_group_magic(Gu);
+    const dim3 grid((n + 255u) / 256u), block(256);
+    auto go = [&](auto k) {
+        hipLaunchKernelGGL(k, grid, block, 0, (hipStream_t)stream, c, di, o->piece_off, (Piece*)o->pieces, (PieceRare*)o->rare, (int2*)o->keyreach, o->eb,
+                           di.qual, di.seq4, o->refcode, list, n, uniform_len, Gu, magic);
+    };
+    if (uniform_len) { if (c.pack_shift == 16) go(k_annot_simple<true, 16>); else go(k_annot_simple<true, 12>); }
+    else { if (c.pack_shift == 16) go(k_annot_simple<false, 16>); else go(k_annot_simple<false, 12>); }
+    return BRC_ANNOT_ENQUEUED;
+}
+
+int brc_annot_general(const void* cfg, size_t cfg_bytes, const void* in, size_t in_bytes, const brc_annot_bufs* o,
+                      const uint32_t* list, uint32_t n, void* stream) {
+    if (!cfg || !in || !o || cfg_bytes != sizeof(DevCfg) || in_bytes != sizeof(DevIn)) return BRC_ANNOT_DECLINED;
+    const DevCfg& c = *(const DevCfg*)cfg; const DevIn& di = *(const DevIn*)in;
+    if (!c.has_ref || c.per_lib || c.Lp != 1 || (c.pack_shift != 16 && c.pack_shift != 12)) return BRC_ANNOT_DECLINED;
+    g_counts[BRC_ANNOT_N_GENERAL].store(n);
+    if (!n) return BRC_ANNOT_ENQUEUED;
+    const auto k = c.pack_shift == 16 ? k_annot_general<true, 16> : k_annot_general<true, 12>;
+    hipLaunchKernelGGL(k, dim3((n + 255u) / 256u), dim3(256), 0, (hipStream_t)stream, c, di, (DRead*)o->reads, o->piece_off, (Piece*)o->pieces, (PieceRare*)o->rare,
+                       (int2*)o->keyreach, o->eb, (IndelEv*)o->ev_raw, o->bucket_cnt, di.cigar, di.qual, di.seq4, o->refcode, o->wanted, list, n);
+    return BRC_ANNOT_ENQUEUED;
+}
+
+void brc_annot_last_counts(uint64_t out[4]) { for (int i = 0; i < 4; ++i) out[i] = g_counts[i].load(); }
+
+}
diff --git a/bam_readcount_amd/csrc/brc_annot_core.h b/bam_readcount_amd/csrc/brc_annot_core.h
--- /dev/null
+++ b/bam_readcount_amd/csrc/brc_annot_core.h
@@ -0,0 +1,52 @@
+#ifndef BRC_ANNOT_CORE_H
+#define BRC_ANNOT_CORE_H
+
+#include "brc_core.h"
+
+namespace brc {
+
+enum { ANNOT_DIV_X = 1 << 13, ANNOT_DIV_G = (TABLE_MAX + 7) / 8 };
+BRC_HD uint32_t annot_group_magic(uint32_t G) { return G > 1u ? (uint32_t)((0x100000000ull + G - 1u) / G) : 0u; }
+BRC_HD uint32_t annot_group_div(uint32_t x, uint32_t G, uint32_t magic) { return G > 1u ? (uint32_t)(((uint64_t)x * magic) >> 32) : x; }
+
+#if defined(__HIPCC__)
+__device__ __forceinline__ uint64_t wave_min_u64(uint64_t v) {
+#pragma unroll
+    for (int o = 32; o > 0; o >>= 1) {
+        const uint64_t u = ((uint64_t)(uint32_t)__shfl_xor((int)(uint32_t)(v >> 32), o, 64) << 32) | (uint64_t)(uint32_t)__shfl_xor((int)(uint32_t)v, o, 64);
+        v = u < v ? u : v;
+    }
+    return ((uint64_t)(uint32_t)__builtin_amdgcn_readfirstlane((int)(uint32_t)(v >> 32)) << 32) | (uint64_t)(uint32_t)__builtin_amdgcn_readfirstlane((int)(uint32_t)v);
+}
+__device__ __forceinline__ int lane_shr1(int v) { return __builtin_amdgcn_update_dpp(0, v, 0x138, 0xf, 0xf, false); }
+__device__ __forceinline__ int lane_shl1(int v) { return __builtin_amdgcn_update_dpp(0, v, 0x130, 0xf, 0xf, false); }
+__device__ __forceinline__ uint32_t nzb7(uint32_t x) { return x + 0x7f7f7f7fu; }
+
+__device__ __forceinline__ uint32_t grp_index_of(uint32_t codes) {
+    const uint32_t sx = codes & 0x07070707u;
+    const uint32_t lx = __builtin_amdgcn_perm(0x80808002u, 0x80010080u, sx), hx = __builtin_amdgcn_perm(0x80808080u, 0x80808003u, sx);
+    const uint32_t gx = (codes + 0x78787878u) & 0x80808080u;
+    const uint32_t mx = (gx - (gx >> 7)) | gx;
+    return (hx & mx) | (lx & ~mx);
+}
+__device__ __forceinline__ uint32_t grp_ev_bytes(uint32_t Qd, uint32_t Id, uint32_t valid7, uint32_t& esc7) {
+    const uint32_t qlo = Qd & 0x7f7f7f7fu, qhi = Qd & 0x80808080u;
+    const uint32_t q0 = ~(nzb7(qlo) | qhi), q63 = (qlo + 0x41414141u) | qhi;
+    esc7 = (Id | q0 | q63) & valid7;
+    return ((Qd & 0x3f3f3f3fu) << 2) | (Id & 0x03030303u);
+}
+__device__ __forceinline__ uint32_t grp_ge7(uint32_t x, uint32_t y) {
+    const uint32_t t = ((x | 0x80808080u) - (y & 0x7f7f7f7fu));
+    return ((x & ~y) | (~(x ^ y) & t)) & 0x80808080u;
+}
+__device__ __forceinline__ void grp_escape(const DevCfg& c, uint2 Q, uint32_t ex, uint32_t ey, uint2& E) {
+    const uint32_t mq = (uint32_t)(c.min_bq < 0 ? 0 : (c.min_bq > 255 ? 255 : c.min_bq)) * 0x01010101u;
+    const uint32_t none = c.min_bq > 255 ? 0u : 0xffffffffu;
+    const uint32_t px = ((grp_ge7(Q.x, mq) & none) >> 7) * 0xffu, py = ((grp_ge7(Q.y, mq) & none) >> 7) * 0xffu;
+    const uint32_t mx2 = (ex >> 7) * 0xffu, my3 = (ey >> 7) * 0xffu;
+    E.x = (E.x & ~mx2) | (mx2 & px & 0xfcfcfcfcu); E.y = (E.y & ~my3) | (my3 & py & 0xfcfcfcfcu);
+}
+#endif
+
+}
+#endif
diff --git a/bam_readcount_amd/csrc/brc_engine.hip b/bam_readcount_amd/csrc/brc_engine.hip
--- a/bam_readcount_amd/csrc/brc_engine.hip
+++ b/bam_readcount_amd/csrc/brc_engine.hip
@@ -2,6 +2,7 @@
 #include <atomic>
 #include <chrono>
 
+#include <dlfcn.h>
 #include <stdio.h>
 #include <stdlib.h>
 #include <string.h>
@@ -11,6 +12,7 @@
 #include <mutex>
 #include <vector>
 
+#include "../../include/brc_annot.h"
 #include "brc_host.h"
 
 namespace brc {
@@ -1884,6 +1886,34 @@
     (void)k;
 }
 
+static_assert(REFCODE_PAD == BRC_ANNOT_REFCODE_PAD, "the annotator library reads the engine's padded reference codes");
+struct AnnotLib {
+    decltype(&brc_annot_region) region = nullptr; decltype(&brc_annot_simple) simple = nullptr; decltype(&brc_annot_general) general = nullptr;
+    static const AnnotLib* get() {
+        static const AnnotLib lib = load();
+        return lib.region ? &lib : nullptr;
+    }
+  private:
+    static AnnotLib load() {
+        AnnotLib a;
+#ifdef BRC_CHECKED
+        static const char kName[] = "libbrc_annot_hip_checked.so";
+#else
+        static const char kName[] = "libbrc_annot_hip.so";
+#endif
+        Dl_info di;
+        if (!dladdr((const void*)&AnnotLib::load, &di) || !di.dli_fname) return a;
+        std::string path = di.dli_fname;
+        const size_t sl = path.rfind('/');
+        path = (sl == std::string::npos ? std::string() : path.substr(0, sl + 1)) + kName;
+        void* const h = dlopen(path.c_str(), RTLD_NOW | RTLD_LOCAL);
+        if (!h) return a;
+        a.region = (decltype(a.region))dlsym(h, "brc_annot_region"); a.simple = (decltype(a.simple))dlsym(h, "brc_annot_simple"); a.general = (decltype(a.general))dlsym(h, "brc_annot_general");
+        if (!a.region || !a.simple || !a.general) a.region = nullptr;
+        return a;
+    }
+};
+
 class HipBackend : public Backend {
     std::string err; int device = 0;
     DevCfg c; DevIn in;
@@ -1905,6 +1935,9 @@
     bool wave_huge = false;
     bool wave_eqx = false; uint32_t s_max_ncigar = 0;
     bool cursor_on = false;
+    const AnnotLib* annot = nullptr;
+    bool annot_take = false;
+    int32_t annot_len = 0; uint32_t n_ann_uniform = 0, n_ann_other = 0, n_ann_general = 0;
     unsigned long long h_steps[3] = {0, 0, 0};
     std::vector<XAgg> xagg_compact; std::vector<IndelOut> iout_compact;
     enum { XEV_SHARDS = 1024 }; size_t xev_cap = 0;
@@ -1922,6 +1955,7 @@
     DBuf<int32_t> d_pos, d_lq, d_nm, d_sm; DBuf<uint16_t> d_flag; DBuf<uint8_t> d_mapq, d_tags, d_seq, d_qual; DBuf<int16_t> d_lib;
     DBuf<uint32_t> d_nc, d_cigar, d_pieceoff, d_ievoff; DBuf<uint64_t> d_co, d_so, d_qo, d_bqrow; DBuf<char> d_ref; DBuf<uint8_t> d_refcode;
     DBuf<uint16_t> d_wanted; DBuf<uint32_t> d_tilelist; DBuf<uint2> d_wpairs; DBuf<int64_t> d_libbase;
+    DBuf<uint32_t> d_ann_uniform, d_ann_other, d_ann_general;
     DBuf<uint8_t> d_bq; DBuf<uint16_t> d_bqw; DBuf<Piece> d_pieces; DBuf<PieceRare> d_rare; DBuf<int2> d_keyreach; DBuf<DRead> d_reads;
     DBuf<uint32_t> d_wavelist, d_nc_k1; DBuf<unsigned long long> d_agg; DBuf<uint2> d_rng;
     DBuf<uint32_t> d_ccnt, d_coff; DBuf<Piece> d_cpieces; DBuf<PieceRare> d_crare; DBuf<uint2> d_crng; DBuf<unsigned long long> d_ctot;
@@ -1993,6 +2027,7 @@
         }
         for (Event& e : ev_text) HIPCHK(hipEventCreateWithFlags(&e.h, hipEventDisableTiming));
         HIPCHK(hipEventCreateWithFlags(&ev_lines.h, hipEventDisableTiming));
+        { const char* al = getenv("BRC_ANNOT_LIB"); annot = (al && !strcmp(al, "1")) ? AnnotLib::get() : nullptr; }
         return BRC_OK;
     }
     ~HipBackend() override {
@@ -2142,6 +2177,11 @@
             HIPCHK(hipMemsetD32Async((hipDeviceptr_t)d_slotid.p, (int)((uint32_t)NB_NONE | ((uint32_t)NB_NONE << 8)), Lp * P, stream));
             HIPCHK(hipMemsetAsync(d_tilectr.p, 0, (size_t)ntiles * Lp * sizeof(uint4), stream));
         }
+        annot_take = annot && n > 0 && annot->region(&c, sizeof c, sizeof in) == BRC_ANNOT_ENQUEUED;
+        if (annot_take) {
+            annot_len = s.modal_len(); n_ann_uniform = (uint32_t)s.ann_uniform.n; n_ann_other = (uint32_t)s.ann_other.n; n_ann_general = (uint32_t)s.ann_general.n;
+            if ((rc = up(d_ann_uniform, s.ann_uniform, s.ann_uniform.n)) || (rc = up(d_ann_other, s.ann_other, s.ann_other.n)) || (rc = up(d_ann_general, s.ann_general, s.ann_general.n))) return rc;
+        }
         HIPCHK(hipStreamSynchronize(stream));
         return BRC_OK;
     }
@@ -2156,6 +2196,15 @@
         const auto k = c.Lp == 1 ? by_pack(k_annotate_groups<true, 16>, k_annotate_groups<true, 12>) : by_pack(k_annotate_groups<false, 16>, k_annotate_groups<false, 12>);
         hipLaunchKernelGGL(k, dim3((unsigned)((c.n_reads + 255) / 256)), dim3(256), 0, stream, c, in_k1, d_reads.p, d_pieceoff.p, d_pieces.p, d_rare.p, d_keyreach.p,
                            eb_out(), evraw(), d_cnt.p, in.cigar, in.qual, in.seq4, refcode(), wanted());
+    }
+    int launch_annot_lib(const DevIn& in_k1) {
+        const brc_annot_bufs b = {d_reads.p, d_pieceoff.p, d_pieces.p, d_rare.p, d_keyreach.p, eb_out(), evraw(), d_cnt.p, refcode(), wanted()};
+        if (annot->general(&c, sizeof c, &in_k1, sizeof in_k1, &b, d_ann_general.p, n_ann_general, stream) != BRC_ANNOT_ENQUEUED) return 1;
+        if ((n_ann_uniform && annot->simple(&c, sizeof c, &in_k1, sizeof in_k1, &b, d_ann_uniform.p, n_ann_uniform, annot_len, stream) != BRC_ANNOT_ENQUEUED) ||
+            annot->simple(&c, sizeof c, &in_k1, sizeof in_k1, &b, d_ann_other.p, n_ann_other, 0, stream) != BRC_ANNOT_ENQUEUED) {
+            err = "the annotator library took the region and then declined a launch"; return BRC_E_HIP;
+        }
+        return BRC_OK;
     }
     template <int MCAP, int WAVES, bool EQX = false>
     void launch_annotate_wave(unsigned grid, const uint32_t* list, int step, const unsigned int* count) {
@@ -2212,7 +2261,11 @@
                                wave_on ? 1 : 0, cursor_on ? 1 : 0, &ctr->n_literal, &ctr->n_wave_eqx, &ctr->n_wave_eqx_big);
             in_k1.n_cigar = d_nc_k1.p;
         }
-        launch_annotate_groups(in_k1);
+        {
+            const int rc = annot_take ? launch_annot_lib(in_k1) : 1;
+            if (rc < 0) return rc;
+            if (rc) launch_annotate_groups(in_k1);
+        }
         if (wave_on) {
             const uint32_t* const wl = d_wavelist.p;
             const unsigned nb = (unsigned)std::min<int64_t>((n + 3) / 4, (int64_t)WAVE_FORM_BLOCKS), nb_big = (unsigned)std::min<int64_t>(n, (int64_t)WAVE_FORM_BLOCKS_BIG);
diff --git a/bam_readcount_amd/csrc/brc_host.cpp b/bam_readcount_amd/csrc/brc_host.cpp
--- a/bam_readcount_amd/csrc/brc_host.cpp
+++ b/bam_readcount_amd/csrc/brc_host.cpp
@@ -111,6 +111,17 @@
         }
     }
     return w;
+}
+bool Staged::layout_annot_lists() {
+    const int32_t L0 = modal_len();
+    size_t cnt[3] = {0, 0, 0};
+    auto cls = [&](int64_t i) { return ann_cls.p[i] == (uint8_t)ANNOT_GENERAL ? ANNOT_GENERAL : (l_qseq.p[i] == L0 ? ANNOT_SIMPLE_UNIFORM : ANNOT_SIMPLE_OTHER); };
+    for (int64_t i = 0; i < n; ++i) cnt[cls(i)]++;
+    if (!(ann_general.reserve(cnt[ANNOT_GENERAL] + 16) && ann_other.reserve(cnt[ANNOT_SIMPLE_OTHER] + 16) && ann_uniform.reserve(cnt[ANNOT_SIMPLE_UNIFORM] + 16))) return false;
+    HBuf<uint32_t>* const list[3] = {&ann_general, &ann_other, &ann_uniform};
+    for (auto* l : list) l->n = 0;
+    for (int64_t i = 0; i < n; ++i) { HBuf<uint32_t>& l = *list[cls(i)]; l.p[l.n++] = (uint32_t)i; }
+    return true;
 }
 void Staged::layout_pieces(int Lp, bool per_lib) {
     lib_base.assign((size_t)Lp + 1, 0);
@@ -614,6 +625,7 @@
         if (admit(r, pos, end, C)) { C.acc++; C.last_acc_pos = pos; } else fl |= FHOSTDROP;
     }
     s.flag.p[r] = fl;
+    s.ann_cls.p[r] = (uint8_t)annot_class(fl, nc, nc ? cg[0] : 0u, pos, lq, e->g.ref_len, e->g.ref != nullptr, 0);
     const bool entered = read_enters(fl, cg, nc) && pos >= 0 && !(e->cfg.per_lib && s.lib.p[r] < 0);
     const bool counts = (int)s.mapq.p[r] >= e->cfg.min_mapq && !(fl & BRC_NOCOUNT_MASK);
     uint32_t np = 0; bool past = false;
@@ -703,7 +715,7 @@
         s.sm.p[n0 + i] = b->sm ? b->sm[i] : 0;
         s.tags.p[n0 + i] = b->tags ? b->tags[i] : 0;
     }
-    s.qname_off.n = s.lib.n = s.nm.n = s.sm.n = s.tags.n = s.bq_row.n = s.wide.n = s.piece_cnt.n = s.iev_off.n = n0 + n;
+    s.qname_off.n = s.lib.n = s.nm.n = s.sm.n = s.tags.n = s.bq_row.n = s.wide.n = s.piece_cnt.n = s.iev_off.n = s.ann_cls.n = n0 + n;
     const int32_t maxcnt = e->cfg.max_cnt;
     if (pool && e->accepted + (int64_t)n < (int64_t)maxcnt && !e->heap_built) {
         const size_t CH = (n + (size_t)pool->size() * 4 - 1) / ((size_t)pool->size() * 4);
@@ -776,6 +788,7 @@
         g.ref_hi = std::min<int64_t>(std::max<int64_t>(s.max_end, g.ref_lo), g.ref_len);
     }
     e->st.layout_pieces(g.Lp, e->cfg.per_lib != 0);
+    if (!e->st.layout_annot_lists()) return fail(e, BRC_E_NOMEM, "host staging allocation failed");
     int rc = e->be->upload(e->cfg, s, g);
     if (rc) return fail(e, rc, e->be->last_error());
     e->state = 2; e->t_upload += now_s() - t_in; e->n_regions++;
diff --git a/bam_readcount_amd/csrc/brc_host.h b/bam_readcount_amd/csrc/brc_host.h
--- a/bam_readcount_amd/csrc/brc_host.h
+++ b/bam_readcount_amd/csrc/brc_host.h
@@ -44,6 +44,15 @@
     void destroy() { if (p) A->release(p); p = nullptr; n = cap = 0; }
 };
 
+enum AnnotClass { ANNOT_GENERAL = 0, ANNOT_SIMPLE_OTHER = 1, ANNOT_SIMPLE_UNIFORM = 2 };
+static inline AnnotClass annot_class(uint32_t flag, uint32_t n_cigar, uint32_t cigar0, int32_t pos, int32_t L, int64_t ref_len, bool has_ref, int32_t modal_len) {
+    const bool simple = n_cigar == 1u && (cigar0 & 0xfu) == (uint32_t)CMATCH;
+    const bool dropped = (flag & BRC_PUSH_MASK) != 0u;
+    const bool fallback = !has_ref || pos < 0 || (int64_t)pos + (int64_t)(cigar0 >> 4) > ref_len;
+    if (!(simple && !dropped && !fallback && L > 0 && (int32_t)(cigar0 >> 4) == L)) return ANNOT_GENERAL;
+    return (modal_len > 0 && L == modal_len) ? ANNOT_SIMPLE_UNIFORM : ANNOT_SIMPLE_OTHER;
+}
+
 struct Staged {
     HBuf<int32_t> pos; HBuf<uint16_t> flag; HBuf<uint8_t> mapq; HBuf<int16_t> lib; HBuf<int32_t> l_qseq;
     HBuf<uint32_t> n_cigar; HBuf<uint64_t> cig_off, seq_off, qual_off; HBuf<int32_t> nm, sm; HBuf<uint8_t> tags;
@@ -68,6 +77,9 @@
     HBuf<char> qnames; HBuf<uint64_t> qname_off;
     HBuf<uint32_t> piece_cnt, piece_off;
     HBuf<uint32_t> iev_off;
+    HBuf<uint8_t> ann_cls;
+    HBuf<uint32_t> ann_uniform, ann_other, ann_general;
+    bool layout_annot_lists();
     std::vector<int64_t> lib_base;
     int64_t n_pieces = 0;
     int32_t max_lqseq = 0;
@@ -85,9 +97,9 @@
     std::vector<uint16_t> wanted_tiles(int32_t pos0, int64_t P) const;
     template <class F> void each_read_buf(F f) {
         f(pos); f(flag); f(mapq); f(lib); f(l_qseq); f(n_cigar); f(cig_off); f(seq_off); f(qual_off); f(nm); f(sm); f(tags);
-        f(bq_row); f(wide); f(piece_cnt); f(piece_off); f(iev_off); f(qname_off);
+        f(bq_row); f(wide); f(piece_cnt); f(piece_off); f(iev_off); f(qname_off); f(ann_cls);
     }
-    template <class F> void each_buf(F f) { each_read_buf(f); f(cigar); f(seq4); f(qual); f(qnames); }
+    template <class F> void each_buf(F f) { each_read_buf(f); f(cigar); f(seq4); f(qual); f(qnames); f(ann_uniform); f(ann_other); f(ann_general); }
     bool reserve_reads(size_t reads, size_t cigar_ops);
     void init(const HostAlloc* A);
     void clear();
diff --git a/include/brc_annot.h b/include/brc_annot.h
--- /dev/null
+++ b/include/brc_annot.h
@@ -0,0 +1,48 @@
+#ifndef BRC_ANNOT_H
+#define BRC_ANNOT_H
+
+#include <stddef.h>
+#include <stdint.h>
+
+#ifdef __cplusplus
+extern "C" {
+#endif
+
+#define BRC_ANNOT_ENQUEUED  0
+#define BRC_ANNOT_DECLINED  1
+
+#define BRC_ANNOT_N_UNIFORM   0
+#define BRC_ANNOT_N_OTHER     1
+#define BRC_ANNOT_N_GENERAL   2
+#define BRC_ANNOT_N_DECLINED  3
+
+#define BRC_ANNOT_REFCODE_PAD 16
+
+typedef struct brc_annot_bufs {
+    void* reads;
+    const uint32_t* piece_off;
+    void* pieces;
+    void* rare;
+    void* keyreach;
+    uint8_t* eb;
+    void* ev_raw;
+    uint32_t* bucket_cnt;
+    const uint8_t* refcode;
+    const uint16_t* wanted;
+} brc_annot_bufs;
+
+const char* brc_annot_kind(void);
+
+int brc_annot_region(const void* cfg, size_t cfg_bytes, size_t in_bytes);
+
+int brc_annot_simple(const void* cfg, size_t cfg_bytes, const void* in, size_t in_bytes, const brc_annot_bufs* bufs,
+                     const uint32_t* list, uint32_t n, int32_t uniform_len, void* stream);
+int brc_annot_general(const void* cfg, size_t cfg_bytes, const void* in, size_t in_bytes, const brc_annot_bufs* bufs,
+                      const uint32_t* list, uint32_t n, void* stream);
+
+void brc_annot_last_counts(uint64_t out[4]);
+
+#ifdef __cplusplus
+}
+#endif
+#endif
```

Measured after the change: 334.3 billion. 3.4% lower.
